# ssteinberg/wave_tracer

Measured on AMD Instinct MI355X. Metric: Msamples/sec (whole node), cornell-box 1440^2 wave-mode, higher is better.
Workload: dtype f32

## Files before the change

wave_tracer_amd/csrc/kernels_connect.hip:

```cpp
#include "wtgpu_kernels.h"

namespace wtk {

WT_D bool strategy_valid(const integrator_opts_t& o, int s, int t, int nS, int nT) {
    const int depth = t + s - 2;
    if (t > nT || s > nS) return false;
    if ((t == 1 && s == 1) || depth < 0 || depth > o.max_depth) return false;
    if (!o.emitter_direct && s == 1) return false;
    if (!o.sensor_direct && t == 1) return false;
    if (o.debug_only_s && (int)o.debug_only_s - 1 != s) return false;
    if (o.debug_only_t && (int)o.debug_only_t - 1 != t) return false;
    return true;
}
WT_D bool strategy_class_valid(const integrator_opts_t& o, int sk, int tk, int nS, int nT) {
    const int K = (int)kKeyDim - 1;
    const int t1 = tk < K ? tk : nT, s1 = sk < K ? sk : nS;
    for (int t = tk; t <= t1; ++t)
        for (int s = sk; s <= s1; ++s)
            if (strategy_valid(o, s, t, nS, nT)) return true;
    return false;
}
WT_D int wave_max_i(int v) {
#pragma unroll
    for (int off = 32; off > 0; off >>= 1) v = max(v, __shfl_xor(v, off, 64));
    return v;
}

__global__ void __launch_bounds__(kEnumBlock) k_connect_enum(launch_args_t a) {
    __shared__ uint32_t s_cnt[kNumKeys], s_base[kNumKeys];
    const uint32_t i = blockIdx.x * kEnumBlock + threadIdx.x;
    const size_t W2 = 2 * (size_t)a.st.cap;
    for (uint32_t k = threadIdx.x; k < kNumKeys; k += kEnumBlock) s_cnt[k] = 0;
    int nT = -1, nS = -1;
    if (i < a.nb) {
        nT = (int)a.st.walks[(size_t)(i) * a.st.walk_words + WT_WALK_NVERTS_WORD];
        nS = (int)a.st.walks[(size_t)(a.st.cap + i) * a.st.walk_words + WT_WALK_NVERTS_WORD];
#pragma unroll
        for (int c = 0; c < 4; ++c) a.st.lacc[(size_t)c * a.st.cap + i] = 0.0;
    }
    __syncthreads();
    const int K = (int)kKeyDim - 1;
    const int kT = nT < K ? nT : K, kS = nS < K ? nS : K;
    for (int tk = 0; tk <= kT; ++tk)
        for (int sk = 0; sk <= kS; ++sk)
            if (strategy_class_valid(a.sc.opts, sk, tk, nS, nT)) atomicAdd(&s_cnt[(uint32_t)tk * kKeyDim + (uint32_t)sk], 1u);
    __syncthreads();
    for (uint32_t k = threadIdx.x; k < kNumKeys; k += kEnumBlock) {
        const uint32_t c = s_cnt[k];
        s_base[k] = c ? atomicAdd(a.st.strat_count + k, c) : 0u;
        s_cnt[k] = 0;
    }
    __syncthreads();
    for (int tk = 0; tk <= kT; ++tk)
        for (int sk = 0; sk <= kS; ++sk)
            if (strategy_class_valid(a.sc.opts, sk, tk, nS, nT)) {
                const uint32_t key = (uint32_t)tk * kKeyDim + (uint32_t)sk;
                a.st.strat_items[(size_t)key * a.st.cap + s_base[key] + atomicAdd(&s_cnt[key], 1u)] = i;
            }
}
__global__ void __launch_bounds__(64) k_connect_scan(launch_args_t a) {
    if (a.st.ext)
        for (uint32_t q = threadIdx.x; q < a.st.ext->n_chunks * kChunkCtlWords; q += 64) a.st.ext->chunk_ctl[q] = 0;
    if (threadIdx.x == 0) {
        uint32_t acc = 0;
        for (uint32_t k = 0; k < kNumKeys; ++k) {
            const uint32_t c = a.st.strat_count[k];
            a.st.strat_prefix[k] = acc;
            acc += c;
            a.st.strat_count[k] = 0;
        }
        a.st.strat_prefix[kNumKeys] = acc;
        a.st.ctl[CTL_STRAT_HEAD] = 0;
        a.st.ctl[CTL_STRAT_HEAD_OPEN] = 0;

    }
}
template <bool OPEN>
WT_D void connect_strat_body(const launch_args_t& a) {
    __shared__ stack_entry_t lds[kLdsStack * kBlock];
    __shared__ uint32_t s_prefix[kNumKeys + 1];
    constexpr int K = (int)kKeyDim - 1;
    if (!OPEN) {
        for (uint32_t k = threadIdx.x; k <= kNumKeys; k += kBlock) s_prefix[k] = a.st.strat_prefix[k];
    } else if (threadIdx.x == 0) {
        uint32_t acc = 0;
        for (uint32_t k = 0; k < kNumKeys; ++k) {
            s_prefix[k] = acc;
            if ((int)(k / kKeyDim) == K || (int)(k % kKeyDim) == K) acc += a.st.strat_prefix[k + 1] - a.st.strat_prefix[k];
        }
        s_prefix[kNumKeys] = acc;
    }
    __syncthreads();
    const uint32_t total = s_prefix[kNumKeys];
    bdpt_counters_t ctr;
    memset(&ctr, 0, sizeof(ctr));
    stack_entry_t spill[kSpillStack];
    stack_ref_t stack;
    lds_stack(lds, spill, stack);
    const fsd_pool_t pool{a.st.fsd_hdr, a.st.fsd_edges, a.st.ctl + CTL_FSD_COUNTER, a.st.fsd_cap, a.st.ctl + CTL_FSD_ECOUNTER, a.st.fsd_ecap};
    for (;;) {
        const uint32_t idx = wave_grab(a.st.ctl + (OPEN ? CTL_STRAT_HEAD_OPEN : CTL_STRAT_HEAD)) + (threadIdx.x & 63);
        if (idx - (threadIdx.x & 63) >= total) break;
        if (idx < total) {
            uint32_t lo = 0, hi = kNumKeys;
            while (hi - lo > 1) {
                const uint32_t mid = (lo + hi) >> 1;
                if (s_prefix[mid] <= idx)
                    lo = mid;
                else
                    hi = mid;
            }
            const uint32_t key = lo;
            const int tk = (int)(key / kKeyDim), sk = (int)(key % kKeyDim);
            if (!OPEN && (tk == K || sk == K)) continue;
            const uint32_t i = a.st.strat_items[(size_t)key * a.st.cap + (idx - s_prefix[key])];
            const uint64_t j = a.j0 + i;
            const uint32_t pix = (uint32_t)(j % a.npix);
            const uint64_t smp = a.sample_begin + j / a.npix;
            const uint64_t sample_id = ((uint64_t)pix << 32) | (smp & 0xFFFFFFFFull);
            sample_ctx_t ctx;
            soa_load(a.st.ctx, kCtxWords, i, ctx);
            const vertex_store_t svs{a.st.verts, a.st.vert_words, i}, evs{a.st.verts, a.st.vert_words, (size_t)a.st.cap + i};
            auto one = [&](int s, int t) __attribute__((always_inline)) {
                const stokes_t flux = bdpt_strategy(a.sc, pool, a.film, svs, evs, s, t, ctx, a.seed, sample_id, stack, &ctr, nullptr);
                if (t > 1) {
#pragma unroll
                    for (int c = 0; c < 4; ++c)
                        if (flux.s[c] != 0.f) unsafeAtomicAdd(&a.st.lacc[(size_t)c * a.st.cap + i], (double)flux.s[c]);
                }
            };
            if constexpr (!OPEN) {
                one(sk, tk);
            } else {
                const int nT = (int)a.st.walks[(size_t)i * a.st.walk_words + WT_WALK_NVERTS_WORD];
                const int nS = (int)a.st.walks[((size_t)a.st.cap + i) * a.st.walk_words + WT_WALK_NVERTS_WORD];
                const int t1 = tk == K ? nT : tk, s1 = sk == K ? nS : sk;
                for (int t = tk; t <= t1; ++t)
                    for (int s = sk; s <= s1; ++s)
                        if (strategy_valid(a.sc.opts, s, t, nS, nT)) one(s, t);
            }
        }
    }
    if (a.count_stats) flush_counters(a.st.counters, ctr);
}
__global__ void __launch_bounds__(kBlock, WTGPU_LB_CONNECT) k_connect_strat(launch_args_t a) { connect_strat_body<false>(a); }
__global__ void __launch_bounds__(kBlock, WTGPU_LB_CONNECT) k_connect_strat_open(launch_args_t a) { connect_strat_body<true>(a); }
constexpr uint32_t kPendShadow = 0x80000000u;
WT_D void pending_append(const launch_args_t& a, uint32_t* cctl, bool keep, uint32_t i, int s, int t, const connect_ret_t& cr) {
    const bdpt_ext_t& x = *a.st.ext;
    const unsigned long long m = __ballot(keep);
    if (!m) return;
    const int lane = threadIdx.x & 63;
    const int leader = __ffsll((long long)m) - 1;
    uint32_t base = 0;
    if (lane == leader) base = atomicAdd(cctl + CHUNK_PEND_COUNT, (uint32_t)__popcll(m));
    base = (uint32_t)__shfl((int)base, leader, 64);
    const uint32_t slot = base + (uint32_t)__popcll(m & ((1ull << lane) - 1ull));
    if (!keep || slot >= x.pend_cap) return;
    conn_pending_t r;
    r.i = i;
    r.st = (uint32_t)s | ((uint32_t)t << 16) | (cr.need_shadow ? kPendShadow : 0u);
#pragma unroll
    for (int c = 0; c < 4; ++c) r.L[c] = cr.L.s[c];
    r.o[0] = cr.ray.o.x, r.o[1] = cr.ray.o.y, r.o[2] = cr.ray.o.z;
    r.d[0] = cr.ray.d.x, r.d[1] = cr.ray.d.y, r.d[2] = cr.ray.d.z;
    r.dist = cr.ray.dist;
    x.pend[slot] = r;
}
#ifndef WTGPU_LB_EVAL
#define WTGPU_LB_EVAL 2
#endif
__global__ void __launch_bounds__(kBlock, WTGPU_LB_EVAL) k_connect_eval(launch_args_t a, uint32_t chunk) {
    __shared__ uint32_t s_prefix[kNumKeys + 1];
    for (uint32_t k = threadIdx.x; k <= kNumKeys; k += kBlock) s_prefix[k] = a.st.strat_prefix[k];
    __syncthreads();
    const bdpt_ext_t& x = *a.st.ext;
    uint32_t* cctl = x.chunk_ctl + (size_t)chunk * kChunkCtlWords;
    const uint32_t total = s_prefix[kNumKeys];
    const uint64_t begin = (uint64_t)chunk * x.pend_cap;
    if (begin >= total) return;
    const uint32_t span = (uint32_t)min<uint64_t>(x.pend_cap, total - begin);
    bdpt_counters_t ctr;
    ctr.connections = ctr.shadow_rays = 0;
    const stack_ref_t no_stack = make_stack_ref(nullptr, 0, 0, 0, nullptr);
    const fsd_pool_t pool{a.st.fsd_hdr, a.st.fsd_edges, a.st.ctl + CTL_FSD_COUNTER, a.st.fsd_cap, a.st.ctl + CTL_FSD_ECOUNTER, a.st.fsd_ecap};
    for (;;) {
        const uint32_t off = wave_grab(cctl + CHUNK_EVAL_HEAD) + (threadIdx.x & 63);
        if (off - (threadIdx.x & 63) >= span) break;
        if (off < span) {
            const uint32_t idx = (uint32_t)begin + off;
            uint32_t lo = 0, hi = kNumKeys;
            while (hi - lo > 1) {
                const uint32_t mid = (lo + hi) >> 1;
                if (s_prefix[mid] <= idx)
                    lo = mid;
                else
                    hi = mid;
            }
            const uint32_t key = lo;
            const int t = (int)(key / kKeyDim), s = (int)(key % kKeyDim);
            const uint32_t i = a.st.strat_items[(size_t)key * a.st.cap + (idx - s_prefix[key])];
            const uint64_t j = a.j0 + i;
            const uint32_t pix = (uint32_t)(j % a.npix);
            const uint64_t smp = a.sample_begin + j / a.npix;
            const uint64_t sample_id = ((uint64_t)pix << 32) | (smp & 0xFFFFFFFFull);
            const vertex_store_t svs{a.st.verts, a.st.vert_words, i}, evs{a.st.verts, a.st.vert_words, (size_t)a.st.cap + i};
            connect_ret_t cr;
            bdpt_connect<true>(a.sc, pool, svs, evs, s, t, a.seed, sample_id, no_stack, cr, &ctr, nullptr);
            pending_append(a, cctl, cr.L.s[0] > 0.f, i, s, t, cr);
        }
    }
    if (a.count_stats) {
        unsigned long long vc = ctr.connections, vr = ctr.shadow_rays;
        for (int off = 32; off > 0; off >>= 1) {
            vc += __shfl_down(vc, off, 64);
            vr += __shfl_down(vr, off, 64);
        }
        if ((threadIdx.x & 63) == 0) {
            if (vc) atomicAdd(a.st.counters + offsetof(bdpt_counters_t, connections) / sizeof(unsigned long long), vc);
            if (vr) atomicAdd(a.st.counters + offsetof(bdpt_counters_t, shadow_rays) / sizeof(unsigned long long), vr);
        }
    }
}

__global__ void __launch_bounds__(kBlock, 4) k_connect_shadow(launch_args_t a, uint32_t chunk) {
    __shared__ stack_entry_t lds[kLdsStack * kBlock];
    stack_entry_t spill[kSpillStack];
    stack_ref_t stack;
    lds_stack(lds, spill, stack);
    const bdpt_ext_t& x = *a.st.ext;
    uint32_t* cctl = x.chunk_ctl + (size_t)chunk * kChunkCtlWords;
    const uint32_t n = min(cctl[CHUNK_PEND_COUNT], x.pend_cap);
    if (n == 0) return;
    for (;;) {
        const uint32_t idx = wave_grab(cctl + CHUNK_PEND_HEAD) + (threadIdx.x & 63);
        if (idx - (threadIdx.x & 63) >= n) break;
        bool alive = false;
        if (idx < n) {
            const conn_pending_t& r = x.pend[idx];
            alive = true;
            if (r.st & kPendShadow) alive = !ads_shadow_ray(a.sc, vec3{r.o[0], r.o[1], r.o[2]}, vec3{r.d[0], r.d[1], r.d[2]}, range_t{0.f, r.dist}, stack, nullptr);
        }
        wave_append(x.surv, cctl + CHUNK_SURV_COUNT, alive, idx);
    }
}

#ifndef WTGPU_LB_MIS
#define WTGPU_LB_MIS 2
#endif
__global__ void __launch_bounds__(kBlock, WTGPU_LB_MIS) k_connect_mis(launch_args_t a, uint32_t chunk) {
    const bdpt_ext_t& x = *a.st.ext;
    uint32_t* ctl = a.st.ctl;
    uint32_t* cctl = x.chunk_ctl + (size_t)chunk * kChunkCtlWords;
    const uint32_t n = cctl[CHUNK_SURV_COUNT];
    if (n == 0) return;
    const fsd_pool_t pool{a.st.fsd_hdr, a.st.fsd_edges, ctl + CTL_FSD_COUNTER, a.st.fsd_cap, ctl + CTL_FSD_ECOUNTER, a.st.fsd_ecap};
    bdpt_counters_t ctr;
    ctr.light_splats = 0;
    for (;;) {
        const uint32_t k = wave_grab(cctl + CHUNK_MIS_HEAD) + (threadIdx.x & 63);
        if (k - (threadIdx.x & 63) >= n) break;
        if (k < n) {
            const conn_pending_t& r = x.pend[x.surv[k]];
            const uint32_t i = r.i, st = r.st;
            const int s = (int)(st & 0xFFFFu), t = (int)((st >> 16) & 0x7FFFu);
            stokes_t L;
    #pragma unroll
            for (int c = 0; c < 4; ++c) L.s[c] = r.L[c];
            const uint64_t j = a.j0 + i;
            const uint32_t pix = (uint32_t)(j % a.npix);
            const uint64_t smp = a.sample_begin + j / a.npix;
            const uint64_t sample_id = ((uint64_t)pix << 32) | (smp & 0xFFFFFFFFull);
            sample_ctx_t ctx;
            soa_load(a.st.ctx, kCtxWords, i, ctx);
            const vertex_store_t svs{a.st.verts, a.st.vert_words, i}, evs{a.st.verts, a.st.vert_words, (size_t)a.st.cap + i};
            vertex_nb_t tv;
            sensor_element_t element;
            bool has_element = false;
            if (s <= 1 || t <= 1) bdpt_connect_temp(a.sc, svs, evs, s, t, a.seed, sample_id, tv, element, has_element);
            const stokes_t flux = bdpt_strategy_finish(a.sc, pool, a.film, svs, evs, s, t, ctx, L, tv, element, has_element, &ctr);
            if (t > 1) {
    #pragma unroll
                for (int c = 0; c < 4; ++c)
                    if (flux.s[c] != 0.f) unsafeAtomicAdd(&a.st.lacc[(size_t)c * a.st.cap + i], (double)flux.s[c]);
            }
        }
    }
    if (a.count_stats) {
        unsigned long long v = ctr.light_splats;
        for (int off = 32; off > 0; off >>= 1) v += __shfl_down(v, off, 64);
        if ((threadIdx.x & 63) == 0 && v) atomicAdd(a.st.counters + offsetof(bdpt_counters_t, light_splats) / sizeof(unsigned long long), v);
    }
}

__global__ void __launch_bounds__(kBlock) k_connect_splat(launch_args_t a) {
    const uint32_t i = blockIdx.x * kBlock + threadIdx.x;
    if (i >= a.nb) return;
    sample_ctx_t ctx;
    soa_load(a.st.ctx, kCtxWords, i, ctx);
    stokes_t L;
#pragma unroll
    for (int c = 0; c < 4; ++c) L.s[c] = (float)a.st.lacc[(size_t)c * a.st.cap + i];
    film_splat(a.sc, a.film, ctx.element, L, ctx.k);
}

__global__ void __launch_bounds__(kBlock) k_connect_splat_tiled(launch_args_t a) {
    extern __shared__ double tile[];
    const sensor_t& sn = a.sc.sensor;
    const uint32_t W = a.film.width, H = a.film.height;
    const uint32_t S = film_stokes(sn), P = sn.channels * S, PL = P + 1;
    const uint32_t bpr = (W + kBlock - 1) / kBlock;
    const uint32_t row = blockIdx.x / bpr, x0 = (blockIdx.x % bpr) * kBlock;
    const int r = sn.rf_radius;
    const uint32_t n_px = 3 * kSplatCols;
    for (uint32_t q = threadIdx.x; q < n_px * PL; q += kBlock) tile[q] = 0.0;
    __syncthreads();
    const uint32_t x = x0 + threadIdx.x;
    if (x < W && row < H) {
        const uint64_t p = (uint64_t)row * W + x;
        const uint64_t first = (p + a.npix - (a.j0 % a.npix)) % a.npix;
        for (uint64_t i = first; i < a.nb; i += a.npix) {
            sample_ctx_t ctx;
            soa_load(a.st.ctx, kCtxWords, i, ctx);
            stokes_t L;
#pragma unroll
            for (int c = 0; c < 4; ++c) L.s[c] = (float)a.st.lacc[(size_t)c * a.st.cap + i];
            const rfilter_weights_t rw = film_rfilter_weights(sn, ctx.element.offset);
            float val[16];
            for (uint32_t c = 0; c < sn.channels; ++c) {
                const float f = spectrum_f(a.sc, sn.response_spec[c], ctx.k);
                bool ok = true;
                for (uint32_t q = 0; q < S; ++q) {
                    val[c * S + q] = L.s[q] * f;
                    ok = ok && finitef(val[c * S + q]);
                }
                ok = ok && val[c * S] >= 0.f;
                if (!ok)
                    for (uint32_t q = 0; q < S; ++q) val[c * S + q] = 0.f;
            }
            for (int dy = -r; dy <= r; ++dy) {
                const int y = (int)ctx.element.y + dy;
                if (y < 0 || y >= (int)H) continue;
                for (int dx = -r; dx <= r; ++dx) {
                    const int xx = (int)ctx.element.x + dx;
                    if (xx < 0 || xx >= (int)W) continue;
                    const float w = fmaxf_(0.f, rw.wx[dx + r] * rw.wy[dy + r]) * rw.recp_total;
                    const int ty = y - ((int)row - 1), tx = xx - ((int)x0 - 1);
                    if (ty >= 0 && ty < 3 && tx >= 0 && tx < (int)kSplatCols) {
                        const uint32_t q = (uint32_t)ty * kSplatCols + (uint32_t)tx;
                        unsafeAtomicAdd(&tile[q], (double)w);
                        for (uint32_t c = 0; c < P; ++c) unsafeAtomicAdd(&tile[(size_t)(1 + c) * n_px + q], (double)(w * val[c]));
                    } else {
                        const size_t pix = (size_t)y * W + xx;
                        film_add(&a.film.weight[pix], (double)w);
                        for (uint32_t c = 0; c < P; ++c) film_add(&a.film.value[pix * P + c], (double)(w * val[c]));
                    }
                }
            }
        }
    }
    __syncthreads();
    for (uint32_t q = threadIdx.x; q < n_px; q += kBlock) {
        const int y = (int)row - 1 + (int)(q / kSplatCols), xx = (int)x0 - 1 + (int)(q % kSplatCols);
        if (y < 0 || y >= (int)H || xx < 0 || xx >= (int)W) continue;
        const size_t pix = (size_t)y * W + xx;
        const double wsum = tile[q];
        if (wsum != 0.0) film_add(&a.film.weight[pix], wsum);
        for (uint32_t c = 0; c < P; ++c) {
            const double v = tile[(size_t)(1 + c) * n_px + q];
            if (v != 0.0) film_add(&a.film.value[pix * P + c], v);
        }
    }
}

}
```

wave_tracer_amd/csrc/wt/bdpt.h:

```cpp
#pragma once
#include <cstddef>

#include "bvh.h"
#include "film.h"
#include "fsd.h"

namespace wt {

constexpr uint32_t kMaxVerts = 18;
#ifndef WT_MAX_WALK_ITERS
#define WT_MAX_WALK_ITERS 96
#endif
constexpr uint32_t kMaxWalkIters = WT_MAX_WALK_ITERS;
constexpr uint32_t kWalkIterLimit = 4096;
constexpr uint32_t kMaxConeTris = 64;
#ifdef WT_ORACLE_UNBOUNDED
constexpr uint32_t kMaxEdgeIds = 16384;
#else
constexpr uint32_t kMaxEdgeIds = 96;
#endif

enum vertex_type_e : uint32_t { VT_SENSOR = 0, VT_EMITTER = 1, VT_SURFACE = 2, VT_MEDIUM = 3, VT_FSD = 4 };
enum geo_kind_e : uint32_t { GEO_NONE = 0, GEO_POINT = 1, GEO_SURFACE = 2 };

struct vertex_t {
    uint32_t type;
    uint32_t transport;
    uint32_t delta;
    uint32_t fraunhofer_fsd;
    float pdf_fwd, pdf_bwd;
    float rr_weight;
    int32_t ref;
    int32_t emitter_of_shape;
    uint32_t fsd_slot;
    uint32_t geo_kind;
    uint32_t has_beam;
    surface_t surf;
    beam_t beam;
};
constexpr size_t kVertexWords = sizeof(vertex_t) / 4;
struct vertex_nb_t {
    uint32_t type;
    uint32_t transport;
    uint32_t delta;
    uint32_t fraunhofer_fsd;
    float pdf_fwd, pdf_bwd;
    float rr_weight;
    int32_t ref;
    int32_t emitter_of_shape;
    uint32_t fsd_slot;
    uint32_t geo_kind;
    uint32_t has_beam;
    surface_t surf;
    struct {
        float k;
    } beam;
};
static_assert(offsetof(vertex_nb_t, beam) == offsetof(vertex_t, beam) && offsetof(vertex_nb_t, surf) == offsetof(vertex_t, surf), "vertex_nb_t is a prefix of vertex_t");

struct vertex_store_t {
    uint32_t* base;
    size_t stride;
    size_t idx;
    vertex_t* stage = nullptr;
    uint32_t* staged_idx = nullptr;
    WT_HD void load(uint32_t v, vertex_t& out) const { soa_load(base + (size_t)v * kVertexWords, stride, idx, out); }
    WT_HD void load(uint32_t v, vertex_nb_t& out) const {
        const uint32_t* b = base + (size_t)v * kVertexWords + idx * stride;
        uint32_t* w = reinterpret_cast<uint32_t*>(&out);
#if defined(__HIP_DEVICE_COMPILE__)
#pragma unroll
#endif
        for (size_t i = 0; i < offsetof(vertex_t, beam) / 4; ++i) w[i] = b[i];
        out.beam.k = load_word<float>(v, (offsetof(vertex_t, beam) + offsetof(beam_t, k)) / 4);
    }
    WT_HD vec3 load_wp(uint32_t v) const {
        constexpr size_t o = (offsetof(vertex_t, surf) + offsetof(surface_t, wp)) / 4;
        return vec3{load_word<float>(v, o), load_word<float>(v, o + 1), load_word<float>(v, o + 2)};
    }
    WT_HD void store(uint32_t v, const vertex_t& in) const {
        if (stage) {
            *stage = in;
            *staged_idx = v;
            return;
        }
        soa_store(base + (size_t)v * kVertexWords, stride, idx, in);
    }
    template <class F>
    WT_HD void store_word(uint32_t v, size_t word, F value) const {
        static_assert(sizeof(F) == 4, "");
        uint32_t w;
        __builtin_memcpy(&w, &value, 4);
        if (stage && *staged_idx == v) {
            reinterpret_cast<uint32_t*>(stage)[word] = w;
            return;
        }
        base[idx * stride + (size_t)v * kVertexWords + word] = w;
    }
    template <class F>
    WT_HD F load_word(uint32_t v, size_t word) const {
        const uint32_t w = base[idx * stride + (size_t)v * kVertexWords + word];
        F f;
        __builtin_memcpy(&f, &w, 4);
        return f;
    }
};
#define WT_VWORD(field) (offsetof(vertex_t, field) / 4)

struct fsd_pool_t {
    fsd_aperture_t* hdr;
    fsd_edge_t* edges;
    uint32_t* counter;
    uint32_t cap;
    uint32_t* edge_counter;
    uint32_t edge_cap;
};
WT_HD fsd_edges_ref_t fsd_pool_edges(const fsd_pool_t& p, uint32_t slot) {
    return fsd_edges_ref_t{p.edges + (size_t)p.hdr[slot].edge_offset, 1};
}
WT_HD bool fsd_pool_alloc_edges(const fsd_pool_t& p, uint32_t slot, uint32_t need, fsd_aperture_t& ap) {
    if (!p.edge_counter) {
        ap.edge_offset = slot * kFsdMaxEdges;
        ap.edge_cap = kFsdMaxEdges;
        return true;
    }
    if (need > kFsdMaxEdges) need = kFsdMaxEdges;
    uint32_t off = 0;
    if (need) {
#if defined(__HIP_DEVICE_COMPILE__)
        off = atomicAdd(p.edge_counter, need);
#else
        off = __atomic_fetch_add(p.edge_counter, need, __ATOMIC_RELAXED);
#endif
    }
    ap.edge_offset = off;
    ap.edge_cap = need;
    if ((size_t)off + need > p.edge_cap) {
        ap.edge_offset = 0;
        ap.edge_cap = 0;
        return false;
    }
    return true;
}
WT_HD uint32_t fsd_pool_alloc(const fsd_pool_t& p) {
#if defined(__HIP_DEVICE_COMPILE__)
    const unsigned long long m = __ballot(1);
    const int lane = (int)(threadIdx.x & 63u);
    const int leader = __ffsll((long long)m) - 1;
    uint32_t base = 0;
    if (lane == leader) base = atomicAdd(p.counter, (uint32_t)__popcll(m));
    base = (uint32_t)__shfl((int)base, leader, 64);
    return base + (uint32_t)__popcll(m & ((1ull << lane) - 1ull));
#else
    return __atomic_fetch_add(p.counter, 1u, __ATOMIC_RELAXED);
#endif
}

template <class V>
WT_HD vec3 vertex_wp(const V& v) { return v.surf.wp; }
template <class V>
WT_HD bool vertex_is_on_surface(const scene_t& sc, const V& v) {
    return v.type == VT_SURFACE || (v.type == VT_EMITTER && emitter_is_area(sc.emitters[v.ref])) ||
           (v.type == VT_SENSOR && v.geo_kind == GEO_SURFACE);
}
template <class V>
WT_HD bool vertex_has_real_surface(const scene_t& sc, const V& v) {
    return v.type == VT_SURFACE || (v.type == VT_EMITTER && emitter_is_area(sc.emitters[v.ref]));
}
template <class V>
WT_HD vec3 vertex_ng(const scene_t& sc, const V& v) { return vertex_has_real_surface(sc, v) ? v.surf.geo.n : vec3{0, 0, 1}; }
template <class V>
WT_HD vec3 vertex_ns(const scene_t& sc, const V& v) { return vertex_has_real_surface(sc, v) ? v.surf.shading.n : vec3{0, 0, 1}; }
WT_HD bool vertex_is_interaction(const vertex_t& v) { return v.type == VT_FSD || v.type == VT_SURFACE || v.type == VT_MEDIUM; }
WT_HD bool vertex_on_emitter(const vertex_t& v) { return v.type == VT_EMITTER || (v.type == VT_SURFACE && v.emitter_of_shape >= 0); }
template <class V>
WT_HD int vertex_get_emitter(const V& v) { return v.type == VT_EMITTER ? v.ref : v.emitter_of_shape; }
template <class V>
WT_HD bool vertex_is_delta_emitter(const scene_t& sc, const V& v) {
    return v.type == VT_EMITTER && (emitter_is_delta_direction(sc.emitters[v.ref]) || emitter_is_delta_position(sc.emitters[v.ref]));
}
template <class V>
WT_HD bool vertex_is_delta_sensor(const scene_t& sc, const V& v) {
    return v.type == VT_SENSOR && (sensor_is_delta_direction(sc.sensor) || sensor_is_delta_position(sc.sensor));
}
WT_HD bool vertex_is_connectible(const scene_t& sc, const vertex_t& v) {
    switch (v.type) {
    case VT_FSD: return true;
    case VT_EMITTER: return !emitter_is_delta_direction(sc.emitters[v.ref]);
    case VT_SENSOR: return !sensor_is_delta_direction(sc.sensor);
    case VT_SURFACE: return !material_is_delta_only(sc, v.ref, v.beam.k);
    default: return false;
    }
}
WT_HD vec3 geo_offseted_ray_origin(const scene_t& sc, const vertex_t& v, vec3 ro, vec3 rd) {
    return v.geo_kind == GEO_SURFACE ? surface_offseted_ray_origin(sc, v.surf, ro, rd) : ro;
}

template <class V>
WT_HD float convert_directional_density_to_area(const scene_t& sc, float dpdf_tagged, vec3 p, const V& next) {
    const float dens = pd_density_or_zero(dpdf_tagged);
    if (dens == 0.f) return 0.f;
    const vec3 d = vertex_wp(next) - p;
    const float d2 = length2(d);
    if (d2 == 0.f) return WT_INF;
    float ppdf = dens * (1.f / d2);
    if (vertex_is_on_surface(sc, next)) ppdf *= fabsf(dot(vertex_ng(sc, next), normalize(d)));
    return ppdf;
}
template <class V, class N>
WT_HD float vertex_pdf_next_from_sensor(const scene_t& sc, const V& v, const N& next) {
    const vec3 dl = vertex_wp(next) - vertex_wp(v);
    const float recp_dist2 = 1.f / length2(dl);
    const vec3 d = dl * sqrtf(recp_dist2);
    const float dpdf = pd_density_or_zero(sensor_pdf_direction(sc, d));
    float ppdf = dpdf * recp_dist2;
    if (vertex_is_on_surface(sc, next)) ppdf *= fabsf(dot(vertex_ng(sc, next), d));
    return ppdf;
}
WT_HD float vertex_pdf_sensor(const scene_t& sc) { return pd_density_or_zero(sensor_pdf_position(sc)); }
template <class V, class N>
WT_HD float vertex_pdf_next_from_emitter(const scene_t& sc, const V& v, const N& next) {
    const vec3 dl = vertex_wp(next) - vertex_wp(v);
    const float recp_dist2 = 1.f / length2(dl);
    const vec3 d = dl * sqrtf(recp_dist2);
    const int ei = vertex_get_emitter(v);
    if (emitter_is_infinite(sc.emitters[ei])) return directional_pdf_target_position(sc.emitters[ei], vertex_wp(next));
    const float dpdf = pd_density_or_zero(emitter_pdf_direction(sc, ei, d, vertex_has_real_surface(sc, v) ? &v.surf : nullptr));
    float ppdf = dpdf * recp_dist2;
    if (vertex_is_on_surface(sc, next)) ppdf *= fabsf(dot(vertex_ng(sc, next), d));
    return ppdf;
}
template <class V>
WT_HD float vertex_pdf_emitter(const scene_t& sc, const V& v) {
    const int ei = vertex_get_emitter(v);
    return sc.emitters[ei].select_pmf * pd_density_or_zero(emitter_pdf_position(sc, ei, vertex_has_real_surface(sc, v) ? &v.surf : nullptr));
}
template <class V, class N>
WT_HD float vertex_pdf(const scene_t& sc, const fsd_pool_t& pool, const V& v, vec3 prev_wp, const N& next, uint32_t mode) {
    if (v.type == VT_EMITTER) return vertex_pdf_next_from_emitter(sc, v, next);
    if (v.type == VT_SENSOR) return vertex_pdf_next_from_sensor(sc, v, next);
    const vec3 p = vertex_wp(v);
    const vec3 wiworld = normalize(prev_wp - p);
    const vec3 woworld = normalize(vertex_wp(next) - p);
    float pdf = 0.f;
    if (v.type == VT_SURFACE) {
        const vec3 wi = to_local(v.surf.shading, wiworld), wo = to_local(v.surf.shading, woworld);
        pdf = material_pdf(sc, v.ref, wi, wo, v.beam.k, mode, v.surf.uv);
    } else if (v.type == VT_FSD) {
        const fsd_aperture_t ap = pool.hdr[v.fsd_slot];
        pdf = fsd_pdf(ap, fsd_pool_edges(pool, v.fsd_slot), to_local(ap.frame, woworld));
    }
    return convert_directional_density_to_area(sc, pdf, p, next);
}

WT_HD bool vertex_interact(const scene_t& sc, const fsd_pool_t& pool, const vertex_t& v, vec3 next_wp, bool ignore_fsd, beam_t& out) {
    const vec3 wiworld = -v.beam.env.d;
    const float k = v.beam.k;
    float f = 0.f;
    if (v.fraunhofer_fsd && !ignore_fsd) {
        const fsd_aperture_t ap = pool.hdr[v.fsd_slot];
        const vec3 woworld = normalize(next_wp - vertex_wp(v));
        f = fsd_pdf(ap, fsd_pool_edges(pool, v.fsd_slot), to_local(ap.frame, woworld));
    }
    if (v.type == VT_SURFACE) {
        const surface_t& srf = v.surf;
        const vec3 woworld = normalize(next_wp - vertex_wp(v));
        const vec3 wi = to_local(srf.shading, wiworld), wo = to_local(srf.shading, woworld);
        const vec3 ng = srf.geo.n, ns = srf.shading.n;
        const float wig = dot(wiworld, ng), wog = dot(woworld, ng);
        const float wis = wi.z, wos = wo.z;
        if (wig * wis <= 0.f || wog * wos <= 0.f) return false;
        mueller_t M = material_f(sc, v.ref, wi, wo, k, v.transport, v.surf.uv);
        float scale = 1.f / fabsf(wos);
        if (!veq(ns, ng)) scale *= shading_normals_correction_scale(v.transport, wig, wog, wis, wos);
        M = M * scale;
        if (f > 0.f) M = M + mueller_identity() * f;
        if (mueller_mean_intensity(M) == 0.f) return false;
        out = v.beam;
        beam_transform_surface_interaction(out, srf, woworld, M, 1.f);
        return true;
    }
    if (v.type == VT_FSD) {
        const vec3 p = vertex_wp(v);
        const float beam_dist = dot(p - v.beam.env.o, v.beam.env.d);
        const vec3 woworld = normalize(next_wp - p);
        out = v.beam;
        beam_transform_region_interaction(out, p, beam_dist, woworld, f);
        return true;
    }
    return false;
}

struct conn_end_t {
    vec3 wp, ng;
    uint32_t geo_kind, tuid;
};
template <class V>
WT_HD conn_end_t conn_end_of(const V& v) { return conn_end_t{v.surf.wp, v.surf.geo.n, v.geo_kind, v.surf.tuid}; }
WT_HD vec3 conn_end_offseted_origin(const scene_t& sc, const conn_end_t& e, vec3 ro, vec3 rd) {
    if (e.geo_kind != GEO_SURFACE || e.tuid == kInvalid) return ro;
    const tri_geo_t g = sc.tri_geo[e.tuid];
    const vec3 err = triangle_fp_errors(g.a, g.b, g.c, ro);
    const float offset_dist = dot(err, vabs(e.ng));
    const vec3 offset = offset_dist * e.ng;
    return ro + (dot(rd, offset) >= 0.f ? offset : -offset);
}
struct shadow_ray_t {
    vec3 o, d;
    float dist;
};
WT_HD shadow_ray_t conn_shadow_ray(const scene_t& sc, const conn_end_t& a, const conn_end_t& b) {
    const vec3 rd = normalize(b.wp - a.wp);
    const vec3 o = conn_end_offseted_origin(sc, a, a.wp, rd);
    const vec3 t = conn_end_offseted_origin(sc, b, b.wp, -rd);
    const float dist = length(t - o);
    return shadow_ray_t{o, (t - o) / dist, dist};
}
WT_HD bool bdpt_shadow(const scene_t& sc, const vertex_t& a, const vertex_t& b, const stack_ref_t& stack, bvh_counters_t* ctr) {
    const shadow_ray_t r = conn_shadow_ray(sc, conn_end_of(a), conn_end_of(b));
    return ads_shadow_ray(sc, r.o, r.d, range_t{0.f, r.dist}, stack, ctr);
}

struct walk_t {
    beam_t beam;
    float pdf_from_prev;
    float throughput, rr_weight;
    uint32_t nverts;
    uint32_t active;
    uint32_t rng_draws;
    vec3 prev_wp, prev_ng;
    uint32_t prev_on_surface;
    uint32_t prev_offset_tuid;
};

#define WT_WALK_NVERTS_WORD (offsetof(walk_t, nverts) / 4)

struct sample_ctx_t {
    float k;
    float recp_spectral_pd;
    float k_density;
    sensor_element_t element;
};

struct bdpt_counters_t {
    unsigned long long segments, ray_queries, cone_queries, vertices, connections, shadow_rays;
    unsigned long long cone_tri_overflow, edge_overflow, fsd_edge_overflow, fsd_pool_overflow, fsd_interactions, null_interactions;
    unsigned long long surface_interactions, light_splats;
};

WT_HD void walk_cache_prev(const scene_t& sc, walk_t& w, const vertex_t& v) {
    w.prev_wp = vertex_wp(v);
    w.prev_ng = vertex_ng(sc, v);
    w.prev_on_surface = vertex_is_on_surface(sc, v);
    w.prev_offset_tuid = v.geo_kind == GEO_SURFACE ? v.surf.tuid : kInvalid;
}

WT_HD void bdpt_generate(const scene_t& sc, uint64_t seed, uint64_t sample_id, uint32_t px, uint32_t py, sample_ctx_t& ctx, walk_t& sw, walk_t& ew,
                         const vertex_store_t& svs, const vertex_store_t& evs) {
    sampler_t smp = make_sampler(seed, sample_id, STREAM_SCENE);
    const emitter_k_sample_t ek = scene_sample_emitter_and_spectrum(sc, smp);
    const float k = ek.wavenumber.k;
    const emitter_sample_t es = emitter_sample(sc, ek.emitter, k, smp);
    const bool disc = pd_is_discrete(ek.wavenumber.wpd);
    ctx.k = k;
    ctx.recp_spectral_pd = disc ? 1.f / pd_mass(ek.wavenumber.wpd) : 1.f / scene_sum_spectral_pdf(sc, k);
    ctx.k_density = disc ? pd_mass(ek.wavenumber.wpd) : ek.wavenumber.wpd;
    const sensor_sample_t ss = sensor_sample(sc, px, py, k, smp);
    ctx.element = ss.element;

    vertex_t v;
    v.type = VT_SENSOR;
    v.transport = TRANSPORT_BACKWARD;
    v.delta = 0;
    v.fraunhofer_fsd = 0;
    v.pdf_fwd = -1.f;
    v.pdf_bwd = pd_density_or_zero(ss.ppd);
    v.rr_weight = 1.f;
    v.ref = -1;
    v.emitter_of_shape = -1;
    v.fsd_slot = kInvalid;
    v.has_beam = 1;
    v.beam = ss.beam;
    if (ss.has_surface) {
        v.geo_kind = GEO_SURFACE;
        v.surf = ss.surface;
    } else {
        v.geo_kind = GEO_POINT;
        v.surf = make_dummy_surface(vec3{0, 0, 1}, ss.beam.env.o);
    }
    svs.store(0, v);
    sw.beam = ss.beam;
    sw.pdf_from_prev = ss.dpd;
    sw.throughput = 1.f;
    sw.rr_weight = 1.f;
    sw.nverts = 1;
    sw.active = 1;
    sw.rng_draws = 0;
    walk_cache_prev(sc, sw, v);

    v.type = VT_EMITTER;
    v.transport = TRANSPORT_FORWARD;
    v.pdf_fwd = pd_density_or_zero(es.ppd) * ek.emitter_pdf;
    v.pdf_bwd = -1.f;
    v.ref = ek.emitter;
    v.beam = es.beam;
    if (es.has_surface) {
        v.geo_kind = GEO_SURFACE;
        v.surf = es.surface;
    } else {
        v.geo_kind = GEO_POINT;
        v.surf = make_dummy_surface(vec3{0, 0, 1}, es.beam.env.o);
    }
    evs.store(0, v);
    ew.beam = es.beam;
    ew.pdf_from_prev = es.dpd;
    ew.throughput = 1.f;
    ew.rr_weight = 1.f;
    ew.nverts = 1;
    ew.active = 1;
    ew.rng_draws = 0;
    walk_cache_prev(sc, ew, v);
}

struct walk_trace_in_t {
    cone_t env;
    float k;
    vec3 prev_ng;
    uint32_t prev_offset_tuid;
};
template <class F>
WT_HD F soa_word(const uint32_t* base, size_t stride, size_t idx, size_t word) {
    static_assert(sizeof(F) == 4, "");
    const uint32_t w = base[idx * stride + word];
    F f;
    __builtin_memcpy(&f, &w, 4);
    return f;
}
#define WT_WALK_WORD(field) (offsetof(walk_t, field) / 4)
WT_HD walk_trace_in_t walk_load_trace_in(const uint32_t* base, size_t stride, size_t idx) {
    walk_trace_in_t r;
    r.env.o = {soa_word<float>(base, stride, idx, WT_WALK_WORD(beam.env.o.x)), soa_word<float>(base, stride, idx, WT_WALK_WORD(beam.env.o.y)),
               soa_word<float>(base, stride, idx, WT_WALK_WORD(beam.env.o.z))};
    r.env.d = {soa_word<float>(base, stride, idx, WT_WALK_WORD(beam.env.d.x)), soa_word<float>(base, stride, idx, WT_WALK_WORD(beam.env.d.y)),
               soa_word<float>(base, stride, idx, WT_WALK_WORD(beam.env.d.z))};
    r.env.x = {soa_word<float>(base, stride, idx, WT_WALK_WORD(beam.env.x.x)), soa_word<float>(base, stride, idx, WT_WALK_WORD(beam.env.x.y)),
               soa_word<float>(base, stride, idx, WT_WALK_WORD(beam.env.x.z))};
    r.env.x0 = soa_word<float>(base, stride, idx, WT_WALK_WORD(beam.env.x0));
    r.env.tan_alpha = soa_word<float>(base, stride, idx, WT_WALK_WORD(beam.env.tan_alpha));
    r.env.e = soa_word<float>(base, stride, idx, WT_WALK_WORD(beam.env.e));
    r.env.one_over_e = soa_word<float>(base, stride, idx, WT_WALK_WORD(beam.env.one_over_e));
    r.env.z_apex = soa_word<float>(base, stride, idx, WT_WALK_WORD(beam.env.z_apex));
    r.k = soa_word<float>(base, stride, idx, WT_WALK_WORD(beam.k));
    r.prev_ng = {soa_word<float>(base, stride, idx, WT_WALK_WORD(prev_ng.x)), soa_word<float>(base, stride, idx, WT_WALK_WORD(prev_ng.y)),
                 soa_word<float>(base, stride, idx, WT_WALK_WORD(prev_ng.z))};
    r.prev_offset_tuid = soa_word<uint32_t>(base, stride, idx, WT_WALK_WORD(prev_offset_tuid));
    return r;
}
WT_HD cone_t walk_trace_envelope(const scene_t& sc, const walk_trace_in_t& w) {
    cone_t env = w.env;
    if (w.prev_offset_tuid != kInvalid) {
        const tri_geo_t g = sc.tri_geo[w.prev_offset_tuid];
        const vec3 err = triangle_fp_errors(g.a, g.b, g.c, env.o);
        const float offset_dist = dot(err, vabs(w.prev_ng));
        const vec3 offset = offset_dist * w.prev_ng;
        env.o = env.o + (dot(env.d, offset) >= 0.f ? offset : -offset);
    }
    return env;
}

WT_HD cone_t walk_trace_envelope(const scene_t& sc, const walk_t& w) {
    cone_t env = w.beam.env;
    if (w.prev_offset_tuid != kInvalid) {
        const tri_geo_t g = sc.tri_geo[w.prev_offset_tuid];
        const vec3 err = triangle_fp_errors(g.a, g.b, g.c, env.o);
        const float offset_dist = dot(err, vabs(w.prev_ng));
        const vec3 offset = offset_dist * w.prev_ng;
        env.o = env.o + (dot(env.d, offset) >= 0.f ? offset : -offset);
    }
    return env;
}

WT_HD bool walk_append_vertex(const scene_t& sc, walk_t& w, const vertex_store_t& vs, vertex_t& v, float pdf_fwd, float pdf_revr) {
    if (veq(w.prev_wp, vertex_wp(v))) return false;
    const float pv = convert_directional_density_to_area(sc, w.pdf_from_prev, w.prev_wp, v);
    if (v.transport == TRANSPORT_FORWARD)
        v.pdf_fwd = pv;
    else
        v.pdf_bwd = pv;
    v.beam = w.beam;
    v.has_beam = 1;
    {
        const float dens = pd_density_or_zero(pdf_revr);
        float prev_rev = 0.f;
        if (dens != 0.f) {
            const vec3 d = w.prev_wp - vertex_wp(v);
            const float d2 = length2(d);
            if (d2 == 0.f)
                prev_rev = WT_INF;
            else {
                prev_rev = dens * (1.f / d2);
                if (w.prev_on_surface) prev_rev *= fabsf(dot(w.prev_ng, normalize(d)));
            }
        }
        vs.store_word(w.nverts - 1, v.transport == TRANSPORT_BACKWARD ? WT_VWORD(pdf_fwd) : WT_VWORD(pdf_bwd), prev_rev);
    }
    w.pdf_from_prev = pdf_fwd;
    vs.store(w.nverts, v);
    w.nverts++;
    walk_cache_prev(sc, w, v);
    return true;
}

WT_HD bool walk_continue(const scene_t& sc, walk_t& w, const vertex_store_t& vs, bool allow_RR, sampler_t& smp) {
    if ((int)w.nverts > sc.opts.max_depth + 1) return false;
    if (!allow_RR || !sc.opts.RR) return true;
    vs.store_word(w.nverts - 1, WT_VWORD(rr_weight), w.rr_weight);
    const float r = w.throughput < 1.f ? fmaxf_(w.throughput, .5f) : 1.f;
    if (sampler_r(smp) <= r) {
        const float scale = 1.f / r;
        w.rr_weight *= scale;
        w.throughput *= scale;
        return true;
    }
    return false;
}

WT_HD float region_triangle_flux(const scene_t& sc, const frame_t& beam_frame, const cone_t& envelope, const range_t& izr, vec2 sigma, uint32_t tuid,
                                 bool want_front) {
    const tri_geo_t g = sc.tri_geo[tuid];
    const bool front_face = dot(g.n, -envelope.d) > 0.f;
    if (front_face != want_front) return 0.f;
    return region_local_triangle_flux(envelope, izr, centre(izr), sigma, to_local(beam_frame, g.a - envelope.o), to_local(beam_frame, g.b - envelope.o),
                                      to_local(beam_frame, g.c - envelope.o));
}

struct fsd_defer_t {
    uint32_t split_no_primary, no_primary;
    uint32_t known_no_primary;
    uint32_t has_gather, gather_n_edges, gather_edge_overflow;
    float gather_flux;
    const uint32_t* gather_edges;
    uint32_t defer_sampling, to_sampling_pass, have_aperture;
    uint32_t pending, resolved;
    uint32_t slot, base, next_try, end_draws;
    fsd_sample_t fs;
#ifdef WTGPU_STEP_PROF
    long long marks[8];
#endif
};

#if defined(WTGPU_STEP_PROF) && defined(__HIP_DEVICE_COMPILE__)
#define WT_STEP_MARK(i) \
    if (defer) defer->marks[i] = clock64()
#else
#define WT_STEP_MARK(i) ((void)0)
#endif
template <int MODE = 0, class TriList>
WT_HD bool bdpt_walk_step(const scene_t& sc, walk_t& w, const trav_result_t& tr, const TriList& tris, const vertex_store_t& vs,
                          const fsd_pool_t& pool, uint64_t seed, uint64_t sample_id, uint32_t stream, bdpt_counters_t* ctr,
                          const stack_ref_t* primary_query_stack = nullptr, fsd_defer_t* defer = nullptr) {
    if (tr.empty) return false;
    sampler_t smp = make_sampler(seed, sample_id, stream, w.rng_draws);
    beam_t& beam = w.beam;
    const float beam_dist = tr.dist;
    const range_t izr{beam_dist, beam_dist + tr.region_depth};
    const bool is_ballistic = tr.ballistic || beam_is_ray(beam);
    const vec3 origin_wp = tr.origin;
    const vec3 interaction_wp = origin_wp + izr.min * beam.env.d;
    const frame_t beam_frame = cone_frame(beam.env);
    const cone_t envelope = beam.env;
    const vec3 sd3 = beam_footprint(beam, beam_dist) / kBeamEnvelope;
    const vec2 sigma{sd3.x, sd3.y};

    uint32_t primary = kInvalid;
    ray_tri_hit_t phit{WT_INF, 0.f, 0.f};
    double integrated_flux = 0.0;
    if (is_ballistic) {
        primary = tr.tuid;
        phit.dist = tr.dist;
        phit.bx = tr.bx;
        phit.by = tr.by;
    } else {
        if (defer && defer->known_no_primary) {
        } else if (tr.aborted == 2) {
            if (tr.tuid != kInvalid) {
                primary = tr.tuid;
                phit.dist = tr.pdist;
                phit.bx = tr.bx;
                phit.by = tr.by;
            }
        } else if (primary_query_stack && tr.overflow > 0) {
            const float wtol = cone_intersection_tolerance(origin_wp, sc.world_min, sc.world_max, sc.world_max);
            ray_hit_t rh;
            if (ads_intersect_ray(sc, origin_wp, beam.env.d, grow(izr, wtol), *primary_query_stack, rh)) {
                const tri_geo_t g = sc.tri_geo[rh.tuid];
                const float fptol = cone_intersection_tolerance(origin_wp, g.a, g.b, g.c);
                if (contains(grow(izr, fptol), rh.dist)) {
                    primary = rh.tuid;
                    phit.dist = rh.dist;
                    phit.bx = rh.bx;
                    phit.by = rh.by;
                }
            }
        } else
        for (uint32_t i = 0; i < tr.ntris; ++i) {
            const uint32_t tuid = tris[i];
            const tri_geo_t g = sc.tri_geo[tuid];
            const float fptol = cone_intersection_tolerance(origin_wp, g.a, g.b, g.c);
            ray_tri_hit_t h;
            if (intersect_ray_tri(origin_wp, beam.env.d, g.a, g.b, g.c, grow(izr, fptol), h) && h.dist < phit.dist) {
                primary = tuid;
                phit = h;
            }
        }
        if (primary == kInvalid && defer && defer->split_no_primary) {
            defer->no_primary = 1;
            return false;
        }
        WT_STEP_MARK(0);
    }

    bool do_RR = true;
    bool ok = true;
    bool took_surface = false;
    if constexpr (MODE != 2) {
    if (primary != kInvalid) {
        took_surface = true;
        const tri_geo_t g = sc.tri_geo[primary];
        const vec3 sampled_tri_wp = origin_wp + envelope.d * phit.dist;
        surface_t srf = make_surface(sc, primary, g.n, vec2{phit.bx, phit.by}, sampled_tri_wp);
        srf.footprint = beam_surface_footprint_static(beam, srf, beam_dist);
        const shape_t shp = sc.shapes[srf.shape];
        const float k = beam.k;
        const uint32_t transport = beam.transport;
        const vec3 ng = srf.geo.n, ns = srf.shading.n;
        const vec3 wiworld = -beam.env.d;
        const vec3 wi = to_local(srf.shading, wiworld);
        const float wig = dot(wiworld, ng), wis = wi.z;
        ok = wig * wis > 0.f;
        bsdf_sample_t bs;
        if (ok) {
            bs = material_sample(sc, shp.material, wi, k, transport, smp, srf.uv);
            ok = bs.valid && bs.dpd != 0.f;
        }
        if (ok) {
            const bool is_delta = pd_is_discrete(bs.dpd);
            const vec3 wo = bs.wo;
            const vec3 woworld = normalize(to_world(srf.shading, wo));
            const float wog = dot(woworld, ng), wos = wo.z;
            if (ctr) ctr->surface_interactions++;
            ok = wog * wos > 0.f;
            if (ok) {
                const float pdf_revr = material_pdf(sc, shp.material, wo, wi, k, flip_transport(transport), srf.uv);
                vertex_t v;
                v.type = VT_SURFACE;
                v.transport = transport;
                v.delta = is_delta;
                v.fraunhofer_fsd = 0;
                v.pdf_fwd = v.pdf_bwd = -1.f;
                v.rr_weight = 1.f;
                v.ref = shp.material;
                v.emitter_of_shape = shp.emitter;
                v.fsd_slot = kInvalid;
                v.geo_kind = GEO_SURFACE;
                v.surf = srf;
                ok = walk_append_vertex(sc, w, vs, v, bs.dpd, pdf_revr);
                if (ok) {
                    if (ctr) ctr->vertices++;
                    float ws = 1.f;
                    if (!veq(ns, ng)) ws *= shading_normals_correction_scale(transport, wig, wog, wis, wos);
                    beam_transform_surface_interaction(beam, srf, woworld, bs.M, ws);
                    w.throughput *= ws * mueller_mean_intensity(bs.M);
                    if (transport == TRANSPORT_BACKWARD && bs.eta != 1.f) w.throughput /= sqr(bs.eta);
                }
            }
        }
    }
    }
    if constexpr (MODE != 1) {
    if (!took_surface) {
        WT_STEP_MARK(1);
        uint32_t edge_ids[kMaxEdgeIds];
        const uint32_t* eids = edge_ids;
        uint32_t n_edge_ids = 0;
        const bool have_ap = defer && (defer->resolved || defer->have_aperture);
        if (have_ap) {
            n_edge_ids = 1;
        } else if (sc.opts.FSD && !is_ballistic && defer && defer->has_gather) {
            n_edge_ids = defer->gather_n_edges;
            eids = defer->gather_edges;
            if (ctr) ctr->edge_overflow += defer->gather_edge_overflow;
        } else if (sc.opts.FSD && !is_ballistic) {
            for (uint32_t i = 0; i < tr.ntris; ++i) {
                const tri_meta_t m = sc.tri_meta[tris[i]];
                for (int e = 0; e < 3; ++e) {
                    const uint32_t id = m.edge[e];
                    if (id == kInvalid) continue;
                    uint32_t pos = 0;
                    while (pos < n_edge_ids && edge_ids[pos] < id) ++pos;
                    if (pos < n_edge_ids && edge_ids[pos] == id) continue;
                    if (n_edge_ids == kMaxEdgeIds) {
                        if (ctr) ctr->edge_overflow++;
                        continue;
                    }
                    for (uint32_t j = n_edge_ids; j > pos; --j) edge_ids[j] = edge_ids[j - 1];
                    edge_ids[pos] = id;
                    ++n_edge_ids;
                }
            }
        }
        WT_STEP_MARK(2);
        if (n_edge_ids > 0) {
            const bool resume = defer && defer->resolved;
            const uint32_t slot = have_ap ? defer->slot : fsd_pool_alloc(pool);
            if (slot >= pool.cap) {
                if (ctr) ctr->fsd_pool_overflow++;
                ok = false;
            } else {
                fsd_aperture_t ap;
                if (have_ap) {
                    ap = pool.hdr[slot];
                } else {
                    uint32_t need = 0;
                    if (pool.edge_counter) {
                        const vec2 cse = sigma * kBeamEnvelope;
                        const float max_len = .33f * fmaxf_(cse.x, cse.y);
                        for (uint32_t ei = 0; ei < n_edge_ids; ++ei) need += fsd_count_segments(sc, beam_frame, envelope, cse, max_len, eids[ei]);
                    }
                    if (!fsd_pool_alloc_edges(pool, slot, need, ap) && ctr) ctr->fsd_pool_overflow++;
                }
                const fsd_edges_ref_t ed{pool.edges + (size_t)ap.edge_offset, 1};
                if (!have_ap) {
                    fsd_build_aperture(sc, beam_frame, beam.k, 1.f, envelope, eids, n_edge_ids, sigma, ap, ed);
                    WT_STEP_MARK(3);
                    if (ctr && ap.overflow) ctr->fsd_edge_overflow += ap.overflow;
                    pool.hdr[slot] = ap;
                    if (ap.n_edges > 0 && defer && defer->defer_sampling) {
                        defer->to_sampling_pass = 1;
                        defer->slot = slot;
                        return false;
                    }
                }
                if (ap.n_edges > 0 && !resume) {
                    if (defer && defer->has_gather) {
                        integrated_flux = defer->gather_flux;
                    } else {
                        for (uint32_t i = 0; i < tr.ntris; ++i)
                            integrated_flux += region_triangle_flux(sc, beam_frame, envelope, izr, sigma, tris[i], tr.front_face != 0);
                    }
                    const float I = (float)(1.0 - integrated_flux);
                    ap.recp_I = I > 0.f ? 1.f / I : 0.f;
                    pool.hdr[slot] = ap;
                }
                if (ap.n_edges == 0) {
                    beam_transform_restart(beam, interaction_wp, beam_dist);
                    do_RR = false;
                } else {
                    fsd_sample_t fs;
                    if (!defer) {
                        fs = fsd_sample(sc, ap, ed, smp);
                    } else if (resume) {
                        fs = defer->fs;
                        sampler_seek(smp, defer->end_draws);
                    } else {
                        const uint32_t max_tries = fsd_max_tries(ap), base = fsd_tries_base(smp);
                        const uint32_t t1 = max_tries < kFsdInlineTries ? max_tries : kFsdInlineTries;
                        fsd_try_t r{{0.f, 0.f}, 0.f, 0u};
                        const uint32_t t = fsd_run_tries(sc, ap, ed, smp, base, 0, t1, r);
                        if (t == 0xFFFFFFFFu && t1 < max_tries) {
                            defer->pending = 1;
                            defer->slot = slot;
                            defer->base = base;
                            defer->next_try = t1;
                            return false;
                        }
                        const bool accepted = t != 0xFFFFFFFFu;
                        sampler_seek(smp, fsd_draws_after(base, accepted ? t : max_tries - 1u));
                        fs = fsd_finalize(ap, accepted, r.x, r.f);
                    }
                    ok = !(fs.dpd == 0.f || fs.weight == 0.f);
                    if (ok) {
                        if (ctr) ctr->fsd_interactions++;
                        const vec3 woworld = to_world(ap.frame, fs.wo);
                        vertex_t v;
                        v.type = VT_FSD;
                        v.transport = beam.transport;
                        v.delta = 0;
                        v.fraunhofer_fsd = 1;
                        v.pdf_fwd = v.pdf_bwd = -1.f;
                        v.rr_weight = 1.f;
                        v.ref = -1;
                        v.emitter_of_shape = -1;
                        v.fsd_slot = slot;
                        v.geo_kind = GEO_POINT;
                        v.surf = make_dummy_surface(vec3{0, 0, 1}, interaction_wp);
                        ok = walk_append_vertex(sc, w, vs, v, fs.dpd, fs.dpd);
                        if (ok) {
                            if (ctr) ctr->vertices++;
                            beam_transform_region_interaction(beam, interaction_wp, beam_dist, woworld, fs.weight);
                            w.throughput *= fs.weight;
                        }
                    }
                }
            }
        } else {
            do_RR = false;
            beam_transform_restart(beam, interaction_wp, beam_dist);
            if (ctr) ctr->null_interactions++;
        }
    }
    }
    WT_STEP_MARK(4);
    bool cont = false;
    if (ok) cont = walk_continue(sc, w, vs, do_RR, smp);
    WT_STEP_MARK(5);
    w.rng_draws = smp.draws;
    return cont;
}

enum walk_class_e : uint32_t { WCLS_DIFFUSE = 0, WCLS_DIELECTRIC = 1, WCLS_SPM = 2, WCLS_ANY = 3, kNumWalkClasses = 4, WCLS_NO_PRIMARY = 4, WCLS_END = 5 };
struct primary_hit_t {
    uint32_t tuid;
    float dist, bx, by;
};
WT_HD uint32_t walk_class_of_material_type(int32_t type) { return type >= 0 && type < (int32_t)MAT_COMPOSITE ? (uint32_t)type : (uint32_t)WCLS_ANY; }
WT_HD uint32_t walk_class_of_triangle(const scene_t& sc, uint32_t tuid) {
    return walk_class_of_material_type(sc.materials[sc.shapes[sc.tri_meta[tuid].shape_idx].material].type);
}
template <class TriList>
WT_HD uint32_t bdpt_classify(const scene_t& sc, vec3 beam_d, bool beam_ray, const trav_result_t& tr, const TriList& tris, const unsigned char* tri_class, primary_hit_t& ph) {
    ph.tuid = kInvalid;
    ph.dist = WT_INF;
    ph.bx = ph.by = 0.f;
    if (tr.empty) return WCLS_END;
    const bool is_ballistic = tr.ballistic || beam_ray;
    if (is_ballistic) {
        ph.tuid = tr.tuid;
        ph.dist = tr.dist;
        ph.bx = tr.bx;
        ph.by = tr.by;
    } else if (tr.aborted == 2) {
        if (tr.tuid != kInvalid) {
            ph.tuid = tr.tuid;
            ph.dist = tr.pdist;
            ph.bx = tr.bx;
            ph.by = tr.by;
        }
    } else {
        const range_t izr{tr.dist, tr.dist + tr.region_depth};
        for (uint32_t i = 0; i < tr.ntris; ++i) {
            const uint32_t tuid = tris[i];
            const tri_geo_t g = sc.tri_geo[tuid];
            const float fptol = cone_intersection_tolerance(tr.origin, g.a, g.b, g.c);
            ray_tri_hit_t h;
            if (intersect_ray_tri(tr.origin, beam_d, g.a, g.b, g.c, grow(izr, fptol), h) && h.dist < ph.dist) {
                ph.tuid = tuid;
                ph.dist = h.dist;
                ph.bx = h.bx;
                ph.by = h.by;
            }
        }
    }
    if (ph.tuid == kInvalid) return WCLS_NO_PRIMARY;
    return tri_class ? (uint32_t)tri_class[ph.tuid] : walk_class_of_triangle(sc, ph.tuid);
}

struct walk_rec_t {
    uint32_t* p;
    template <class F>
    WT_HD F get(size_t word) const {
        static_assert(sizeof(F) == 4, "");
        const uint32_t w = p[word];
        F f;
        __builtin_memcpy(&f, &w, 4);
        return f;
    }
    template <class F>
    WT_HD void set(size_t word, F value) const {
        static_assert(sizeof(F) == 4, "");
        uint32_t w;
        __builtin_memcpy(&w, &value, 4);
        p[word] = w;
    }
    WT_HD vec3 get3(size_t word) const { return vec3{get<float>(word), get<float>(word + 1), get<float>(word + 2)}; }
    WT_HD void set3(size_t word, vec3 v) const {
        set(word, v.x);
        set(word + 1, v.y);
        set(word + 2, v.z);
    }
};
template <int CLS>
WT_HD bool bdpt_surface_step(const scene_t& sc, const walk_rec_t& wr, vec3 origin_wp, float beam_dist, const primary_hit_t& ph, const vertex_store_t& vs, uint64_t seed,
                             uint64_t sample_id, uint32_t stream, bdpt_counters_t* ctr) {
    sampler_t smp = make_sampler(seed, sample_id, stream, wr.get<uint32_t>(WT_WALK_WORD(rng_draws)));
    cone_t env;
    {
        uint32_t* e = reinterpret_cast<uint32_t*>(&env);
#if defined(__HIP_DEVICE_COMPILE__)
#pragma unroll
#endif
        for (size_t i = 0; i < sizeof(cone_t) / 4; ++i) e[i] = wr.p[WT_WALK_WORD(beam.env) + i];
    }
    const float k = wr.get<float>(WT_WALK_WORD(beam.k));
    const uint32_t transport = wr.get<uint32_t>(WT_WALK_WORD(beam.transport));
    const uint32_t primary = ph.tuid;
    const vec3 gn = sc.tri_geo[primary].n;
    const vec3 sampled_tri_wp = origin_wp + env.d * ph.dist;
    surface_t srf = make_surface(sc, primary, gn, vec2{ph.bx, ph.by}, sampled_tri_wp);
    srf.footprint = cone_surface_footprint_static(env, srf, beam_dist);
    const shape_t shp = sc.shapes[srf.shape];
    const vec3 ng = srf.geo.n, ns = srf.shading.n;
    const vec3 wiworld = -env.d;
    const vec3 wi = to_local(srf.shading, wiworld);
    const float wig = dot(wiworld, ng), wis = wi.z;
    if (!(wig * wis > 0.f)) return false;
    const bsdf_sample_t bs = material_sample<CLS>(sc, shp.material, wi, k, transport, smp, srf.uv);
    if (!(bs.valid && bs.dpd != 0.f)) return false;
    const bool is_delta = pd_is_discrete(bs.dpd);
    const vec3 wo = bs.wo;
    const vec3 woworld = normalize(to_world(srf.shading, wo));
    const float wog = dot(woworld, ng), wos = wo.z;
    if (ctr) ctr->surface_interactions++;
    if (!(wog * wos > 0.f)) return false;
    const float pdf_revr = material_pdf<CLS>(sc, shp.material, wo, wi, k, flip_transport(transport), srf.uv);
    const vec3 prev_wp = wr.get3(WT_WALK_WORD(prev_wp));
    if (veq(prev_wp, srf.wp)) return false;
    uint32_t nverts = wr.get<uint32_t>(WT_WALK_WORD(nverts));
    {
        struct {
            uint32_t type;
            int32_t ref;
            uint32_t geo_kind;
            const surface_t& surf;
        } vview{VT_SURFACE, shp.material, GEO_SURFACE, srf};
        const float pv = convert_directional_density_to_area(sc, wr.get<float>(WT_WALK_WORD(pdf_from_prev)), prev_wp, vview);
        const uint32_t hdr[12] = {VT_SURFACE,
                                  transport,
                                  is_delta ? 1u : 0u,
                                  0u,
                                  __builtin_bit_cast(uint32_t, transport == TRANSPORT_FORWARD ? pv : -1.f),
                                  __builtin_bit_cast(uint32_t, transport == TRANSPORT_FORWARD ? -1.f : pv),
                                  __builtin_bit_cast(uint32_t, 1.f),
                                  (uint32_t)shp.material,
                                  (uint32_t)shp.emitter,
                                  kInvalid,
                                  (uint32_t)GEO_SURFACE,
                                  1u};
        static_assert(WT_VWORD(type) == 0 && WT_VWORD(transport) == 1 && WT_VWORD(delta) == 2 && WT_VWORD(fraunhofer_fsd) == 3 && WT_VWORD(pdf_fwd) == 4 && WT_VWORD(pdf_bwd) == 5 &&
                          WT_VWORD(rr_weight) == 6 && WT_VWORD(ref) == 7 && WT_VWORD(emitter_of_shape) == 8 && WT_VWORD(fsd_slot) == 9 && WT_VWORD(geo_kind) == 10 &&
                          WT_VWORD(has_beam) == 11 && WT_VWORD(surf) == 12,
                      "vertex_t header layout");
        uint32_t* vp = vs.base + vs.idx * vs.stride + (size_t)nverts * kVertexWords;
#if defined(__HIP_DEVICE_COMPILE__)
#pragma unroll
#endif
        for (int i = 0; i < 12; ++i) vp[i] = hdr[i];
        const uint32_t* sw = reinterpret_cast<const uint32_t*>(&srf);
#if defined(__HIP_DEVICE_COMPILE__)
#pragma unroll
#endif
        for (size_t i = 0; i < sizeof(surface_t) / 4; ++i) vp[WT_VWORD(surf) + i] = sw[i];
        const uint32_t* ew = reinterpret_cast<const uint32_t*>(&env);
#if defined(__HIP_DEVICE_COMPILE__)
#pragma unroll
#endif
        for (size_t i = 0; i < sizeof(cone_t) / 4; ++i) vp[WT_VWORD(beam) + i] = ew[i];
#if defined(__HIP_DEVICE_COMPILE__)
#pragma unroll
#endif
        for (size_t i = sizeof(cone_t) / 4; i < sizeof(beam_t) / 4; ++i) vp[WT_VWORD(beam) + i] = wr.p[WT_WALK_WORD(beam) + i];
        const float dens = pd_density_or_zero(pdf_revr);
        float prev_rev = 0.f;
        if (dens != 0.f) {
            const vec3 d = prev_wp - srf.wp;
            const float d2 = length2(d);
            if (d2 == 0.f)
                prev_rev = WT_INF;
            else {
                prev_rev = dens * (1.f / d2);
                if (wr.get<uint32_t>(WT_WALK_WORD(prev_on_surface))) prev_rev *= fabsf(dot(wr.get3(WT_WALK_WORD(prev_ng)), normalize(d)));
            }
        }
        vs.store_word(nverts - 1, transport == TRANSPORT_BACKWARD ? WT_VWORD(pdf_fwd) : WT_VWORD(pdf_bwd), prev_rev);
        ++nverts;
        wr.set(WT_WALK_WORD(pdf_from_prev), bs.dpd);
        wr.set(WT_WALK_WORD(nverts), nverts);
        wr.set3(WT_WALK_WORD(prev_wp), srf.wp);
        wr.set3(WT_WALK_WORD(prev_ng), ng);
        wr.set(WT_WALK_WORD(prev_on_surface), 1u);
        wr.set(WT_WALK_WORD(prev_offset_tuid), srf.tuid);
    }
    if (ctr) ctr->vertices++;
    float ws = 1.f;
    if (!veq(ns, ng)) ws *= shading_normals_correction_scale(transport, wig, wog, wis, wos);
    {
        beam_t b;
        float sid;
        b.env = cone_through_surface_footprint(srf, srf.wp, woworld, env.tan_alpha, &sid);
        b.k = k;
        b.transport = transport;
        uint32_t* bw = reinterpret_cast<uint32_t*>(&b);
#if defined(__HIP_DEVICE_COMPILE__)
#pragma unroll
#endif
        for (size_t i = offsetof(beam_t, frame) / 4; i < sizeof(beam_t) / 4; ++i) bw[i] = wr.p[WT_WALK_WORD(beam) + i];
        beam_apply_bsdf(b, ws * bs.M, woworld, srf, cone_frame(b.env));
        b.self_intersection_distance = sid;
#if defined(__HIP_DEVICE_COMPILE__)
#pragma unroll
#endif
        for (size_t i = 0; i < sizeof(beam_t) / 4; ++i) wr.p[WT_WALK_WORD(beam) + i] = bw[i];
    }
    float throughput = wr.get<float>(WT_WALK_WORD(throughput)) * (ws * mueller_mean_intensity(bs.M));
    if (transport == TRANSPORT_BACKWARD && bs.eta != 1.f) throughput /= sqr(bs.eta);
    bool cont = true;
    float rr_weight = wr.get<float>(WT_WALK_WORD(rr_weight));
    if ((int)nverts > sc.opts.max_depth + 1)
        cont = false;
    else if (sc.opts.RR) {
        vs.store_word(nverts - 1, WT_VWORD(rr_weight), rr_weight);
        const float r = throughput < 1.f ? fmaxf_(throughput, .5f) : 1.f;
        if (sampler_r(smp) <= r) {
            const float scale = 1.f / r;
            rr_weight *= scale;
            throughput *= scale;
        } else
            cont = false;
    }
    wr.set(WT_WALK_WORD(throughput), throughput);
    wr.set(WT_WALK_WORD(rr_weight), rr_weight);
    wr.set(WT_WALK_WORD(rng_draws), smp.draws);
    return cont;
}

WT_HD uint32_t connect_stream(int s, int t) {
    if (s < 32 && t < 32) return STREAM_CONNECT + (uint32_t)t * 32u + (uint32_t)s;
    return STREAM_CONNECT + 1024u + (uint32_t)t * 4096u + (uint32_t)s;
}
struct connect_ret_t {
    stokes_t L;
    vertex_t temporary_vert;
    uint32_t has_temp;
    sensor_element_t element;
    uint32_t has_element;
    shadow_ray_t ray;
    uint32_t need_shadow;
};

template <bool DEFER>
WT_HD stokes_t connect_and_integrate(const scene_t& sc, const beam_t& db, const conn_end_t& dv, const beam_t& eb, const conn_end_t& ev, const stack_ref_t& stack,
                                     bdpt_counters_t* ctr, bvh_counters_t* bctr, connect_ret_t& ret) {
    if (beam_intensity(db) == 0.f || beam_intensity(eb) == 0.f) return stokes_zero();
    if (ctr) ctr->shadow_rays++;
    const shadow_ray_t ray = conn_shadow_ray(sc, dv, ev);
    if (DEFER) {
        const stokes_t L = integrate_beams(db, eb);
        if (L.s[0] > 0.f) {
            ret.ray = ray;
            ret.need_shadow = 1;
        }
        return L;
    }
    if (ads_shadow_ray(sc, ray.o, ray.d, range_t{0.f, ray.dist}, stack, bctr)) return stokes_zero();
    return integrate_beams(db, eb);
}

WT_HD void make_temp_vertex(vertex_t& v, uint32_t type, uint32_t transport, int ref, bool has_surface, const surface_t& surface, vec3 p) {
    v.type = type;
    v.transport = transport;
    v.delta = 0;
    v.fraunhofer_fsd = 0;
    v.pdf_fwd = v.pdf_bwd = -1.f;
    v.rr_weight = 1.f;
    v.ref = ref;
    v.emitter_of_shape = -1;
    v.fsd_slot = kInvalid;
    v.has_beam = 0;
    if (has_surface) {
        v.geo_kind = GEO_SURFACE;
        v.surf = surface;
    } else {
        v.geo_kind = GEO_POINT;
        v.surf = make_dummy_surface(vec3{0, 0, 1}, p);
    }
}
WT_HD bool vertex_store_connectible(const scene_t& sc, const vertex_store_t& vs, uint32_t idx) {
    struct {
        uint32_t type;
        int32_t ref;
        struct {
            float k;
        } beam;
    } v{vs.load_word<uint32_t>(idx, WT_VWORD(type)), vs.load_word<int32_t>(idx, WT_VWORD(ref)), {vs.load_word<float>(idx, WT_VWORD(beam) + offsetof(beam_t, k) / 4)}};
    switch (v.type) {
    case VT_FSD: return true;
    case VT_EMITTER: return !emitter_is_delta_direction(sc.emitters[v.ref]);
    case VT_SENSOR: return !sensor_is_delta_direction(sc.sensor);
    case VT_SURFACE: return !material_is_delta_only(sc, v.ref, v.beam.k);
    default: return false;
    }
}

template <bool DEFER = false>
WT_HD void bdpt_connect(const scene_t& sc, const fsd_pool_t& pool, const vertex_store_t& svs, const vertex_store_t& evs, int s, int t,
                        uint64_t seed, uint64_t sample_id, const stack_ref_t& stack, connect_ret_t& ret, bdpt_counters_t* ctr, bvh_counters_t* bctr) {
    ret.L = stokes_zero();
    ret.has_temp = 0;
    ret.has_element = 0;
    ret.need_shadow = 0;
    sampler_t smp = make_sampler(seed, sample_id, connect_stream(s, t));
    if (ctr) ctr->connections++;

    if (s == 0) {
        vertex_t last;
        svs.load(t - 1, last);
        if (vertex_on_emitter(last)) {
            beam_t QE = last.beam;
            beam_scale(QE, last.rr_weight);
            ret.L = emitter_Li(sc, vertex_get_emitter(last), QE, last.surf);
        }
    } else if (t == 0) {
        if (sensor_is_virtual(sc.sensor)) {
            vertex_t last;
            evs.load(s - 1, last);
            vertex_nb_t current;
            evs.load(s - 2, current);
            const vec3 wp_end = vertex_wp(last);
            const beam_t& beam = last.beam;
            const float dist = length(wp_end - beam.env.o);
            sensor_direct_connection_t dc = vplane_Si(sc, beam, range_t{0.f, dist});
            if (dc.valid) {
                ret.element = dc.element;
                ret.has_element = 1;
                float wgt = current.rr_weight;
                if (vertex_is_on_surface(sc, current) && (current.type == VT_FSD || current.type == VT_SURFACE || current.type == VT_MEDIUM) && !current.delta)
                    wgt /= fabsf(dot(dc.beam.env.d, vertex_ns(sc, current)));
                wgt /= fabsf(dot(dc.beam.env.d, dc.surface.geo.n));
                beam_scale(dc.beam, wgt);
                make_temp_vertex(ret.temporary_vert, VT_SENSOR, TRANSPORT_BACKWARD, -1, true, dc.surface, dc.beam.env.o);
                ret.has_temp = 1;
                ret.L = integrate_beams(dc.beam, beam);
            }
        }
    } else if (s == 1) {
        vertex_t last;
        svs.load(t - 1, last);
        if (vertex_is_connectible(sc, last)) {
            const float k = last.beam.k;
            const vec3 wp = vertex_wp(last);
            emitter_direct_sample_t ed = scene_sample_emitter_direct(sc, wp, k, smp);
            if ((pd_is_discrete(ed.dpd) || ed.dpd != 0.f) && beam_intensity(ed.beam) > 0.f) {
                float wgt = last.rr_weight;
                if (vertex_is_on_surface(sc, last)) wgt *= fabsf(dot(ed.beam.env.d, vertex_ns(sc, last)));
                beam_scale(ed.beam, wgt);
                make_temp_vertex(ret.temporary_vert, VT_EMITTER, TRANSPORT_FORWARD, ed.emitter, ed.has_surface, ed.surface, ed.beam.env.o);
                ret.has_temp = 1;
                beam_t db;
                if (vertex_interact(sc, pool, last, vertex_wp(ret.temporary_vert), false, db))
                    ret.L = connect_and_integrate<DEFER>(sc, db, conn_end_of(last), ed.beam, conn_end_of(ret.temporary_vert), stack, ctr, bctr, ret);
            }
        }
    } else if (t == 1) {
        vertex_t last;
        evs.load(s - 1, last);
        const bool is_virtual = sensor_is_virtual(sc.sensor);
        const bool do_direct = (is_virtual || last.type != VT_FSD) && vertex_is_connectible(sc, last);
        if (do_direct) {
            sensor_direct_sample_t sd = sensor_sample_direct(sc, vertex_wp(last), last.beam.k, smp);
            if ((pd_is_discrete(sd.dpd) || sd.dpd != 0.f) && beam_intensity(sd.beam) > 0.f) {
                float wgt = last.rr_weight;
                if (vertex_is_on_surface(sc, last)) wgt *= fabsf(dot(sd.beam.env.d, vertex_ns(sc, last)));
                beam_scale(sd.beam, wgt);
                make_temp_vertex(ret.temporary_vert, VT_SENSOR, TRANSPORT_BACKWARD, -1, sd.has_surface, sd.surface, sd.beam.env.o);
                ret.has_temp = 1;
                beam_t eb;
                if (vertex_interact(sc, pool, last, vertex_wp(ret.temporary_vert), false, eb)) {
                    ret.L = connect_and_integrate<DEFER>(sc, sd.beam, conn_end_of(ret.temporary_vert), eb, conn_end_of(last), stack, ctr, bctr, ret);
                    ret.element = sd.element;
                    ret.has_element = 1;
                }
            }
        }
    } else {
        const vec3 ev_wp = evs.load_wp(s - 1), sv_wp = svs.load_wp(t - 1);
        const vec3 dl = ev_wp - sv_wp;
        if (vertex_store_connectible(sc, evs, s - 1) && vertex_store_connectible(sc, svs, t - 1) && !(dl.x == 0.f && dl.y == 0.f && dl.z == 0.f)) {
            beam_t eb, db;
            conn_end_t ev_end, sv_end;
            vec3 ev_ns, sv_ns;
            bool ev_on, sv_on, heb, hdb = false;
            float ev_rr, sv_rr;
            {
                vertex_t ev;
                evs.load(s - 1, ev);
                heb = vertex_interact(sc, pool, ev, sv_wp, true, eb);
                ev_end = conn_end_of(ev);
                ev_ns = vertex_ns(sc, ev);
                ev_on = vertex_is_on_surface(sc, ev);
                ev_rr = ev.rr_weight;
            }
            if (heb) {
                vertex_t sv;
                svs.load(t - 1, sv);
                hdb = vertex_interact(sc, pool, sv, ev_wp, true, db);
                sv_end = conn_end_of(sv);
                sv_ns = vertex_ns(sc, sv);
                sv_on = vertex_is_on_surface(sc, sv);
                sv_rr = sv.rr_weight;
            }
            if (heb && hdb) {
                const float recp_d2 = 1.f / length2(dl);
                const vec3 d = dl * sqrtf(recp_d2);
                float wev = ev_rr;
                float wsv = sv_rr * recp_d2;
                if (sv_on) wev *= fabsf(dot(sv_ns, d));
                if (ev_on) wsv *= fabsf(dot(ev_ns, d));
                beam_scale(db, wsv);
                beam_scale(eb, wev);
                ret.L = connect_and_integrate<DEFER>(sc, db, sv_end, eb, ev_end, stack, ctr, bctr, ret);
            }
        }
    }
}
WT_HD void bdpt_connect_temp(const scene_t& sc, const vertex_store_t& svs, const vertex_store_t& evs, int s, int t, uint64_t seed, uint64_t sample_id, vertex_nb_t& tv,
                             sensor_element_t& element, bool& has_element) {
    has_element = false;
    vertex_t tmp;
    bool has_temp = false;
    sampler_t smp = make_sampler(seed, sample_id, connect_stream(s, t));
    if (s == 0) {
    } else if (t == 0) {
        if (sensor_is_virtual(sc.sensor)) {
            vertex_t last;
            evs.load(s - 1, last);
            const float dist = length(vertex_wp(last) - last.beam.env.o);
            const sensor_direct_connection_t dc = vplane_Si(sc, last.beam, range_t{0.f, dist});
            if (dc.valid) {
                element = dc.element;
                has_element = true;
                make_temp_vertex(tmp, VT_SENSOR, TRANSPORT_BACKWARD, -1, true, dc.surface, dc.beam.env.o);
                has_temp = true;
            }
        }
    } else if (s == 1) {
        const emitter_direct_sample_t ed = scene_sample_emitter_direct(sc, svs.load_wp(t - 1), svs.load_word<float>(t - 1, WT_VWORD(beam) + offsetof(beam_t, k) / 4), smp);
        make_temp_vertex(tmp, VT_EMITTER, TRANSPORT_FORWARD, ed.emitter, ed.has_surface, ed.surface, ed.beam.env.o);
        has_temp = true;
    } else if (t == 1) {
        const sensor_direct_sample_t sd = sensor_sample_direct(sc, evs.load_wp(s - 1), evs.load_word<float>(s - 1, WT_VWORD(beam) + offsetof(beam_t, k) / 4), smp);
        make_temp_vertex(tmp, VT_SENSOR, TRANSPORT_BACKWARD, -1, sd.has_surface, sd.surface, sd.beam.env.o);
        has_temp = true;
        element = sd.element;
        has_element = true;
    }
    if (has_temp) __builtin_memcpy(&tv, &tmp, offsetof(vertex_t, beam));
    tv.beam.k = 0.f;
}

template <class TV>
WT_HD float bdpt_mis_weight(const scene_t& sc, const fsd_pool_t& pool, const vertex_store_t& svs, const vertex_store_t& evs, int s, int t, const TV& tv) {
    if (s + t <= 2) return 1.f;
    float srev_last = 0.f, srev_prev = 0.f, spdf_first = 0.f, erev_last = 0.f, erev_prev = 0.f, epdf_first = 0.f;
    bool has_srev_last = false, has_srev_prev = false, has_spdf_first = false, has_erev_last = false, has_erev_prev = false, has_epdf_first = false;
    if (s == 0) {
        vertex_nb_t last, prev;
        svs.load(t - 1, last);
        svs.load(t - 2, prev);
        srev_last = vertex_pdf_emitter(sc, last);
        srev_prev = vertex_pdf_next_from_emitter(sc, last, prev);
        has_srev_last = has_srev_prev = true;
    } else if (t == 0) {
        vertex_nb_t prev;
        evs.load(s - 2, prev);
        erev_last = vertex_pdf_sensor(sc);
        if (sensor_is_virtual(sc.sensor))
            erev_prev = vertex_pdf_next_from_sensor(sc, tv, prev);
        else {
            vertex_nb_t last;
            evs.load(s - 1, last);
            erev_prev = vertex_pdf_next_from_sensor(sc, last, prev);
        }
        has_erev_last = has_erev_prev = true;
    } else if (s == 1) {
        vertex_nb_t last;
        svs.load(t - 1, last);
        srev_last = vertex_pdf_next_from_emitter(sc, tv, last);
        erev_last = vertex_pdf(sc, pool, last, svs.load_wp(t - 2), tv, TRANSPORT_BACKWARD);
        epdf_first = vertex_pdf_emitter(sc, tv);
        has_srev_last = has_erev_last = has_epdf_first = true;
    } else if (t == 1) {
        vertex_nb_t last;
        evs.load(s - 1, last);
        erev_last = vertex_pdf_next_from_sensor(sc, tv, last);
        srev_last = vertex_pdf(sc, pool, last, evs.load_wp(s - 2), tv, TRANSPORT_FORWARD);
        spdf_first = vertex_pdf_sensor(sc);
        has_erev_last = has_srev_last = has_spdf_first = true;
    } else {
        vertex_nb_t ev, sv;
        evs.load(s - 1, ev);
        svs.load(t - 1, sv);
        const vec3 ev_prev_wp = evs.load_wp(s - 2), sv_prev_wp = svs.load_wp(t - 2);
        vertex_nb_t ev_prev, sv_prev;
        evs.load(s - 2, ev_prev);
        svs.load(t - 2, sv_prev);
        erev_last = vertex_pdf(sc, pool, sv, sv_prev_wp, ev, TRANSPORT_BACKWARD);
        erev_prev = vertex_pdf(sc, pool, ev, vertex_wp(sv), ev_prev, TRANSPORT_BACKWARD);
        srev_last = vertex_pdf(sc, pool, ev, ev_prev_wp, sv, TRANSPORT_FORWARD);
        srev_prev = vertex_pdf(sc, pool, sv, vertex_wp(ev), sv_prev, TRANSPORT_FORWARD);
        has_erev_last = has_erev_prev = has_srev_last = has_srev_prev = true;
    }
    bool delta_emitter, delta_sensor;
    if (s == 1)
        delta_emitter = vertex_is_delta_emitter(sc, tv);
    else if (s > 1) {
        struct {
            uint32_t type;
            int32_t ref;
        } ev0{evs.load_word<uint32_t>(0, WT_VWORD(type)), evs.load_word<int32_t>(0, WT_VWORD(ref))};
        delta_emitter = vertex_is_delta_emitter(sc, ev0);
    } else
        delta_emitter = true;
    if (t == 1)
        delta_sensor = vertex_is_delta_sensor(sc, tv);
    else if (t > 1) {
        struct {
            uint32_t type;
        } sv0{svs.load_word<uint32_t>(0, WT_VWORD(type))};
        delta_sensor = vertex_is_delta_sensor(sc, sv0);
    } else
        delta_sensor = true;

    float sum_Ri = 0.f, ri = 1.f;
    {
        bool del_i = false;
        for (int i0 = t - 1; i0 >= 0; i0 -= 4) {
            float F[4], R[4];
            uint32_t D[4];
#pragma unroll
            for (int j = 0; j < 4; ++j) {
                const int i = i0 - j;
                F[j] = R[j] = 0.f;
                D[j] = 0u;
                if (i >= 0) {
                    F[j] = svs.load_word<float>(i, WT_VWORD(pdf_bwd));
                    R[j] = svs.load_word<float>(i, WT_VWORD(pdf_fwd));
                    if (i > 0) D[j] = svs.load_word<uint32_t>(i - 1, WT_VWORD(delta));
                }
            }
#pragma unroll
            for (int j = 0; j < 4; ++j) {
                const int i = i0 - j;
                if (i < 0) break;
                const float f = (i == 0 && has_spdf_first) ? spdf_first : F[j];
                const float rv = (i == t - 1 && has_srev_last) ? srev_last : ((i == t - 2 && has_srev_prev) ? srev_prev : R[j]);
                const bool del_prev = i > 0 ? D[j] != 0 : delta_sensor;
                const float fwd = (finitef(f) && f > FLT_EPSILON) ? f : 1.f;
                const float rev = (finitef(rv) && rv > FLT_EPSILON) ? rv : 1.f;
                ri *= rev / fwd;
                if (!del_i && !del_prev) sum_Ri += ri;
                del_i = del_prev;
            }
        }
    }
    ri = 1.f;
    {
        bool del_i = false;
        for (int i0 = s - 1; i0 >= 0; i0 -= 4) {
            float F[4], R[4];
            uint32_t D[4];
#pragma unroll
            for (int j = 0; j < 4; ++j) {
                const int i = i0 - j;
                F[j] = R[j] = 0.f;
                D[j] = 0u;
                if (i >= 0) {
                    F[j] = evs.load_word<float>(i, WT_VWORD(pdf_fwd));
                    R[j] = evs.load_word<float>(i, WT_VWORD(pdf_bwd));
                    if (i > 0) D[j] = evs.load_word<uint32_t>(i - 1, WT_VWORD(delta));
                }
            }
#pragma unroll
            for (int j = 0; j < 4; ++j) {
                const int i = i0 - j;
                if (i < 0) break;
                const float f = (i == 0 && has_epdf_first) ? epdf_first : F[j];
                const float rv = (i == s - 1 && has_erev_last) ? erev_last : ((i == s - 2 && has_erev_prev) ? erev_prev : R[j]);
                const bool del_prev = i > 0 ? D[j] != 0 : delta_emitter;
                const float fwd = (finitef(f) && f > FLT_EPSILON) ? f : 1.f;
                const float rev = (finitef(rv) && rv > FLT_EPSILON) ? rv : 1.f;
                ri *= rev / fwd;
                if (!del_i && !del_prev) sum_Ri += ri;
                del_i = del_prev;
            }
        }
    }
    return 1.f / (1.f + sum_Ri);
}

template <class TV>
WT_HD stokes_t bdpt_strategy_finish(const scene_t& sc, const fsd_pool_t& pool, const film_t& film, const vertex_store_t& svs, const vertex_store_t& evs, int s, int t,
                                    const sample_ctx_t& ctx, const stokes_t& L, const TV& tv, const sensor_element_t& element, bool has_element, bdpt_counters_t* ctr) {
    float mis;
    if (sc.opts.debug_only_s || sc.opts.debug_only_t)
        mis = ctx.recp_spectral_pd;
    else if (sc.opts.MIS)
        mis = bdpt_mis_weight(sc, pool, svs, evs, s, t, tv) * ctx.recp_spectral_pd;
    else
        mis = 1.f / (float(s + t + 1) * ctx.k_density);
    const stokes_t flux = L * mis;
    if (t > 1) return flux;
    if (has_element) {
        film_splat_direct(sc, film, element, flux, ctx.k);
        if (ctr) ctr->light_splats++;
    }
    return stokes_zero();
}
template <bool STAGED = false>
WT_HD stokes_t bdpt_strategy(const scene_t& sc, const fsd_pool_t& pool, const film_t& film, const vertex_store_t& svs, const vertex_store_t& evs, int s,
                             int t, const sample_ctx_t& ctx, uint64_t seed, uint64_t sample_id, const stack_ref_t& stack, bdpt_counters_t* ctr,
                             bvh_counters_t* bctr) {
    connect_ret_t cr;
    bdpt_connect<STAGED>(sc, pool, svs, evs, s, t, seed, sample_id, stack, cr, ctr, bctr);
    if (!(cr.L.s[0] > 0.f)) return stokes_zero();
    if (STAGED) {
        if (cr.need_shadow && ads_shadow_ray(sc, cr.ray.o, cr.ray.d, range_t{0.f, cr.ray.dist}, stack, bctr)) return stokes_zero();
        vertex_nb_t tv;
        sensor_element_t element;
        bool has_element;
        bdpt_connect_temp(sc, svs, evs, s, t, seed, sample_id, tv, element, has_element);
        return bdpt_strategy_finish(sc, pool, film, svs, evs, s, t, ctx, cr.L, tv, element, has_element, ctr);
    }
    return bdpt_strategy_finish(sc, pool, film, svs, evs, s, t, ctx, cr.L, cr.temporary_vert, cr.element, cr.has_element != 0, ctr);
}

template <bool STAGED = false>
WT_HD void bdpt_connect_all(const scene_t& sc, const fsd_pool_t& pool, const film_t& film, const vertex_store_t& svs, const vertex_store_t& evs, int nT,
                            int nS, const sample_ctx_t& ctx, uint64_t seed, uint64_t sample_id, const stack_ref_t& stack, bdpt_counters_t* ctr,
                            bvh_counters_t* bctr) {
    stokes_t L = stokes_zero();
    for (int t = 0; t <= nT; ++t)
        for (int s = 0; s <= nS; ++s) {
            const int depth = t + s - 2;
            if ((t == 1 && s == 1) || depth < 0) continue;
            if (!sc.opts.emitter_direct && s == 1) continue;
            if (!sc.opts.sensor_direct && t == 1) continue;
            if (depth > sc.opts.max_depth) break;
            if (sc.opts.debug_only_s && (int)sc.opts.debug_only_s - 1 != s) continue;
            if (sc.opts.debug_only_t && (int)sc.opts.debug_only_t - 1 != t) continue;
            L = L + bdpt_strategy<STAGED>(sc, pool, film, svs, evs, s, t, ctx, seed, sample_id, stack, ctr, bctr);
        }
#if defined(WTGPU_DEBUG_PRINT) && defined(__HIP_DEVICE_COMPILE__)
    if (ctx.element.x == 0 && ctx.element.y == 0)
        printf("dbg3 L=%g nT=%d nS=%d ch=%u rfs=%g r=%d\n", L.s[0], nT, nS, sc.sensor.channels, sc.sensor.rfilter_sigma, sc.sensor.rf_radius);
#endif
    film_splat(sc, film, ctx.element, L, ctx.k);
}

}
```

wave_tracer_amd/csrc/wtgpu.hip:

```cpp
#include "wtgpu_host.h"

thread_local std::string g_err;

static void note_rounds(wtgpu_scene* s, uint32_t n) { s->rounds_hist[s->rounds_hist_n++ % 8u] = n; }
static int drain_rec(wtgpu_scene* s, chunk_rec_t& r) {
    if (!r.busy) return WTGPU_OK;
    HIP_CHECK(hipEventSynchronize(r.ev[r.ev_final]));
    const uint32_t rounds = r.h_ctl[CTL_ROUNDS];
    s->cap_hits += r.h_ctl[CTL_COUNT0 + (r.rounds_launched & 1u)] + r.h_ctl[CTL_BACK0 + (r.rounds_launched & 1u)];
    s->acc[4] += rounds;
    s->acc[5] += rounds;
    s->acc[6] += 1;
    s->rounds_launched_total += r.rounds_launched;
    if (s->knobs.timing) {
        auto elapsed = [](hipEvent_t a, hipEvent_t b) {
            float ms = 0.f;
            return hipEventElapsedTime(&ms, a, b) == hipSuccess ? ms : 0.f;
        };
        s->acc[0] += elapsed(r.ev[0], r.ev[1]);
        size_t e = 1;
        for (uint32_t k = 0; k < r.rounds_timed; ++k, e += 6) {
            static const int slot[6] = {1, 7, 2, 8, 9, 10};
            for (int q = 0; q < 6; ++q) s->acc[slot[q]] += elapsed(r.ev[e + q], r.ev[e + q + 1]);
        }
        s->acc[3] += elapsed(r.ev[e], r.ev[r.ev_final]);
    }
    r.busy = false;
    return WTGPU_OK;
}

struct batch_launcher_t {
    wtgpu_scene* s;
    const wtgpu_scene::knobs_t& K;
    uint32_t grid_round = 0, grid_heavy = 0;
    bool path_mode = false;
    bool ev_fail = false;
    static constexpr int kHpSlots = 64;
    bool hp_on = false, trace_on = false;
    double hp_t[kHpSlots] = {0};
    unsigned long hp_n[kHpSlots] = {0};
    static const char** hp_labels() {
        static const char* labels[kHpSlots] = {nullptr};
        return labels;
    }
    static int hp_slot(const char* label) {
        static std::mutex m;
        std::lock_guard<std::mutex> l(m);
        const char** labels = hp_labels();
        int i = 0;
        while (i < kHpSlots - 1 && labels[i] && std::strcmp(labels[i], label) != 0) ++i;
        if (!labels[i]) labels[i] = label;
        return i;
    }
    explicit batch_launcher_t(wtgpu_scene* s_) : s(s_), K(s_->knobs) {
        int n_cu = 256;
        (void)hipDeviceGetAttribute(&n_cu, hipDeviceAttributeMultiprocessorCount, s->device);
        grid_round = (uint32_t)n_cu * K.round_blocks_per_cu;
        grid_heavy = (uint32_t)n_cu * K.heavy_waves_per_cu;
        path_mode = s->host.opts.integrator != INTEGRATOR_BDPT;
        hp_on = K.host_prof != 0;
        trace_on = K.trace_launch != 0;
    }
#define HP_LAUNCH(kernel, ...)                                                                                            \
    do {                                                                                                                  \
        if (trace_on) {    \
            fprintf(stderr, "[wtgpu launch] %s ...", #kernel);                                                            \
            hipLaunchKernelGGL(kernel, __VA_ARGS__);                                                                      \
            const hipError_t e_ = hipDeviceSynchronize();                                                                 \
            fprintf(stderr, " done (%s)\n", hipGetErrorString(e_));                                                       \
        } else if (hp_on) {                                                                                                      \
            static const int slot_ = hp_slot(#kernel);                                                                    \
            const auto t0_ = std::chrono::steady_clock::now();                                                            \
            hipLaunchKernelGGL(kernel, __VA_ARGS__);                                                                      \
            hp_t[slot_] += std::chrono::duration<double, std::micro>(std::chrono::steady_clock::now() - t0_).count();     \
            hp_n[slot_]++;                                                                                                \
        } else                                                                                                            \
            hipLaunchKernelGGL(kernel, __VA_ARGS__);                                                                      \
    } while (0)
    void rec(chunk_rec_t& r, hipStream_t st_) {
        const auto hp0_ = std::chrono::steady_clock::now();
        if (s->knobs.timing && r.ev_used + 1 >= r.ev.size()) return;
        if (s->knobs.timing && hipEventRecord(r.ev[r.ev_used++], st_) != hipSuccess) ev_fail = true;
        if (hp_on) { static const int slot_ = hp_slot("hipEventRecord"); hp_t[slot_] += std::chrono::duration<double, std::micro>(std::chrono::steady_clock::now() - hp0_).count(); hp_n[slot_]++; }
    }
    uint32_t g_full(uint32_t nb) const { return std::min<uint32_t>(grid_round, ((path_mode ? 1u : 2u) * nb + kBlock - 1) / kBlock); }
    void generate(const launch_args_t& a, chunk_rec_t& r, hipStream_t st_) {
        r.ev_used = 0;
        r.rounds_launched = 0;
        r.rounds_timed = 0;
        rec(r, st_);
        if (path_mode)
            HP_LAUNCH(k_path_generate, dim3((a.nb + kBlock - 1) / kBlock), dim3(kBlock), 0, st_, a);
        else
            HP_LAUNCH(k_generate, dim3((a.nb + kBlock - 1) / kBlock), dim3(kBlock), 0, st_, a);
        rec(r, st_);
    }
    int rounds(const launch_args_t& a, const path_state_t* ps, chunk_rec_t& r, hipStream_t st_, uint32_t r_begin, uint32_t r_end, int stage_from = 0) {
        const uint32_t nb = a.nb, walks_per_sample = path_mode ? 1u : 2u, gf = g_full(nb);
        const uint32_t grid_div_b = K.grid_div_b, grid_div_c = K.grid_div_c, grid_mul_flux = K.grid_mul_flux;
        const int dbg_stage = (int)K.dbg_stage;
        for (uint32_t round = r_begin; round < r_end; ++round) {
            const int in = (int)(round & 1u), first = round == 0 ? 1 : 0;
            if (s->knobs.timing && r.ev_used + 7 < r.ev.size()) r.rounds_timed++;
            if (round == K.stagger_round && K.stagger_round > 0) {
                HIP_CHECK(hipEventRecord(r.ev_stagger, st_));
                s->ev_stagger_last = r.ev_stagger;
            }
            uint32_t g0, gh;
            if (K.decay_q > 0) {
                const double f = std::min(1.0, (double)K.decay_c * std::pow(K.decay_q * .01, (double)round));
                g0 = std::max<uint32_t>(2u, (uint32_t)(gf * f));
                gh = std::max<uint32_t>(2u, (uint32_t)(std::min<uint32_t>(grid_heavy, walks_per_sample * nb) * f));
            } else {
                const uint32_t shrink = round < K.shrink_r1 ? 1u : (round < K.shrink_r2 ? K.shrink_f1 : K.shrink_f2);
                g0 = std::max<uint32_t>(1u, gf / shrink);
                gh = std::max<uint32_t>(1u, std::min<uint32_t>(grid_heavy, walks_per_sample * nb) / (round < K.shrink_r1 ? 1u : (round < K.shrink_r2 ? K.shrink_h1 : 32u)));
            }
            const int sf = round == r_begin ? stage_from : 0;
            if (sf <= 0 && dbg_stage >= 2 + 3 * (int)round) {
                if (round < K.trace_ab) {
                    const int rc = trace_ab_round(s, a, st_, in, first, round, g0);
                    if (rc) return rc;
                } else if (K.trace_sm || (K.trace_staged && round < K.trace_staged_rounds))
                    launch_trace_alt(s, a, st_, in, first, round, g0);
                else
                    HP_LAUNCH(k_trace_refill, dim3(g0), dim3(kBlock), 0, st_, a, in, first, round);
            }
            rec(r, st_);
            if (sf <= 1 && dbg_stage >= 3 + 3 * (int)round) HP_LAUNCH(k_trace_heavy, dim3(gh), dim3(64), 0, st_, a);
            rec(r, st_);
            if (path_mode) {
                if (round > 0) HP_LAUNCH(k_path_fsd, dim3(gh), dim3(64), 0, st_, a, ps, round);
                if (dbg_stage >= 4 + 3 * (int)round) HP_LAUNCH(k_path_interact, dim3(g0), dim3(kBlock), 0, st_, a, ps, in, first, round);
                HP_LAUNCH(k_path_edges, dim3(gh), dim3(64), 0, st_, a, ps);
                HP_LAUNCH(k_path_interact_b, dim3(std::max<uint32_t>(1u, g0 / 2u)), dim3(kBlock), 0, st_, a, ps, in, round);
                HP_LAUNCH(k_path_nee, dim3(gh), dim3(64), 0, st_, a, ps, round);
                rec(r, st_);
                rec(r, st_);
                rec(r, st_);
                rec(r, st_);
                continue;
            }
            if (sf > 2) {
            } else if (K.sorted_interact) {
                HP_LAUNCH(k_classify, dim3(g0), dim3(kBlock), 0, st_, a, in, first);
                if (K.sorted_interact >= 2)
                    HP_LAUNCH(k_interact_sorted, dim3(g0), dim3(kBlock), 0, st_, a, in);
                else {
                HP_LAUNCH(k_interact_diffuse, dim3(std::max<uint32_t>(1u, g0 / K.grid_div_cls[0])), dim3(kBlock), 0, st_, a, in);
                HP_LAUNCH(k_interact_dielectric, dim3(std::max<uint32_t>(1u, g0 / K.grid_div_cls[1])), dim3(kBlock), 0, st_, a, in);
                HP_LAUNCH(k_interact_spm, dim3(std::max<uint32_t>(1u, g0 / K.grid_div_cls[2])), dim3(kBlock), 0, st_, a, in);
                HP_LAUNCH(k_interact_any, dim3(std::max<uint32_t>(1u, g0 / K.grid_div_cls[3])), dim3(kBlock), 0, st_, a, in);
                }
            } else if (K.coop_io)
                HP_LAUNCH(k_interact_coop, dim3(g0), dim3(kBlock), 0, st_, a, in, first);
            else
                HP_LAUNCH(k_interact, dim3(g0), dim3(kBlock), 0, st_, a, in, first);
            rec(r, st_);
            if (sf <= 3) HP_LAUNCH(k_edges, dim3(gh), dim3(64), 0, st_, a);
            if (sf <= 4) HP_LAUNCH(k_interact_b, dim3(std::max<uint32_t>(1u, g0 / grid_div_b)), dim3(kBlock), 0, st_, a, in);
            rec(r, st_);
            HP_LAUNCH(k_flux_split, dim3(std::max<uint32_t>(1u, gh / 4u)), dim3(64), 0, st_, a);
            HP_LAUNCH(k_flux_tasks, dim3(std::max<uint32_t>(1u, gh * grid_mul_flux)), dim3(64), 0, st_, a);
            rec(r, st_);
            HP_LAUNCH(k_interact_c, dim3(std::max<uint32_t>(1u, gh / grid_div_c)), dim3(64), 0, st_, a, in);
            HP_LAUNCH(k_interact_c_hard, dim3(std::max<uint32_t>(1u, gh / K.grid_div_hard)), dim3(WTGPU_HARD_BLOCK), 0, st_, a, in);
            rec(r, st_);
        }
        r.rounds_launched = r_end;
        return WTGPU_OK;
    }
    void light(const launch_args_t& a, hipStream_t st_, uint32_t launched) {
        if (path_mode || !K.light_rounds || launched >= K.max_rounds) return;
        HP_LAUNCH(k_light_rounds, dim3(1), dim3(kBlock), 0, st_, a, (int)(launched & 1u), launched, K.max_rounds - launched);
    }
    int tail(const launch_args_t& a, chunk_rec_t& r, hipStream_t st_) {
        const uint32_t nb = a.nb, gf = g_full(nb);
        if (path_mode) {
            HP_LAUNCH(k_path_flush, dim3(kFlushGrid), dim3(kBlock), 0, st_, a, (int)(r.rounds_launched & 1u));
        } else {
            HP_LAUNCH(k_connect_enum, dim3((nb + kEnumBlock - 1) / kEnumBlock), dim3(kEnumBlock), 0, st_, a);
            HP_LAUNCH(k_connect_scan, dim3(1), dim3(64), 0, st_, a);
            const bool open = (uint32_t)s->host.opts.max_depth + 2 >= kKeyDim - 1;
            if (K.staged_connect && !open) {
                for (uint32_t c = 0; c < s->n_chunks; ++c) {
                    const uint32_t g = c == 0 ? gf : std::max<uint32_t>(1u, gf / 8u);
                    HP_LAUNCH(k_connect_eval, dim3(g), dim3(kBlock), 0, st_, a, c);
                    HP_LAUNCH(k_connect_shadow, dim3(g), dim3(kBlock), 0, st_, a, c);
                    HP_LAUNCH(k_connect_mis, dim3(g), dim3(kBlock), 0, st_, a, c);
                }
            } else {
                HP_LAUNCH(k_connect_strat, dim3(gf), dim3(kBlock), 0, st_, a);
                if (open) HP_LAUNCH(k_connect_strat_open, dim3(std::max<uint32_t>(1u, gf / 8u)), dim3(kBlock), 0, st_, a);
            }
            const uint32_t fw = a.film.width, fh = a.film.height, planes = film_planes(s->host.sensor);
            if (K.tiled_splat && s->host.sensor.rf_radius <= 1 && planes <= 16 && (uint64_t)nb * 2u >= (uint64_t)a.npix)
                HP_LAUNCH(k_connect_splat_tiled, dim3(fh * ((fw + kBlock - 1) / kBlock)), dim3(kBlock), 3 * kSplatCols * (planes + 1) * sizeof(double), st_, a);
            else
                HP_LAUNCH(k_connect_splat, dim3((nb + kBlock - 1) / kBlock), dim3(kBlock), 0, st_, a);
        }
        HIP_CHECK(hipGetLastError());
        HIP_CHECK(hipMemcpyAsync(r.h_ctl, a.st.ctl, CTL_WORDS * sizeof(uint32_t), hipMemcpyDeviceToHost, st_));
        r.ev_final = s->knobs.timing ? r.ev_used : 0;
        HIP_CHECK(hipEventRecord(r.ev[r.ev_final], st_));
        if (ev_fail) return fail(WTGPU_ERR_HIP, "hipEventRecord failed");
        r.busy = true;
        return WTGPU_OK;
    }
#undef HP_LAUNCH
    void report() const {
        if (!hp_on) return;
        const char* const* labels = hp_labels();
        for (int i = 0; i < kHpSlots; ++i)
            if (hp_n[i]) fprintf(stderr, "[host prof] %-22s %6lu calls %9.1f us total %7.2f us each\n", labels[i], hp_n[i], hp_t[i], hp_t[i] / hp_n[i]);
    }
};
static_assert(sizeof(launch_args_t) <= sizeof(wtgpu_scene::pending_t::args), "pending_t::args holds a launch block");

static uint32_t expected_rounds(const wtgpu_scene* s) {
    if (s->knobs.first_rounds) return s->knobs.first_rounds;
    if (s->rounds_hist_n == 0) return std::min<uint32_t>(kMaxWalkIters, 32u);
    const uint32_t n = std::min<uint32_t>(s->rounds_hist_n, 8u);
    uint32_t sum = 0;
    for (uint32_t i = 0; i < n; ++i) sum += s->rounds_hist[i];
    const uint32_t mean = (sum + n - 1) / n;
    return std::min<uint32_t>(kMaxWalkIters, mean + s->knobs.rounds_margin);
}
static int finish_look(wtgpu_scene* s, size_t k, batch_launcher_t& L) {
    wtgpu_scene::pending_t& p = s->pending[k];
    chunk_rec_t& r = *p.rec;
    launch_args_t a;
    std::memcpy(&a, p.args, sizeof(a));
    hipStream_t st_ = s->streams[k];
    uint32_t& launched = p.launched;
    const bool light = !L.path_mode && s->knobs.light_rounds != 0;
    uint32_t stop = 0;
    if (light && launched < s->knobs.max_rounds) {
        launched += r.h_mid[CTL_LIGHT_DONE];
        stop = r.h_mid[CTL_LIGHT_STOP];
        s->light_rounds_run += r.h_mid[CTL_LIGHT_DONE];
    }
    bool done = false;
    if (s->knobs.tail_diag) {
        static unsigned long long looks = 0, by_stop[8] = {0}, light_done = 0, left_sum = 0;
        static bool reg = false;
        if (!reg) { reg = true; atexit([] { fprintf(stderr, "[tail diag] looks %llu (stop 0/1/2/3/4: %llu %llu %llu %llu %llu), light rounds %llu, walks left at looks (sum) %llu\n", looks, by_stop[0], by_stop[1], by_stop[2], by_stop[3], by_stop[4], light_done, left_sum); }); }
        looks++; by_stop[stop < 8 ? stop : 7]++; light_done += light ? r.h_mid[CTL_LIGHT_DONE] : 0;
        left_sum += r.h_mid[CTL_COUNT0 + (launched & 1u)] + r.h_mid[CTL_BACK0 + (launched & 1u)];
    }
    if (stop >= 1 && stop <= 3) {
        static const int from[4] = {0, 1, 3, 5};
        const int rc = L.rounds(a, s->d_path_slices[k], r, st_, launched, launched + 1, from[stop]);
        if (rc) return rc;
        launched += 1;
    } else {
        const uint32_t q = launched & 1u;
        const uint32_t left = r.h_mid[CTL_COUNT0 + q] + r.h_mid[CTL_BACK0 + q];
        if (left == 0) {
            note_rounds(s, std::min<uint32_t>(r.h_mid[CTL_ROUNDS], kMaxWalkIters));
            done = true;
        } else if (launched >= s->knobs.max_rounds)
            done = true;
        else {
            s->round_fallbacks++;
            const uint32_t next = std::min<uint32_t>(s->knobs.max_rounds, launched + p.rounds_step);
            const int rc = L.rounds(a, s->d_path_slices[k], r, st_, launched, next);
            if (rc) return rc;
            launched = next;
            p.rounds_step = std::min<uint32_t>(64u, p.rounds_step * 2u);
        }
    }
    if (done) {
        p.active = false;
        r.rounds_launched = launched;
        return L.tail(a, r, st_);
    }
    L.light(a, st_, launched);
    HIP_CHECK(hipMemcpyAsync(r.h_mid, a.st.ctl, CTL_WORDS * sizeof(uint32_t), hipMemcpyDeviceToHost, st_));
    HIP_CHECK(hipEventRecord(r.ev_mid, st_));
    return WTGPU_OK;
}
static int serve_pending(wtgpu_scene* s, size_t k, batch_launcher_t& L) {
    const size_t n = s->pending.size();
    for (;;) {
        bool any = false, progressed = false;
        for (size_t j = 0; j < n; ++j) {
            wtgpu_scene::pending_t& p = s->pending[j];
            if (!p.active) continue;
            if (k != (size_t)-1 && !s->pending[k].active) break;
            any = true;
            const hipError_t q = hipEventQuery(p.rec->ev_mid);
            if (q == hipSuccess) {
                const int rc = finish_look(s, j, L);
                if (rc) return rc;
                progressed = true;
            } else if (q != hipErrorNotReady)
                HIP_CHECK(q);
            else
                (void)hipGetLastError();
        }
        if (k != (size_t)-1 ? !s->pending[k].active : !any) return WTGPU_OK;
        if (!progressed) {
            std::this_thread::sleep_for(std::chrono::microseconds(20));
        }
    }
}
static int finish_all_pending(wtgpu_scene* s) {
    bool any = false;
    for (const auto& p : s->pending) any = any || p.active;
    if (!any) return WTGPU_OK;
    batch_launcher_t L(s);
    return serve_pending(s, (size_t)-1, L);
}
int drain_all(wtgpu_scene* s) {
    {
        const int rc = finish_all_pending(s);
        if (rc) return rc;
    }
    for (auto& r : s->recs) {
        const int rc = drain_rec(s, r);
        if (rc) return rc;
    }
    return WTGPU_OK;
}

extern "C" {

const char* wtgpu_last_error(void) { return g_err.c_str(); }

int wtgpu_join(wtgpu_scene* s, void* stream_) {
    if (!s || !s->uploaded) return fail(WTGPU_ERR_INVALID, "scene not uploaded");
    hipStream_t caller = static_cast<hipStream_t>(stream_);
    device_guard_t guard(s->device);
    {
        const int rc = finish_all_pending(s);
        if (rc) return rc;
    }
    for (size_t k = 0; k < s->slices.size(); ++k) {
        HIP_CHECK(hipEventRecord(s->ev_done[k], s->streams[k]));
        HIP_CHECK(hipStreamWaitEvent(caller, s->ev_done[k], 0));
    }
    return WTGPU_OK;
}

int wtgpu_render(wtgpu_scene* s, void* stream_, double* d_value, double* d_weight, double* d_light, uint64_t sb, uint64_t se, uint64_t seed) {
    const int rc = wtgpu_render_async(s, stream_, d_value, d_weight, d_light, sb, se, seed);
    return rc ? rc : wtgpu_join(s, stream_);
}

int wtgpu_render_async(wtgpu_scene* s, void* stream_, double* d_value, double* d_weight, double* d_light, uint64_t sb, uint64_t se, uint64_t seed) {
    if (!s || !s->uploaded) return fail(WTGPU_ERR_INVALID, "scene not uploaded");
    if (!d_value || !d_weight || !d_light || se < sb) return fail(WTGPU_ERR_INVALID, "bad film pointers / sample range");
    hipStream_t caller = static_cast<hipStream_t>(stream_);
    device_guard_t guard(s->device);
    const scene_t& h = s->host;
    const uint64_t npix = (uint64_t)h.sensor.width * h.sensor.height;
    const uint64_t total = npix * (se - sb);
    if (total == 0) return WTGPU_OK;
    launch_args_t a;
    static_assert(sizeof(launch_args_t) <= 984, "by-value kernel arguments beyond 1 KB serialise the streams (see path_state_t)");
    a.sc = s->dev;
    a.film = film_t{d_value, d_weight, d_light, h.sensor.width, h.sensor.height, h.sensor.channels};
    a.seed = seed;
    a.npix = (uint32_t)npix;
    a.sample_begin = sb;
    const wtgpu_scene::knobs_t& K = s->knobs;
    a.count_stats = K.count_stats;
    a.cone_budget = K.cone_budget;
    a.profile = K.profile;
    a.coop_aperture_min = K.coop_aperture_min;
    a.heavy_probe = K.heavy_probe;
    a.split_queues = K.split_queues;
    a.lane_cache = K.lane_cache;
    a.heavy_cache = K.heavy_cache;
    a.flux_task_tris = K.flux_task_tris;
    a.collect_list = ((h.opts.integrator != INTEGRATOR_BDPT || !K.no_lists) ? 1u : 0u) | ((h.opts.integrator == INTEGRATOR_BDPT && K.primary_axis) ? 2u : 0u);
    batch_launcher_t L(s);

    HIP_CHECK(hipEventRecord(s->ev_begin, caller));
    const size_t n_slices = s->slices.size();
    std::vector<char> used(n_slices, 0);
    const uint64_t cap = s->slices[0].cap;
    for (uint64_t j0 = 0; j0 < total; j0 += cap) {
        const size_t k = s->slice_next++ % n_slices;
        hipStream_t st_ = s->streams[k];
        {
            const int rc = s->pending[k].active ? serve_pending(s, k, L) : WTGPU_OK;
            if (rc) return rc;
        }
        if (!used[k]) {
            HIP_CHECK(hipStreamWaitEvent(st_, s->ev_begin, 0));
            used[k] = 1;
        }
        chunk_rec_t& r = s->recs[s->rec_next];
        s->rec_next = (s->rec_next + 1) % s->recs.size();
        int rc = drain_rec(s, r);
        if (rc) return rc;
        const uint32_t nb = (uint32_t)std::min<uint64_t>(cap, total - j0);
        if (K.stagger_round > 0 && s->ev_stagger_last && n_slices > 1) HIP_CHECK(hipStreamWaitEvent(st_, s->ev_stagger_last, 0));
        a.st = s->slices[k];
        a.j0 = j0;
        a.nb = nb;
        const uint32_t r1 = expected_rounds(s);
        L.generate(a, r, st_);
        rc = L.rounds(a, s->d_path_slices[k], r, st_, 0, r1);
        if (rc) return rc;
        HIP_CHECK(hipGetLastError());
        L.light(a, st_, r1);
        HIP_CHECK(hipMemcpyAsync(r.h_mid, a.st.ctl, CTL_WORDS * sizeof(uint32_t), hipMemcpyDeviceToHost, st_));
        HIP_CHECK(hipEventRecord(r.ev_mid, st_));
        wtgpu_scene::pending_t& p = s->pending[k];
        std::memcpy(p.args, &a, sizeof(a));
        p.rec = &r;
        p.launched = r1;
        p.rounds_step = 8;
        p.active = true;

    }
    L.report();
    s->samples_rendered += total;
    return WTGPU_OK;
}

int wtgpu_last_render_timings(wtgpu_scene* s, float out[12]) {
    if (!s || !out || !s->uploaded) return fail(WTGPU_ERR_INVALID, "scene not uploaded");
    const int rc = drain_all(s);
    if (rc) return rc;
    for (int i = 0; i < 12; ++i) out[i] = (float)s->acc[i];
    out[11] = s->acc[6] > 0 ? (float)((double)s->rounds_launched_total / s->acc[6]) : (float)kMaxWalkIters;
    return WTGPU_OK;
}

}
```

wave_tracer_amd/csrc/wtgpu_kernels.h:

```cpp
#pragma once
#include <hip/hip_runtime.h>

#include <cstddef>
#include <cstdint>
#include <cstring>

#include "../../include/wtgpu.h"
#include "wt/bdpt.h"
#include "wt/coop.h"
#include "wt/coop_fsd.h"
#include "wt/coop_utd.h"
#include "wt/path.h"

using namespace wt;

namespace wtk {


#ifndef WTGPU_LB_TRACE
#define WTGPU_LB_TRACE 3
#endif
#ifndef WTGPU_LB_HEAVY
#define WTGPU_LB_HEAVY 2
#endif
#ifndef WTGPU_LB_INTERACT
#define WTGPU_LB_INTERACT 3
#endif
#ifndef WTGPU_LB_INTERACT_B
#define WTGPU_LB_INTERACT_B 3
#endif
#ifndef WTGPU_LB_INTERACT_C
#define WTGPU_LB_INTERACT_C 3
#endif
#ifndef WTGPU_LB_FLUX
#define WTGPU_LB_FLUX 3
#endif
#ifndef WTGPU_LB_CONNECT
#define WTGPU_LB_CONNECT 2
#endif
constexpr uint32_t kFluxTaskTris = 2048;
constexpr int kBlock = 128;
#ifndef WTGPU_LDS_STACK
#define WTGPU_LDS_STACK 20
#endif
constexpr int kLdsStack = WTGPU_LDS_STACK;
constexpr uint32_t kConeBudget = 96;
constexpr int kSpillStack = 64 - kLdsStack;

enum : uint32_t { CTL_STRAT_HEAD_OPEN = 25, CTL_UTD_COUNT0 = 26, CTL_UTD_COUNT1 = 27, CTL_FSDQ_COUNT0 = 28, CTL_FSDQ_COUNT1 = 29, CTL_FSDQ_HEAD = 30, CTL_NEEQ_COUNT = 31, CTL_NEEQ_HEAD = 32, CTL_COUNT0 = 0, CTL_COUNT1 = 1, CTL_HEAD_TRACE = 2, CTL_HEAD_INTERACT = 3, CTL_HEAVY_COUNT = 4, CTL_HEAVY_HEAD = 5, CTL_FSD_COUNTER = 6,
                  CTL_ROUNDS = 7, CTL_STRAT_HEAD = 8, CTL_INTB_COUNT = 9, CTL_INTB_HEAD = 10, CTL_GATHER_COUNT = 11, CTL_GATHER_HEAD = 12, CTL_INTC_COUNT = 13, CTL_INTC_HEAD = 14, CTL_FTASK_COUNT = 15, CTL_FTASK_HEAD = 16, CTL_FSPLIT_HEAD = 17, CTL_EPOOL_COUNT = 18, CTL_FSD_ECOUNTER = 19, CTL_INTD_COUNT = 20, CTL_INTD_HEAD = 21, CTL_BACK0 = 22, CTL_BACK1 = 23,
                  CTL_TPOL_COUNT0 = 41, CTL_TPOL_COUNT1 = 42, CTL_TPOL_HEAD = 43, CTL_TCONE_COUNT0 = 44, CTL_TCONE_COUNT1 = 45, CTL_TCONE_HEAD = 46,
                  CTL_CLS_COUNT0 = 33, CTL_CLS_HEAD0 = 37,
                  CTL_LIGHT_DONE = 47, CTL_LIGHT_STOP = 48,
                  CTL_WORDS = 56 };
constexpr uint32_t kTriListWords = 128;
constexpr uint32_t kGatherMarker = 0xFFFFFFFEu;
constexpr uint32_t kApertureMarker = 0xFFFFFFFDu, kNullApertureMarker = 0xFFFFFFFCu;
__host__ __device__ inline bool is_region_marker(uint32_t t) { return t == kGatherMarker || t == kApertureMarker; }
constexpr uint32_t kKeyDim = kMaxVerts + 2, kNumKeys = kKeyDim * kKeyDim;

struct device_state_t {
    uint64_t cap = 0;
    uint32_t max_verts = 0;
    uint32_t walk_words = 0;
    size_t vert_words = 0;
    uint32_t* walks = nullptr;
    uint32_t* verts = nullptr;
    uint32_t* ctx = nullptr;
    uint32_t* trav = nullptr;
    uint32_t* tris = nullptr;
    uint32_t* queue[2] = {nullptr, nullptr};
    uint32_t* heavy_queue = nullptr;
    uint32_t* intb_queue = nullptr;
    uint32_t* gather_queue = nullptr;
    uint32_t* intc_queue = nullptr;
    uint32_t* intd_queue = nullptr;
    uint2* ftasks = nullptr;
    uint32_t ftask_cap = 0;
    double* facc = nullptr;
    uint32_t* epool = nullptr;
    uint32_t epool_cap = 0;
    uint32_t* ctl = nullptr;
    fsd_aperture_t* fsd_hdr = nullptr;
    fsd_edge_t* fsd_edges = nullptr;
    uint32_t fsd_cap = 0;
    uint32_t fsd_ecap = 0;
    uint32_t* strat_items = nullptr;
    uint32_t* strat_count = nullptr;
    uint32_t* strat_prefix = nullptr;
    double* lacc = nullptr;
    unsigned long long* counters = nullptr;
    const struct bdpt_ext_t* ext = nullptr;
};
struct bdpt_ext_t {
    const unsigned char* tri_class = nullptr;
    uint32_t* cls_queue = nullptr;
    struct conn_pending_t* pend = nullptr;
    uint32_t* surv = nullptr;
    uint32_t* chunk_ctl = nullptr;
    uint32_t pend_cap = 0, n_chunks = 0;
};
enum : uint32_t { CHUNK_EVAL_HEAD = 0, CHUNK_PEND_COUNT = 1, CHUNK_PEND_HEAD = 2, CHUNK_SURV_COUNT = 3, CHUNK_MIS_HEAD = 4, kChunkCtlWords = 8 };
struct conn_pending_t {
    uint32_t i;
    uint32_t st;
    float L[4];
    float o[3], d[3], dist;
};
struct path_state_t {
    utd_edge_rec_t* utd[2] = {nullptr, nullptr};
    uint32_t utd_cap = 0;
    uint32_t* fsdq[2] = {nullptr, nullptr};
    uint32_t* neeq = nullptr;
    float* fsd_f = nullptr;
    path_nee_rec_t* nee_recs = nullptr;
    uint2* gather_info = nullptr;
};
constexpr size_t kWalkWords = sizeof(walk_t) / 4;
constexpr size_t kCtxWords = sizeof(sample_ctx_t) / 4;
constexpr size_t kTravWords = sizeof(trav_result_t) / 4;
#define WT_TRAV_WORD(field) (offsetof(trav_result_t, field) / 4)
struct trace_stage_t {
    cone_t env;
    axis_walk_t aw;
};
constexpr size_t kStageWords = sizeof(trace_stage_t) / 4;
constexpr size_t kNumCounters = sizeof(bdpt_counters_t) / sizeof(unsigned long long);
constexpr size_t kProfSlots = 128;
constexpr size_t kDroppedSlot = kNumCounters + kProfSlots;


struct launch_args_t {
    scene_t sc;
    device_state_t st;
    film_t film;
    uint64_t seed;
    uint64_t j0;
    uint32_t nb;
    uint32_t npix;
    uint64_t sample_begin;
    uint32_t count_stats;
    uint32_t cone_budget;
    uint32_t flux_task_tris;
    uint32_t heavy_probe;
    uint32_t coop_aperture_min;
    uint32_t profile;
    uint32_t split_queues;
    uint32_t lane_cache, heavy_cache;
    uint32_t collect_list;
};

WT_D uint32_t* trace_stage_words(const launch_args_t& a) { return a.st.trav + kTravWords * 2 * (size_t)a.st.cap; }
WT_D uint32_t* trace_pol_queue(const launch_args_t& a) { return a.st.heavy_queue + 2 * (size_t)a.st.cap; }
WT_D uint32_t* trace_cone_queue(const launch_args_t& a) { return a.st.heavy_queue + 4 * (size_t)a.st.cap; }
WT_D void lds_stack(stack_entry_t* lds, stack_entry_t* spill, stack_ref_t& s, uint32_t block = kBlock) {
    s = make_stack_ref(lds + threadIdx.x, block, kLdsStack + kSpillStack, kLdsStack, spill);
}

WT_D void flush_counters(unsigned long long* g, const bdpt_counters_t& c) {
    const unsigned long long* p = reinterpret_cast<const unsigned long long*>(&c);
#pragma unroll
    for (size_t i = 0; i < kNumCounters; ++i) {
        unsigned long long v = p[i];
        for (int off = 32; off > 0; off >>= 1) v += __shfl_down(v, off, 64);
        if ((threadIdx.x & 63) == 0 && v) atomicAdd(&g[i], v);
    }
}

WT_D void walk_ident(const launch_args_t& a, uint32_t w, uint32_t& i, uint32_t& stream) {
    if (w < a.st.cap) {
        i = w;
        stream = STREAM_SENSOR_WALK;
    } else {
        i = w - (uint32_t)a.st.cap;
        stream = STREAM_EMITTER_WALK;
    }
}
WT_D uint32_t queue_count(const uint32_t* ctl, int in) { return ctl[CTL_COUNT0 + in] + ctl[CTL_BACK0 + in]; }
WT_D uint32_t queue_walk(const launch_args_t& a, const uint32_t* ctl, int in, uint32_t qi, int first_round) {
    if (first_round) return qi < a.nb ? qi : (uint32_t)a.st.cap + (qi - a.nb);
    const uint32_t front = ctl[CTL_COUNT0 + in];
    return qi < front ? a.st.queue[in][qi] : a.st.queue[in][2 * (size_t)a.st.cap - 1 - (qi - front)];
}
WT_D bool wave_first_lane() { return __builtin_amdgcn_mbcnt_hi(~0u, __builtin_amdgcn_mbcnt_lo(~0u, 0u)) == 0u; }
WT_D uint32_t wave_grab0(uint32_t* head, uint32_t inc) {
    __builtin_amdgcn_wave_barrier();
    uint32_t old = 0;
    if (wave_first_lane()) old = atomicAdd(head, inc);
    __builtin_amdgcn_wave_barrier();
    return (uint32_t)__builtin_amdgcn_readfirstlane((int)old);
}
WT_D uint32_t wave_grab(uint32_t* head) { return wave_grab0(head, 64u); }
WT_D uint32_t wave_grab_item(uint32_t* head) { return wave_grab0(head, 1u); }
WT_D uint32_t wave_bcast0(uint32_t v) {
    __builtin_amdgcn_wave_barrier();
    return (uint32_t)__builtin_amdgcn_readfirstlane((int)v);
}
WT_D void wave_append(uint32_t* queue, uint32_t* count, bool pred, uint32_t w) {
    const unsigned long long m = __ballot(pred);
    if (!m) return;
    const int lane = threadIdx.x & 63;
    const int leader = __ffsll((long long)m) - 1;
    uint32_t base = 0;
    if (lane == leader) base = atomicAdd(count, (uint32_t)__popcll(m));
    base = (uint32_t)__shfl((int)base, leader, 64);
    if (pred) queue[base + (uint32_t)__popcll(m & ((1ull << lane) - 1ull))] = w;
}

WT_D void queue_append(const launch_args_t& a, uint32_t* ctl, int out, bool pred, uint32_t w) {
    const bool back = pred && w >= a.st.cap && a.split_queues;
    wave_append(a.st.queue[out], ctl + CTL_COUNT0 + out, pred && !back, w);
    const unsigned long long m = __ballot(back);
    if (!m) return;
    const int lane = threadIdx.x & 63;
    const int leader = __ffsll((long long)m) - 1;
    uint32_t base = 0;
    if (lane == leader) base = atomicAdd(ctl + CTL_BACK0 + out, (uint32_t)__popcll(m));
    base = (uint32_t)__shfl((int)base, leader, 64);
    if (back) a.st.queue[out][2 * (size_t)a.st.cap - 1 - (base + (uint32_t)__popcll(m & ((1ull << lane) - 1ull)))] = w;
}

constexpr int kIoRows = 32;
template <int W>
constexpr int io_pitch() { return (W & 1) ? W : W + 1; }
template <int W, class T>
WT_D void wave_load_records(const uint32_t* base, size_t stride, uint32_t idx, bool valid, uint32_t* lds, T& out) {
    static_assert(sizeof(T) == 4 * W, "record size");
    constexpr int P = io_pitch<W>();
    const int lane = threadIdx.x & 63;
    uint32_t* o = reinterpret_cast<uint32_t*>(&out);
    const unsigned long long all = __ballot(valid);
#pragma unroll 1
    for (int h = 0; h < 2; ++h) {
        unsigned long long m = all & (h ? 0xFFFFFFFF00000000ull : 0x00000000FFFFFFFFull);
        while (m) {
            const int r = __ffsll((long long)m) - 1;
            m &= m - 1;
            const uint32_t* src = base + (size_t)__builtin_amdgcn_readlane(idx, r) * stride;
#pragma unroll
            for (int w0 = 0; w0 < W; w0 += 64)
                if (w0 + lane < W) lds[(r & 31) * P + w0 + lane] = src[w0 + lane];
        }
        __builtin_amdgcn_wave_barrier();
        if (valid && (lane >> 5) == h) {
#pragma unroll
            for (int i = 0; i < W; ++i) o[i] = lds[(lane & 31) * P + i];
        }
        __builtin_amdgcn_wave_barrier();
    }
}
template <int W, class T>
WT_D void wave_store_records(uint32_t* base, size_t stride, uint32_t idx, uint32_t off, bool valid, uint32_t* lds, const T& in) {
    static_assert(sizeof(T) == 4 * W, "record size");
    constexpr int P = io_pitch<W>();
    const int lane = threadIdx.x & 63;
    const uint32_t* o = reinterpret_cast<const uint32_t*>(&in);
    const unsigned long long all = __ballot(valid);
    if (!all) return;
#pragma unroll 1
    for (int h = 0; h < 2; ++h) {
        if (valid && (lane >> 5) == h) {
#pragma unroll
            for (int i = 0; i < W; ++i) lds[(lane & 31) * P + i] = o[i];
        }
        __builtin_amdgcn_wave_barrier();
        unsigned long long m = all & (h ? 0xFFFFFFFF00000000ull : 0x00000000FFFFFFFFull);
        while (m) {
            const int r = __ffsll((long long)m) - 1;
            m &= m - 1;
            uint32_t* dst = base + (size_t)__builtin_amdgcn_readlane(idx, r) * stride + __builtin_amdgcn_readlane(off, r);
#pragma unroll
            for (int w0 = 0; w0 < W; w0 += 64)
                if (w0 + lane < W) dst[w0 + lane] = lds[(r & 31) * P + w0 + lane];
        }
        __builtin_amdgcn_wave_barrier();
    }
}

constexpr uint32_t kFlushGrid = 64;
constexpr int kEnumBlock = 1024;
constexpr uint32_t kSplatCols = kBlock + 2;
#ifndef WTGPU_HARD_BLOCK
#define WTGPU_HARD_BLOCK 256
#endif
__global__ void k_generate(launch_args_t a);
__global__ void k_trace_refill(launch_args_t a, int in, int first_round, uint32_t round);
__global__ void k_trace_sm(launch_args_t a, int in, int first_round, uint32_t round);
__global__ void k_tr_axis(launch_args_t a, int in, int first_round, uint32_t round);
__global__ void k_tr_cone(launch_args_t a, uint32_t it);
__global__ void k_tr_policy(launch_args_t a, uint32_t it);
__global__ void k_tr_tail(launch_args_t a, uint32_t it);
__global__ void k_trace_heavy(launch_args_t a);
__global__ void k_interact(launch_args_t a, int in, int first_round);
__global__ void k_classify(launch_args_t a, int in, int first_round);
__global__ void k_interact_diffuse(launch_args_t a, int in);
__global__ void k_interact_dielectric(launch_args_t a, int in);
__global__ void k_interact_spm(launch_args_t a, int in);
__global__ void k_interact_any(launch_args_t a, int in);
__global__ void k_interact_sorted(launch_args_t a, int in);
__global__ void k_interact_coop(launch_args_t a, int in, int first_round);
__global__ void k_edges(launch_args_t a);
__global__ void k_interact_b(launch_args_t a, int in);
__global__ void k_light_rounds(launch_args_t a, int in, uint32_t round, uint32_t max_rounds);
__global__ void k_flux_split(launch_args_t a);
__global__ void k_flux_tasks(launch_args_t a);
__global__ void k_interact_c(launch_args_t a, int in);
__global__ void k_interact_c_hard(launch_args_t a, int in);
__global__ void k_path_generate(launch_args_t a);
__global__ void k_path_fsd(launch_args_t a, const path_state_t* __restrict__ ps, uint32_t round);
__global__ void k_path_edges(launch_args_t a, const path_state_t* __restrict__ ps);
__global__ void k_path_interact(launch_args_t a, const path_state_t* __restrict__ ps, int in, int first_round, uint32_t round);
__global__ void k_path_interact_b(launch_args_t a, const path_state_t* __restrict__ ps, int in, uint32_t round);
__global__ void k_path_nee(launch_args_t a, const path_state_t* __restrict__ ps, uint32_t round);
__global__ void k_path_flush(launch_args_t a, int in);
__global__ void k_connect_enum(launch_args_t a);
__global__ void k_connect_scan(launch_args_t a);
__global__ void k_connect_strat(launch_args_t a);
__global__ void k_connect_strat_open(launch_args_t a);
__global__ void k_connect_eval(launch_args_t a, uint32_t chunk);
__global__ void k_connect_shadow(launch_args_t a, uint32_t chunk);
__global__ void k_connect_mis(launch_args_t a, uint32_t chunk);
__global__ void k_connect_splat(launch_args_t a);
__global__ void k_connect_splat_tiled(launch_args_t a);
__global__ void k_calib_copy(const uint32_t* in, uint32_t* out, size_t n);
__global__ void k_trace_rays(scene_t sc, const float* rays, uint32_t n, float* dist, uint32_t* tuid, float* bary, uint32_t* front);
__global__ void k_traverse_cones(scene_t sc, const float* cones, uint32_t n, uint32_t cap, float* dist, uint32_t* flags, uint32_t* ntris, uint32_t* out_tris,
                                 uint32_t* scratch_tris);
__global__ void k_query_regions(scene_t sc, const float* cones, uint32_t n, uint32_t edge_cap, float* dist, uint32_t* flags, uint32_t* primary, uint32_t* ntris,
                                uint32_t* nedges, uint32_t* edges, float* flux, unsigned long long* dropped);
int test_fsd_apertures(const scene_t& sc, hipStream_t stream, const float* d_cones, const float* d_sk, const uint32_t* d_ids, const uint32_t* d_n_ids,
                       uint32_t n, uint32_t id_cap, uint32_t pool_cap, uint32_t mode, uint32_t* d_hdr, float* d_segs);
int test_utd_sums(const scene_t& sc, hipStream_t stream, const float* d_queries, const uint32_t* d_ids, const uint32_t* d_n_ids, uint32_t n, uint32_t id_cap,
                  uint32_t utd_cap, uint32_t* d_recs, uint32_t* d_hdr, uint32_t* d_edges);
int test_bsdf_queries(const scene_t& sc, hipStream_t stream, const uint32_t* d_queries, uint32_t n, int form, uint32_t* d_out);
int sensor_mask_launch(const scene_t& sc, hipStream_t stream, const uint8_t* d_shape_matches, uint32_t samples, uint64_t seed, float* d_out);
void sensor_mask_host(const scene_t& sc, const uint8_t* shape_matches, uint32_t samples, uint64_t seed, uint32_t n_threads, float* out);

}
using namespace wtk;
```

wave_tracer_amd/csrc/wtgpu_knobs.h:

```cpp
#pragma once
#include <cstddef>
#include <cstdint>

struct knobs_t {
    uint32_t cone_budget, count_stats, split_queues, lane_cache, heavy_cache, heavy_probe, coop_aperture_min, flux_task_tris, profile, no_lists, primary_axis;
    uint32_t streams, state_gb, timing, conn_pool;
    uint32_t first_rounds, rounds_margin, light_rounds, max_rounds, stagger_round;
    uint32_t shrink_r1, shrink_f1, shrink_r2, shrink_f2, shrink_h1, decay_q, decay_c;
    uint32_t heavy_waves_per_cu, round_blocks_per_cu, grid_div_b, grid_div_c, grid_div_hard, grid_mul_flux;
    uint32_t sorted_interact, coop_io, staged_connect, tiled_splat;
    uint32_t trace_staged, trace_stages, trace_staged_rounds, trace_sm, trace_ab;
    uint32_t dbg_stage;
    uint32_t host_prof, trace_launch, tail_diag, trace_ab_verbose;
    uint32_t grid_div_cls[4];
};

enum knob_kind_t {
    KNOB_U32,
    KNOB_INT,
    KNOB_NONZERO,
    KNOB_PRESENT
};
struct knob_t {
    const char* name;
    uint32_t knobs_t::*field;
    knob_kind_t kind;
    long long dflt, lo, hi;
    const char* help;
};
#pragma GCC visibility push(hidden)
extern const knob_t kKnobs[];
extern const size_t kNumKnobs;
constexpr uint32_t kKnobConeBudget = 96, kKnobFluxTaskTris = 2048;

void read_knobs(knobs_t& k);
#pragma GCC visibility pop
```

wave_tracer_amd/csrc/wtgpu_knobs.hip:

```cpp
#include "wtgpu_knobs.h"

#include <algorithm>
#include <climits>
#include <cstdio>
#include <cstdlib>

#include "wt/bdpt.h"

using wt::kMaxWalkIters;
using wt::kWalkIterLimit;

#define K(field) &knobs_t::field
static constexpr long long kU32 = 0xFFFFFFFFll;
const knob_t kKnobs[] = {
    {"WTGPU_CONE_BUDGET", K(cone_budget), KNOB_U32, kKnobConeBudget, 0, kU32, "work units one lane may spend on a cone query before it is handed to a wavefront (wtgpu_kernels.h: kConeBudget)"},
    {"WTGPU_COUNT_STATS", K(count_stats), KNOB_U32, 1, 0, kU32, "0: the kernels keep no statistics (wtgpu_kernels.h: launch_args_t::count_stats)"},
    {"WTGPU_SPLIT_QUEUES", K(split_queues), KNOB_U32, 1, 0, kU32, "round queues keep sensor and emitter walks apart; 0: one mixed queue (A/B)"},
    {"WTGPU_LANE_CACHE", K(lane_cache), KNOB_U32, 1, 0, kU32, "0 (diagnostic): the per-lane traversal without its remembered rejecting triangles"},
    {"WTGPU_HEAVY_CACHE", K(heavy_cache), KNOB_U32, 1, 0, kU32, "0 (diagnostic): the wave-cooperative traversal without its remembered rejecting triangles"},
    {"WTGPU_HEAVY_PROBE", K(heavy_probe), KNOB_U32, 1, 0, kU32, "k_trace_heavy: any-hit probe of the near slab before the handed-over cone query too; 0: off"},
    {"WTGPU_COOP_APERTURE_MIN", K(coop_aperture_min), KNOB_U32, 8, 0, kU32, "segments from which an aperture is built by a wavefront; 0xFFFFFFFF: every aperture by a single lane of pass B"},
    {"WTGPU_FLUX_TASK_TRIS", K(flux_task_tris), KNOB_U32, kKnobFluxTaskTris, 64, kU32, "triangles per region-sum task (k_flux_split / k_flux_tasks; wtgpu_kernels.h: kFluxTaskTris)"},
    {"WTGPU_PROFILE", K(profile), KNOB_U32, 0, 0, kU32, "1 / 2 / 3: in-kernel clock breakdowns, printed by wtgpu_get_counters (wtgpu_counters.hip)"},
    {"WTGPU_NO_LISTS", K(no_lists), KNOB_PRESENT, 0, 0, 1, "set (any value; plt_bdpt, diagnostic): no bounded triangle lists, every interaction region is gathered"},
    {"WTGPU_PRIMARY_AXIS", K(primary_axis), KNOB_U32, 0, 0, kU32, "1 (plt_bdpt): the triangle under the beam axis of every diffusive hit comes from the trace kernels' axis query"},
    {"WTGPU_STREAMS", K(streams), KNOB_INT, 3, 1, INT_MAX, "state slices = internal streams; ms per pass at 1 / 2 / 3 / 4 / 6 / 8: 158 / 142 / 130 / 142 / 157 / 206 (headline)"},
    {"WTGPU_STATE_GB", K(state_gb), KNOB_INT, 224, 1, INT_MAX, "budget of the per-batch state of all slices, GB (of the MI355X's 288; never more than 85 % of what is free): deep scenes get smaller batches"},
    {"WTGPU_TIMING", K(timing), KNOB_NONZERO, 1, 0, 1, "0: no per-kernel HIP events (wtgpu_last_render_timings reads zeros)"},
    {"WTGPU_CONN_POOL", K(conn_pool), KNOB_U32, 16, 1, kU32, "staged connections: pending connections per sample of a chunk"},
    {"WTGPU_FIRST_ROUNDS", K(first_rounds), KNOB_U32, 0, 0, kMaxWalkIters, "rounds launched up front; 0: adaptive (the recent batches' mean + WTGPU_ROUNDS_MARGIN); tests use 2, 96 = as before round 4"},
    {"WTGPU_ROUNDS_MARGIN", K(rounds_margin), KNOB_U32, 2, 0, kU32, "rounds added to the recent batches' mean"},
    {"WTGPU_LIGHT_ROUNDS", K(light_rounds), KNOB_U32, 1, 0, kU32, "0: the rounds beyond the expected ones as ordinary rounds only (k_light_rounds off)"},
    {"WTGPU_MAX_ROUNDS", K(max_rounds), KNOB_U32, kWalkIterLimit, 8, kWalkIterLimit, "rounds a batch may get before its surviving walks are dropped and counted (CHANGES RESULTS below the default, wt/bdpt.h kWalkIterLimit: nothing is dropped in any workload seen; 96 = rounds 1-5)"},
    {"WTGPU_STAGGER_ROUND", K(stagger_round), KNOB_U32, 0, 0, kMaxWalkIters - 1, "r > 0 (diagnostic): a batch starts when the previous one has finished its round r; 0: all streams start at once.  4 streams, r = 0 / 3 / 6 / 10 / 16: 151 / 150 / 161 / 200 / 263 ms per pass"},
    {"WTGPU_SHRINK_R1", K(shrink_r1), KNOB_U32, 8, 0, kU32, "from this round on the round kernels' grids are divided by WTGPU_SHRINK_F1 (heavy: WTGPU_SHRINK_H1)"},
    {"WTGPU_SHRINK_F1", K(shrink_f1), KNOB_U32, 4, 1, kU32, "see WTGPU_SHRINK_R1"},
    {"WTGPU_SHRINK_R2", K(shrink_r2), KNOB_U32, 16, 0, kU32, "from this round on the grids are divided by WTGPU_SHRINK_F2 (heavy: 32)"},
    {"WTGPU_SHRINK_F2", K(shrink_f2), KNOB_U32, 32, 1, kU32, "see WTGPU_SHRINK_R2"},
    {"WTGPU_SHRINK_H1", K(shrink_h1), KNOB_U32, 4, 1, kU32, "see WTGPU_SHRINK_R1"},
    {"WTGPU_DECAY_Q", K(decay_q), KNOB_U32, 0, 0, kU32, "per cent; > 0: grids follow WTGPU_DECAY_C x q^round instead of the step schedule above"},
    {"WTGPU_DECAY_C", K(decay_c), KNOB_U32, 4, 1, kU32, "safety factor of the geometric schedule"},
    {"WTGPU_HEAVY_WAVES", K(heavy_waves_per_cu), KNOB_U32, 8, 1, kU32, "wavefronts per CU of the wave-per-item kernels; swept 6 / 8 / 10 / 12 / 16 / 24 / 32: 169.6 / 168.0 / 171.6 / 174.3 / 176 / 181 / 183 ms per pass"},
    {"WTGPU_ROUND_BLOCKS", K(round_blocks_per_cu), KNOB_U32, 8, 1, kU32, "blocks per CU of the round kernels' persistent grids"},
    {"WTGPU_GRID_B", K(grid_div_b), KNOB_U32, 4, 1, kU32, "pass B's grid relative to the round's (divisor)"},
    {"WTGPU_GRID_C", K(grid_div_c), KNOB_U32, 1, 1, kU32, "pass C's grid (divisor); 2 until round 4; 1: bidir_room 33.6 -> 33.9, cornell 25.15 -> 25.35 Msamples/s, pass C's bracket 69 -> 56 / 93 -> 65 ms"},
    {"WTGPU_GRID_HARD", K(grid_div_hard), KNOB_U32, 4, 1, kU32, "k_interact_c_hard's grid (divisor)"},
    {"WTGPU_GRID_FLUX", K(grid_mul_flux), KNOB_U32, 2, 1, kU32, "k_flux_tasks' grid (multiplier)"},
    {"WTGPU_SORTED_INTERACT", K(sorted_interact), KNOB_U32, 0, 0, kU32, "pass A: 0 k_interact (one kernel, every walk); 1 k_classify + one kernel per material class; 2 k_classify + k_interact_sorted"},
    {"WTGPU_COOP_IO", K(coop_io), KNOB_U32, 0, 0, kU32, "1: pass A with wave-cooperative record transfers (k_interact_coop)"},
    {"WTGPU_STAGED_CONNECT", K(staged_connect), KNOB_U32, 0, 0, kU32, "connections: 0 k_connect_strat (one kernel per strategy item); 1 k_connect_eval -> k_connect_shadow -> k_connect_mis, in chunks"},
    {"WTGPU_TILED_SPLAT", K(tiled_splat), KNOB_U32, 1, 0, kU32, "0: the plain per-sample splat kernel"},
    {"WTGPU_TRACE_STAGED", K(trace_staged), KNOB_U32, 1, 0, kU32, "1: the traversal in stages (k_tr_axis / k_tr_cone / k_tr_policy / k_tr_tail) ..."},
    {"WTGPU_TRACE_STAGES", K(trace_stages), KNOB_U32, 3, 1, 16, "... with this many cone stages before the tail ..."},
    {"WTGPU_TRACE_STAGED_ROUNDS", K(trace_staged_rounds), KNOB_U32, 4, 0, kU32, "... for the first so many rounds of a batch (the long ones: a stage is a launch, and a short round is bound by its launches)"},
    {"WTGPU_TRACE_SM", K(trace_sm), KNOB_U32, 0, 0, kU32, "1: the phase-machine trace kernel (k_trace_sm)"},
    {"WTGPU_TRACE_AB", K(trace_ab), KNOB_U32, 0, 0, kU32, "n: the first n rounds replay their trace queue through both trace kernels, timed, outputs compared (wtgpu_trace_ab.hip)"},
    {"WTGPU_DEBUG_STAGE", K(dbg_stage), KNOB_INT, 1 << 30, INT_MIN, INT_MAX, "bring-up aid: stops launching the round kernels after stage n (INVALID RESULTS)"},
    {"WTGPU_HOST_PROF", K(host_prof), KNOB_PRESENT, 0, 0, 1, "set: host time spent inside each kind of launch call, printed per render call"},
    {"WTGPU_TRACE_LAUNCH", K(trace_launch), KNOB_PRESENT, 0, 0, 1, "set (bring-up aid): every launch is named and waited for — the last line names a kernel that hangs"},
    {"WTGPU_TAIL_DIAG", K(tail_diag), KNOB_PRESENT, 0, 0, 1, "set: why the host was called back for a pending batch, printed at exit (DESIGN.md §9)"},
    {"WTGPU_TRACE_AB_VERBOSE", K(trace_ab_verbose), KNOB_PRESENT, 0, 0, 1, "set: one line per round replayed by WTGPU_TRACE_AB"},
};
#undef K
const size_t kNumKnobs = sizeof(kKnobs) / sizeof(kKnobs[0]);

void read_knobs(knobs_t& k) {
    for (size_t i = 0; i < kNumKnobs; ++i) {
        const knob_t& d = kKnobs[i];
        const char* e = getenv(d.name);
        long long v = d.dflt;
        if (d.kind == KNOB_PRESENT) v = e ? 1 : 0;
        else if (e && d.kind == KNOB_U32) v = std::min<long long>(std::max<long long>(0, strtoll(e, nullptr, 10)), kU32);
        else if (e && d.kind == KNOB_INT) v = atoi(e);
        else if (e) v = atoi(e) != 0;
        k.*d.field = (uint32_t)std::min(d.hi, std::max(d.lo, v));
    }
    unsigned v[4] = {1, 4, 2, 4};
    if (const char* e = getenv("WTGPU_GRID_CLS")) sscanf(e, "%u,%u,%u,%u", &v[0], &v[1], &v[2], &v[3]);
    for (int c = 0; c < 4; ++c) k.grid_div_cls[c] = std::max(1u, v[c]);
}
```

wave_tracer_amd/csrc/wtgpu_upload.hip:

```cpp
#include "wtgpu_host.h"

static int g_env_by_host = 0;
__attribute__((constructor)) static void wtgpu_runtime_settings() {
    if (getenv("HSA_KERNARG_POOL_SIZE")) g_env_by_host |= 1;
    setenv("HSA_KERNARG_POOL_SIZE", "16777216", 0);
}
static int runtime_settings_ok(std::string& why) {
    const char* k = getenv("HSA_KERNARG_POOL_SIZE");
    const long ring = k ? atol(k) : (1l << 20);
    if (getenv("WTGPU_ALLOW_SLOW_RUNTIME")) return 1;
    if (ring < (4l << 20)) {
        why = "HSA_KERNARG_POOL_SIZE=" + std::string(k ? k : "(unset)") + ": a batch enqueues ~900 launches of ~1 KB of kernel arguments; with a ring below 4 MiB the enqueueing "
              "thread blocks and the streams serialise; export HSA_KERNARG_POOL_SIZE=16777216 before the HIP runtime initialises, or WTGPU_ALLOW_SLOW_RUNTIME=1";
        return 0;
    }
    if (!(g_env_by_host & 1) && !getenv("WTGPU_QUIET")) {
        static bool told = false;
        if (!told) fprintf(stderr, "[wtgpu] note: HSA_KERNARG_POOL_SIZE=16777216 defaulted by libwtgpu.so; effective only if the HIP runtime had not initialised before the library was loaded "
                           "(a host that uses HIP earlier exports it itself, INTEGRATION.md)\n");
        told = true;
    }
    return 1;
}

static int upload_scene_arrays(wtgpu_scene* s) {
    const scene_t& h = s->host;
    scene_t d = h;
    int rc;
#define UP(field, n) \
    if ((rc = upload(s, h.field, (size_t)(n), &d.field)) != WTGPU_OK) return rc;
    {
        d.tri_geo = nullptr;
        if (h.n_tris > 0 && h.tri_geo) {
            const size_t nt = h.n_tris;
            std::vector<float> sph(4 * nt);
            for (size_t i = 0; i < nt; ++i) tri_bounding_sphere(h.tri_geo[i].a, h.tri_geo[i].b, h.tri_geo[i].c, &sph[4 * i]);
            void* p = nullptr;
            HIP_CHECK(hipMalloc(&p, nt * (sizeof(tri_geo_t) + 16)));
            s->dev_allocs.push_back(p);
            HIP_CHECK(hipMemcpy(p, h.tri_geo, nt * sizeof(tri_geo_t), hipMemcpyHostToDevice));
            HIP_CHECK(hipMemcpy(static_cast<char*>(p) + nt * sizeof(tri_geo_t), sph.data(), nt * 16, hipMemcpyHostToDevice));
            d.tri_geo = static_cast<const tri_geo_t*>(p);
        }
    }
    UP(tri_meta, h.n_tris)
    UP(tri_shade, h.n_tris)
    UP(edges, h.n_edges)
    {
        d.nodes = nullptr;
        if (h.n_nodes > 0 && h.nodes) {
            const size_t nn = h.n_nodes;
            vec3 mn{WT_INF, WT_INF, WT_INF}, mx{-WT_INF, -WT_INF, -WT_INF};
            for (size_t i = 0; i < nn; ++i)
                for (int c = 0; c < 8; ++c)
                    if (h.nodes[i].child[c] != 0) {
                        mn = vmin(mn, vec3{h.nodes[i].minx[c], h.nodes[i].miny[c], h.nodes[i].minz[c]});
                        mx = vmax(mx, vec3{h.nodes[i].maxx[c], h.nodes[i].maxy[c], h.nodes[i].maxz[c]});
                    }
            const qgrid_t g = qgrid_make(mn, mx);
            std::vector<bvh8_qnode_t> qn(nn);
            bool ok = finitef(mn.x) && finitef(mn.y) && finitef(mn.z) && finitef(mx.x) && finitef(mx.y) && finitef(mx.z);
            for (size_t i = 0; i < nn && ok; ++i) ok = qnode_make(h.nodes[i], g, qn[i]);
            if (!ok) return fail(WTGPU_ERR_INVALID, "the scene's BVH boxes cannot be enclosed by the 16-bit node grid (non-finite or out-of-range box)");
            const float gw[8] = {g.origin.x, g.origin.y, g.origin.z, g.cell.x, g.cell.y, g.cell.z, 0.f, 0.f};
            void* p = nullptr;
            HIP_CHECK(hipMalloc(&p, nn * (sizeof(bvh8_node_t) + sizeof(bvh8_qnode_t)) + sizeof(gw)));
            s->dev_allocs.push_back(p);
            HIP_CHECK(hipMemcpy(p, h.nodes, nn * sizeof(bvh8_node_t), hipMemcpyHostToDevice));
            HIP_CHECK(hipMemcpy(static_cast<char*>(p) + nn * sizeof(bvh8_node_t), qn.data(), nn * sizeof(bvh8_qnode_t), hipMemcpyHostToDevice));
            HIP_CHECK(hipMemcpy(static_cast<char*>(p) + nn * (sizeof(bvh8_node_t) + sizeof(bvh8_qnode_t)), gw, sizeof(gw), hipMemcpyHostToDevice));
            d.nodes = static_cast<const bvh8_node_t*>(p);
        }
    }
    UP(leaves, h.n_leaves)
    UP(shapes, h.n_shapes)
    const scene_extents_t ex = scene_extents(h);
    UP(shape_tri_tuid, ex.shape_tris)
    UP(shape_tri_cdf, ex.shape_tris + h.n_shapes)
    UP(materials, h.n_materials)
    UP(spectra, h.n_spectra)
    UP(spectra_data, ex.spec_words)
    UP(textures, h.n_textures)
    for (uint32_t i = 0; i < h.n_emitters; ++i)
        if (h.emitters[i].type == EMIT_AREA && h.emitters[i].radiance_tex > 0) {
            const emitter_t& e = h.emitters[i];
            if ((uint32_t)e.radiance_tex > h.n_textures || h.textures[e.radiance_tex - 1].type != TEX_BITMAP || e.shape < 0 || (uint32_t)e.shape >= h.n_shapes ||
                e.tab_words < h.shapes[e.shape].tri_count * 5ull + 1)
                return fail(WTGPU_ERR_INVALID, "area emitter " + std::to_string(i) + ": radiance_tex must name a bitmap texture and tab / tab_words the emitter's sampling tables (wt/sources.h area_table_*)");
        }
    UP(texture_data, ex.tex_words)
    UP(emitters, h.n_emitters)
    UP(emitter_cdf, h.n_emitters + 1)
    UP(kdists, h.n_emitters)
    UP(kdist_data, ex.kd_words)
    if ((rc = upload(s, h.lut.icdf_theta1, h.lut.m ? h.lut.n_theta : 0, &d.lut.icdf_theta1)) != WTGPU_OK) return rc;
    if ((rc = upload(s, h.lut.icdf_theta2, h.lut.m ? h.lut.n_theta : 0, &d.lut.icdf_theta2)) != WTGPU_OK) return rc;
    if ((rc = upload(s, h.lut.icdf1, (size_t)h.lut.m * h.lut.m, &d.lut.icdf1)) != WTGPU_OK) return rc;
    if ((rc = upload(s, h.lut.icdf2, (size_t)h.lut.m * h.lut.m, &d.lut.icdf2)) != WTGPU_OK) return rc;
#undef UP
    s->dev = d;
    s->d_tri_class = nullptr;
    if (h.n_tris > 0 && h.opts.integrator == INTEGRATOR_BDPT) {
        std::vector<unsigned char> cls(h.n_tris);
        for (uint32_t t = 0; t < h.n_tris; ++t) cls[t] = (unsigned char)walk_class_of_triangle(h, t);
        if ((rc = upload(s, cls.data(), cls.size(), &s->d_tri_class)) != WTGPU_OK) return rc;
    }
    return WTGPU_OK;
}

static int alloc_slice(wtgpu_scene* s, uint32_t k, uint64_t batch_cap, unsigned long long* counters) {
    const scene_t& h = s->host;
    int rc;
    device_state_t& st = s->slices[k];
    st.cap = batch_cap;
    st.max_verts = (uint32_t)h.opts.max_depth + 2;
    st.walk_words = (uint32_t)(h.opts.integrator != INTEGRATOR_BDPT ? kPathWalkWords : kWalkWords);
    st.vert_words = (size_t)st.max_verts * kVertexWords;
    st.counters = counters;
    const size_t W2 = 2 * (size_t)st.cap;
    const bool path_mode = h.opts.integrator != INTEGRATOR_BDPT;
    if ((rc = dmalloc(s, &st.walks, (path_mode ? kPathWalkWords : kWalkWords) * W2))) return rc;
    {
        path_state_t P;
        P.utd_cap = path_mode ? (uint32_t)std::min<uint64_t>(48ull * st.cap + 65536, 1ull << 28) : 1u;
        for (int q = 0; q < 2; ++q) {
            if ((rc = dmalloc(s, &P.utd[q], (size_t)P.utd_cap))) return rc;
            if ((rc = dmalloc(s, &P.fsdq[q], path_mode ? (size_t)st.cap : 1))) return rc;
        }
        if ((rc = dmalloc(s, &P.neeq, path_mode ? (size_t)st.cap : 1))) return rc;
        if ((rc = dmalloc(s, &P.fsd_f, path_mode ? (size_t)st.cap : 1))) return rc;
        if ((rc = dmalloc(s, &P.nee_recs, path_mode ? (size_t)st.cap : 1))) return rc;
        if ((rc = dmalloc(s, &P.gather_info, path_mode ? (size_t)st.cap : 1))) return rc;
        path_state_t* dP = nullptr;
        if ((rc = dmalloc(s, &dP, 1))) return rc;
        HIP_CHECK(hipMemcpy(dP, &P, sizeof(P), hipMemcpyHostToDevice));
        s->d_path_slices.push_back(dP);
    }
    if (!path_mode) {
        bdpt_ext_t X;
        X.tri_class = s->d_tri_class;
        if (s->knobs.sorted_interact && (rc = dmalloc(s, &X.cls_queue, (size_t)kNumWalkClasses * W2))) return rc;
        X.pend_cap = (uint32_t)std::min<uint64_t>((uint64_t)s->knobs.conn_pool * st.cap + 4096, 0xFFFFFF00ull);
        if (s->knobs.staged_connect) {
            uint64_t pairs = 0;
            const int md = h.opts.max_depth;
            for (int t = 0; t <= md + 2; ++t)
                for (int q = 0; q <= md + 2; ++q)
                    if (t + q - 2 >= 0 && t + q - 2 <= md && !(t == 1 && q == 1)) ++pairs;
            X.n_chunks = (uint32_t)((pairs * st.cap + X.pend_cap - 1) / X.pend_cap);
            if ((rc = dmalloc(s, &X.pend, (size_t)X.pend_cap))) return rc;
            if ((rc = dmalloc(s, &X.surv, (size_t)X.pend_cap))) return rc;
            if ((rc = dmalloc(s, &X.chunk_ctl, (size_t)X.n_chunks * kChunkCtlWords))) return rc;
        } else
            X.pend_cap = 0;
        s->pend_cap = X.pend_cap;
        s->n_chunks = X.n_chunks;
        bdpt_ext_t* dX = nullptr;
        if ((rc = dmalloc(s, &dX, 1))) return rc;
        HIP_CHECK(hipMemcpy(dX, &X, sizeof(X), hipMemcpyHostToDevice));
        st.ext = dX;
    }
    if ((rc = dmalloc(s, &st.verts, path_mode ? 1 : (size_t)st.max_verts * kVertexWords * W2))) return rc;
    if ((rc = dmalloc(s, &st.ctx, kCtxWords * (size_t)st.cap))) return rc;
    if ((rc = dmalloc(s, &st.trav, (kTravWords + kStageWords) * W2))) return rc;
    if ((rc = dmalloc(s, &st.tris, (size_t)kTriListWords * W2))) return rc;
    if ((rc = dmalloc(s, &st.queue[0], W2))) return rc;
    if ((rc = dmalloc(s, &st.queue[1], W2))) return rc;
    if ((rc = dmalloc(s, &st.heavy_queue, 3 * W2))) return rc;
    if ((rc = dmalloc(s, &st.intb_queue, W2))) return rc;
    if ((rc = dmalloc(s, &st.gather_queue, W2))) return rc;
    if ((rc = dmalloc(s, &st.intc_queue, W2))) return rc;
    if ((rc = dmalloc(s, &st.intd_queue, W2))) return rc;
    st.ftask_cap = path_mode ? 1u : (1u << 22);
    if ((rc = dmalloc(s, &st.ftasks, (size_t)st.ftask_cap))) return rc;
    if ((rc = dmalloc(s, &st.facc, path_mode ? 1 : W2))) return rc;
    st.epool_cap = 1u << 23;
    if ((rc = dmalloc(s, &st.epool, (size_t)st.epool_cap))) return rc;
    if ((rc = dmalloc(s, &st.ctl, (size_t)CTL_WORDS))) return rc;
    HIP_CHECK(hipMemset(st.ctl, 0, CTL_WORDS * sizeof(uint32_t)));
    st.fsd_cap = (h.opts.FSD && !h.opts.force_ray_tracing && !path_mode) ? (uint32_t)std::min<uint64_t>(W2, 1u << 22) : 1u;
    if ((rc = dmalloc(s, &st.fsd_hdr, st.fsd_cap))) return rc;
    st.fsd_ecap = st.fsd_cap > 1 ? (uint32_t)std::min<uint64_t>(64ull * st.cap + kFsdMaxEdges, 1ull << 28) : 1u;
    if ((rc = dmalloc(s, &st.fsd_edges, (size_t)st.fsd_ecap))) return rc;
    if ((rc = dmalloc(s, &st.strat_items, path_mode ? 1 : (size_t)kNumKeys * st.cap))) return rc;
    if ((rc = dmalloc(s, &st.strat_count, (size_t)kNumKeys))) return rc;
    if ((rc = dmalloc(s, &st.strat_prefix, (size_t)kNumKeys + 1))) return rc;
    if ((rc = dmalloc(s, &st.lacc, 4 * (size_t)st.cap))) return rc;
    HIP_CHECK(hipMemset(st.strat_count, 0, kNumKeys * sizeof(uint32_t)));
    HIP_CHECK(hipStreamCreateWithFlags(&s->streams[k], hipStreamNonBlocking));
    HIP_CHECK(hipEventCreateWithFlags(&s->ev_done[k], hipEventDisableTiming));
    return WTGPU_OK;
}

static uint64_t size_batches(const wtgpu_scene* s, uint64_t max_batch, uint32_t& n_slices) {
    const scene_t& h = s->host;
    const uint64_t npix = (uint64_t)h.sensor.width * h.sensor.height;
    n_slices = s->knobs.streams;
    uint64_t batch_cap = max_batch ? std::min<uint64_t>(max_batch, 1u << 24) : std::min<uint64_t>(npix, 1u << 22);
    n_slices = (uint32_t)std::min<uint64_t>(n_slices, std::max<uint64_t>(1, batch_cap / 64));
    {
        const bool pm = h.opts.integrator != INTEGRATOR_BDPT;
        const uint64_t mv = (uint64_t)h.opts.max_depth + 2;
        uint64_t per_sample = 4ull * (2 * ((pm ? kPathWalkWords : kWalkWords) + (pm ? 0 : mv * kVertexWords) + kTravWords + kStageWords + 2 + kTriListWords) + kCtxWords) + 64ull * 28ull + 2048ull;
        if (pm) per_sample += 2ull * 48ull * sizeof(utd_edge_rec_t) + sizeof(path_nee_rec_t) + 3ull * 4ull + 4ull + sizeof(uint2);
        else per_sample += (s->knobs.staged_connect ? (uint64_t)s->knobs.conn_pool * (sizeof(conn_pending_t) + 4ull) : 0ull) + (s->knobs.sorted_interact ? 4ull * 2ull * kNumWalkClasses : 0ull);
        uint64_t budget = (uint64_t)s->knobs.state_gb << 30;
        size_t free_b = 0, total_b = 0;
        if (hipMemGetInfo(&free_b, &total_b) == hipSuccess && free_b > 0) budget = std::min<uint64_t>(budget, (uint64_t)((double)free_b * 0.85));
        const uint64_t fixed = (uint64_t)n_slices * ((1ull << 23) * 4ull + (1ull << 22) * 8ull + (64ull << 20));
        budget = budget > 2 * fixed ? budget - fixed : budget / 2;
        const uint64_t fit = std::max<uint64_t>(4096, budget / per_sample / n_slices);
        if (batch_cap > fit) batch_cap = fit;
    }
    return batch_cap;
}

static int upload_impl(wtgpu_scene* s, uint64_t max_batch) {
    read_knobs(s->knobs);
    int rc;
    if ((rc = upload_scene_arrays(s)) != WTGPU_OK) return rc;
    uint32_t n_slices = 0;
    const uint64_t batch_cap = size_batches(s, max_batch, n_slices);
    unsigned long long* counters = nullptr;
    if ((rc = dmalloc(s, &counters, kNumCounters + kProfSlots + 1))) return rc;
    HIP_CHECK(hipMemset(counters, 0, (kNumCounters + kProfSlots + 1) * sizeof(unsigned long long)));
    s->slices.resize(n_slices);
    s->streams.resize(n_slices);
    s->ev_done.resize(n_slices);
    for (uint32_t k = 0; k < n_slices; ++k)
        if ((rc = alloc_slice(s, k, batch_cap, counters)) != WTGPU_OK) return rc;
    HIP_CHECK(hipEventCreateWithFlags(&s->ev_begin, hipEventDisableTiming));
    s->recs.resize(4 * (size_t)n_slices);
    s->pending.assign(n_slices, wtgpu_scene::pending_t{});
    for (auto& r : s->recs) {
        r.ev.resize(s->knobs.timing ? 3 + 6 * (size_t)kMaxWalkIters : 1);
        for (auto& e : r.ev) HIP_CHECK(hipEventCreate(&e));
        HIP_CHECK(hipHostMalloc((void**)&r.h_ctl, CTL_WORDS * sizeof(uint32_t), hipHostMallocDefault));
        HIP_CHECK(hipHostMalloc((void**)&r.h_mid, CTL_WORDS * sizeof(uint32_t), hipHostMallocDefault));
        HIP_CHECK(hipEventCreateWithFlags(&r.ev_mid, hipEventDisableTiming));
        HIP_CHECK(hipEventCreateWithFlags(&r.ev_stagger, hipEventDisableTiming));
    }
    s->uploaded = true;
    return WTGPU_OK;
}

void release_device(wtgpu_scene* s) {
    if (s->device < 0) return;
    device_guard_t guard(s->device);
    (void)hipDeviceSynchronize();
    for (void* p : s->dev_allocs) (void)hipFree(p);
    s->dev_allocs.clear();
    for (auto& r : s->recs) {
        for (auto& e : r.ev)
            if (e) (void)hipEventDestroy(e);
        if (r.h_ctl) (void)hipHostFree(r.h_ctl);
        if (r.h_mid) (void)hipHostFree(r.h_mid);
        if (r.ev_mid) (void)hipEventDestroy(r.ev_mid);
        if (r.ev_stagger) (void)hipEventDestroy(r.ev_stagger);
    }
    s->recs.clear();
    s->pending.clear();
    for (auto& e : s->ev_done)
        if (e) (void)hipEventDestroy(e);
    s->ev_done.clear();
    s->ev_stagger_last = nullptr;
    if (s->ev_begin) (void)hipEventDestroy(s->ev_begin);
    s->ev_begin = nullptr;
    for (auto& st_ : s->streams)
        if (st_) (void)hipStreamDestroy(st_);
    s->streams.clear();
    s->slices.clear();
    s->d_path_slices.clear();
    s->d_tri_class = nullptr;
    s->pend_cap = s->n_chunks = 0;
    s->d_mask_flags = nullptr;
    if (s->h_mask_flags) (void)hipHostFree(s->h_mask_flags);
    s->h_mask_flags = nullptr;
    if (s->ev_mask) (void)hipEventDestroy(s->ev_mask);
    s->ev_mask = nullptr;
    s->uploaded = false;
}

extern "C" {

int wtgpu_scene_upload(wtgpu_scene* s, int device, uint64_t max_batch) {
    if (!s) return fail(WTGPU_ERR_INVALID, "null scene");
    if (s->uploaded) return fail(WTGPU_ERR_INVALID, "scene already uploaded");
    {
        std::string why;
        if (!runtime_settings_ok(why)) return fail(WTGPU_ERR_INVALID, why);
    }
    int ndev = 0;
    const hipError_t dc = hipGetDeviceCount(&ndev);
    if (dc != hipSuccess || ndev == 0)
        return fail(WTGPU_ERR_NO_DEVICE, std::string("no HIP device present (there is no CPU fallback): hipGetDeviceCount -> ") + hipGetErrorString(dc) +
                                             ", count " + std::to_string(ndev));
    if (device < 0 || device >= ndev) return fail(WTGPU_ERR_NO_DEVICE, "invalid device index");
    device_guard_t guard(device);
    s->device = device;
    const int rc_up = upload_impl(s, max_batch);
    if (rc_up != WTGPU_OK) release_device(s);
    return rc_up;
}

}
```

Baseline: 30.53.

## Add optional visibility-first pass splitting inner connections from edge strategies

Adds an opt-in mode that first traces shadow rays for all inner (s,t>=2) connection strategies in a dedicated kernel and stores the results in a bitmask. An inner kernel without a traversal stack then evaluates only the visible connections, and a separate edge kernel handles the remaining strategies. The aim is to separate divergent BVH traversal from shading/MIS work and cut register/LDS pressure. The MIS code also loads only the few fields of the previous vertices it needs instead of whole vertex records. The new path is disabled by default and adds extra launches plus a bitmask buffer.

```diff
diff --git a/wave_tracer_amd/csrc/kernels_connect.hip b/wave_tracer_amd/csrc/kernels_connect.hip
--- a/wave_tracer_amd/csrc/kernels_connect.hip
+++ b/wave_tracer_amd/csrc/kernels_connect.hip
@@ -72,79 +72,148 @@
         a.st.strat_prefix[kNumKeys] = acc;
         a.st.ctl[CTL_STRAT_HEAD] = 0;
         a.st.ctl[CTL_STRAT_HEAD_OPEN] = 0;
-
-    }
-}
-template <bool OPEN>
-WT_D void connect_strat_body(const launch_args_t& a) {
-    __shared__ stack_entry_t lds[kLdsStack * kBlock];
-    __shared__ uint32_t s_prefix[kNumKeys + 1];
+        a.st.ctl[CTL_STRAT_HEAD_VIS] = a.st.ctl[CTL_STRAT_HEAD_EDGE] = a.st.ctl[CTL_STRAT_HEAD_INNER] = 0;
+    }
+}
+enum strat_mode_e : int { STRAT_ALL = 0, STRAT_OPEN = 1, STRAT_EDGE = 2, STRAT_INNER = 3 };
+template <int MODE>
+WT_D bool strat_mode_takes(uint32_t key) {
     constexpr int K = (int)kKeyDim - 1;
-    if (!OPEN) {
+    const int tk = (int)(key / kKeyDim), sk = (int)(key % kKeyDim);
+    const bool open = tk == K || sk == K;
+    if (MODE == STRAT_OPEN) return open;
+    if (MODE == STRAT_EDGE) return !open && (tk < 2 || sk < 2);
+    if (MODE == STRAT_INNER) return !open && tk >= 2 && sk >= 2;
+    return true;
+}
+template <int MODE>
+WT_D void strat_mode_prefix(const launch_args_t& a, uint32_t* s_prefix) {
+    if (MODE == STRAT_ALL) {
         for (uint32_t k = threadIdx.x; k <= kNumKeys; k += kBlock) s_prefix[k] = a.st.strat_prefix[k];
     } else if (threadIdx.x == 0) {
         uint32_t acc = 0;
         for (uint32_t k = 0; k < kNumKeys; ++k) {
             s_prefix[k] = acc;
-            if ((int)(k / kKeyDim) == K || (int)(k % kKeyDim) == K) acc += a.st.strat_prefix[k + 1] - a.st.strat_prefix[k];
+            if (strat_mode_takes<MODE>(k)) acc += a.st.strat_prefix[k + 1] - a.st.strat_prefix[k];
         }
         s_prefix[kNumKeys] = acc;
     }
     __syncthreads();
+}
+WT_D uint32_t strat_key_of(const uint32_t* s_prefix, uint32_t idx) {
+    uint32_t lo = 0, hi = kNumKeys;
+    while (hi - lo > 1) {
+        const uint32_t mid = (lo + hi) >> 1;
+        if (s_prefix[mid] <= idx)
+            lo = mid;
+        else
+            hi = mid;
+    }
+    return lo;
+}
+template <int MODE>
+WT_D void connect_strat_body(const launch_args_t& a, stack_entry_t* lds) {
+    __shared__ uint32_t s_prefix[kNumKeys + 1];
+    constexpr int K = (int)kKeyDim - 1;
+    constexpr bool OPEN = MODE == STRAT_OPEN;
+    constexpr uint32_t HEAD = MODE == STRAT_OPEN ? CTL_STRAT_HEAD_OPEN : MODE == STRAT_EDGE ? CTL_STRAT_HEAD_EDGE : MODE == STRAT_INNER ? CTL_STRAT_HEAD_INNER : CTL_STRAT_HEAD;
+    strat_mode_prefix<MODE>(a, s_prefix);
     const uint32_t total = s_prefix[kNumKeys];
     bdpt_counters_t ctr;
     memset(&ctr, 0, sizeof(ctr));
+    stack_entry_t spill[MODE == STRAT_INNER ? 1 : kSpillStack];
+    stack_ref_t stack = make_stack_ref(nullptr, 0, 0, 0, nullptr);
+    if (MODE != STRAT_INNER) lds_stack(lds, spill, stack);
+    const fsd_pool_t pool{a.st.fsd_hdr, a.st.fsd_edges, a.st.ctl + CTL_FSD_COUNTER, a.st.fsd_cap, a.st.ctl + CTL_FSD_ECOUNTER, a.st.fsd_ecap};
+    const bool clear = true;
+    for (;;) {
+        const uint32_t idx = wave_grab(a.st.ctl + HEAD) + (threadIdx.x & 63);
+        if (idx - (threadIdx.x & 63) >= total) break;
+        uint64_t vis_word = 0;
+        if (MODE == STRAT_INNER) vis_word = a.st.ext->strat_vis[idx >> 6];
+        if (idx < total) {
+            const uint32_t key = strat_key_of(s_prefix, idx);
+            const int tk = (int)(key / kKeyDim), sk = (int)(key % kKeyDim);
+            if (MODE == STRAT_ALL && (tk == K || sk == K)) continue;
+            if (MODE == STRAT_INNER && !((vis_word >> (idx & 63u)) & 1ull)) {
+                ctr.connections++;
+            } else {
+                const uint32_t i = a.st.strat_items[(size_t)key * a.st.cap + (idx - s_prefix[key])];
+                const uint64_t j = a.j0 + i;
+                const uint32_t pix = (uint32_t)(j % a.npix);
+                const uint64_t smp = a.sample_begin + j / a.npix;
+                const uint64_t sample_id = ((uint64_t)pix << 32) | (smp & 0xFFFFFFFFull);
+                sample_ctx_t ctx;
+                soa_load(a.st.ctx, kCtxWords, i, ctx);
+                const vertex_store_t svs{a.st.verts, a.st.vert_words, i}, evs{a.st.verts, a.st.vert_words, (size_t)a.st.cap + i};
+                auto one = [&](int s, int t) __attribute__((always_inline)) {
+                    if (MODE == STRAT_INNER) __builtin_assume(s >= 2 && t >= 2);
+                    const stokes_t flux = bdpt_strategy(a.sc, pool, a.film, svs, evs, s, t, ctx, a.seed, sample_id, stack, &ctr, nullptr, MODE == STRAT_INNER ? &clear : nullptr);
+                    if (t > 1) {
+#pragma unroll
+                        for (int c = 0; c < 4; ++c)
+                            if (flux.s[c] != 0.f) unsafeAtomicAdd(&a.st.lacc[(size_t)c * a.st.cap + i], (double)flux.s[c]);
+                    }
+                };
+                if constexpr (!OPEN) {
+                    one(sk, tk);
+                } else {
+                    const int nT = (int)a.st.walks[(size_t)i * a.st.walk_words + WT_WALK_NVERTS_WORD];
+                    const int nS = (int)a.st.walks[((size_t)a.st.cap + i) * a.st.walk_words + WT_WALK_NVERTS_WORD];
+                    const int t1 = tk == K ? nT : tk, s1 = sk == K ? nS : sk;
+                    for (int t = tk; t <= t1; ++t)
+                        for (int s = sk; s <= s1; ++s)
+                            if (strategy_valid(a.sc.opts, s, t, nS, nT)) one(s, t);
+                }
+            }
+        }
+    }
+    if (a.count_stats) flush_counters(a.st.counters, ctr);
+}
+__global__ void __launch_bounds__(kBlock, WTGPU_LB_CONNECT) k_connect_strat(launch_args_t a) {
+    __shared__ stack_entry_t lds[kLdsStack * kBlock];
+    connect_strat_body<STRAT_ALL>(a, lds);
+}
+__global__ void __launch_bounds__(kBlock, WTGPU_LB_CONNECT) k_connect_strat_open(launch_args_t a) {
+    __shared__ stack_entry_t lds[kLdsStack * kBlock];
+    connect_strat_body<STRAT_OPEN>(a, lds);
+}
+__global__ void __launch_bounds__(kBlock, WTGPU_LB_CONNECT) k_connect_strat_edge(launch_args_t a) {
+    __shared__ stack_entry_t lds[kLdsStack * kBlock];
+    connect_strat_body<STRAT_EDGE>(a, lds);
+}
+__global__ void __launch_bounds__(kBlock, WTGPU_LB_CONNECT_INNER) k_connect_strat_inner(launch_args_t a) { connect_strat_body<STRAT_INNER>(a, nullptr); }
+
+__global__ void __launch_bounds__(kBlock, 4) k_connect_vis(launch_args_t a) {
+    __shared__ stack_entry_t lds[kLdsStack * kBlock];
+    __shared__ uint32_t s_prefix[kNumKeys + 1];
     stack_entry_t spill[kSpillStack];
     stack_ref_t stack;
     lds_stack(lds, spill, stack);
-    const fsd_pool_t pool{a.st.fsd_hdr, a.st.fsd_edges, a.st.ctl + CTL_FSD_COUNTER, a.st.fsd_cap, a.st.ctl + CTL_FSD_ECOUNTER, a.st.fsd_ecap};
+    strat_mode_prefix<STRAT_INNER>(a, s_prefix);
+    const uint32_t total = s_prefix[kNumKeys];
+    unsigned long long rays = 0;
     for (;;) {
-        const uint32_t idx = wave_grab(a.st.ctl + (OPEN ? CTL_STRAT_HEAD_OPEN : CTL_STRAT_HEAD)) + (threadIdx.x & 63);
+        const uint32_t idx = wave_grab(a.st.ctl + CTL_STRAT_HEAD_VIS) + (threadIdx.x & 63);
         if (idx - (threadIdx.x & 63) >= total) break;
+        bool clear = false;
         if (idx < total) {
-            uint32_t lo = 0, hi = kNumKeys;
-            while (hi - lo > 1) {
-                const uint32_t mid = (lo + hi) >> 1;
-                if (s_prefix[mid] <= idx)
-                    lo = mid;
-                else
-                    hi = mid;
-            }
-            const uint32_t key = lo;
-            const int tk = (int)(key / kKeyDim), sk = (int)(key % kKeyDim);
-            if (!OPEN && (tk == K || sk == K)) continue;
+            const uint32_t key = strat_key_of(s_prefix, idx);
+            const int t = (int)(key / kKeyDim), s = (int)(key % kKeyDim);
             const uint32_t i = a.st.strat_items[(size_t)key * a.st.cap + (idx - s_prefix[key])];
-            const uint64_t j = a.j0 + i;
-            const uint32_t pix = (uint32_t)(j % a.npix);
-            const uint64_t smp = a.sample_begin + j / a.npix;
-            const uint64_t sample_id = ((uint64_t)pix << 32) | (smp & 0xFFFFFFFFull);
-            sample_ctx_t ctx;
-            soa_load(a.st.ctx, kCtxWords, i, ctx);
             const vertex_store_t svs{a.st.verts, a.st.vert_words, i}, evs{a.st.verts, a.st.vert_words, (size_t)a.st.cap + i};
-            auto one = [&](int s, int t) __attribute__((always_inline)) {
-                const stokes_t flux = bdpt_strategy(a.sc, pool, a.film, svs, evs, s, t, ctx, a.seed, sample_id, stack, &ctr, nullptr);
-                if (t > 1) {
-#pragma unroll
-                    for (int c = 0; c < 4; ++c)
-                        if (flux.s[c] != 0.f) unsafeAtomicAdd(&a.st.lacc[(size_t)c * a.st.cap + i], (double)flux.s[c]);
-                }
-            };
-            if constexpr (!OPEN) {
-                one(sk, tk);
-            } else {
-                const int nT = (int)a.st.walks[(size_t)i * a.st.walk_words + WT_WALK_NVERTS_WORD];
-                const int nS = (int)a.st.walks[((size_t)a.st.cap + i) * a.st.walk_words + WT_WALK_NVERTS_WORD];
-                const int t1 = tk == K ? nT : tk, s1 = sk == K ? nS : sk;
-                for (int t = tk; t <= t1; ++t)
-                    for (int s = sk; s <= s1; ++s)
-                        if (strategy_valid(a.sc.opts, s, t, nS, nT)) one(s, t);
-            }
-        }
-    }
-    if (a.count_stats) flush_counters(a.st.counters, ctr);
-}
-__global__ void __launch_bounds__(kBlock, WTGPU_LB_CONNECT) k_connect_strat(launch_args_t a) { connect_strat_body<false>(a); }
-__global__ void __launch_bounds__(kBlock, WTGPU_LB_CONNECT) k_connect_strat_open(launch_args_t a) { connect_strat_body<true>(a); }
+            const uint32_t v = bdpt_connect_visible(a.sc, svs, evs, s, t, stack, nullptr);
+            rays += v != CONN_NO_RAY;
+            clear = v == CONN_CLEAR;
+        }
+        const unsigned long long m = __ballot(clear);
+        if (wave_first_lane()) a.st.ext->strat_vis[idx >> 6] = m;
+    }
+    if (a.count_stats) {
+        for (int off = 32; off > 0; off >>= 1) rays += __shfl_down(rays, off, 64);
+        if ((threadIdx.x & 63) == 0 && rays) atomicAdd(a.st.counters + offsetof(bdpt_counters_t, shadow_rays) / sizeof(unsigned long long), rays);
+    }
+}
 constexpr uint32_t kPendShadow = 0x80000000u;
 WT_D void pending_append(const launch_args_t& a, uint32_t* cctl, bool keep, uint32_t i, int s, int t, const connect_ret_t& cr) {
     const bdpt_ext_t& x = *a.st.ext;
diff --git a/wave_tracer_amd/csrc/wt/bdpt.h b/wave_tracer_amd/csrc/wt/bdpt.h
--- a/wave_tracer_amd/csrc/wt/bdpt.h
+++ b/wave_tracer_amd/csrc/wt/bdpt.h
@@ -1049,8 +1049,9 @@
 
 template <bool DEFER>
 WT_HD stokes_t connect_and_integrate(const scene_t& sc, const beam_t& db, const conn_end_t& dv, const beam_t& eb, const conn_end_t& ev, const stack_ref_t& stack,
-                                     bdpt_counters_t* ctr, bvh_counters_t* bctr, connect_ret_t& ret) {
+                                     bdpt_counters_t* ctr, bvh_counters_t* bctr, connect_ret_t& ret, const bool* vis = nullptr) {
     if (beam_intensity(db) == 0.f || beam_intensity(eb) == 0.f) return stokes_zero();
+    if (vis) return *vis ? integrate_beams(db, eb) : stokes_zero();
     if (ctr) ctr->shadow_rays++;
     const shadow_ray_t ray = conn_shadow_ray(sc, dv, ev);
     if (DEFER) {
@@ -1103,7 +1104,8 @@
 
 template <bool DEFER = false>
 WT_HD void bdpt_connect(const scene_t& sc, const fsd_pool_t& pool, const vertex_store_t& svs, const vertex_store_t& evs, int s, int t,
-                        uint64_t seed, uint64_t sample_id, const stack_ref_t& stack, connect_ret_t& ret, bdpt_counters_t* ctr, bvh_counters_t* bctr) {
+                        uint64_t seed, uint64_t sample_id, const stack_ref_t& stack, connect_ret_t& ret, bdpt_counters_t* ctr, bvh_counters_t* bctr,
+                        const bool* vis = nullptr) {
     ret.L = stokes_zero();
     ret.has_temp = 0;
     ret.has_element = 0;
@@ -1111,7 +1113,7 @@
     sampler_t smp = make_sampler(seed, sample_id, connect_stream(s, t));
     if (ctr) ctr->connections++;
 
-    if (s == 0) {
+    if (!vis && s == 0) {
         vertex_t last;
         svs.load(t - 1, last);
         if (vertex_on_emitter(last)) {
@@ -1119,7 +1121,7 @@
             beam_scale(QE, last.rr_weight);
             ret.L = emitter_Li(sc, vertex_get_emitter(last), QE, last.surf);
         }
-    } else if (t == 0) {
+    } else if (!vis && t == 0) {
         if (sensor_is_virtual(sc.sensor)) {
             vertex_t last;
             evs.load(s - 1, last);
@@ -1142,7 +1144,7 @@
                 ret.L = integrate_beams(dc.beam, beam);
             }
         }
-    } else if (s == 1) {
+    } else if (!vis && s == 1) {
         vertex_t last;
         svs.load(t - 1, last);
         if (vertex_is_connectible(sc, last)) {
@@ -1160,7 +1162,7 @@
                     ret.L = connect_and_integrate<DEFER>(sc, db, conn_end_of(last), ed.beam, conn_end_of(ret.temporary_vert), stack, ctr, bctr, ret);
             }
         }
-    } else if (t == 1) {
+    } else if (!vis && t == 1) {
         vertex_t last;
         evs.load(s - 1, last);
         const bool is_virtual = sensor_is_virtual(sc.sensor);
@@ -1217,10 +1219,24 @@
                 if (ev_on) wsv *= fabsf(dot(ev_ns, d));
                 beam_scale(db, wsv);
                 beam_scale(eb, wev);
-                ret.L = connect_and_integrate<DEFER>(sc, db, sv_end, eb, ev_end, stack, ctr, bctr, ret);
-            }
-        }
-    }
+                ret.L = connect_and_integrate<DEFER>(sc, db, sv_end, eb, ev_end, stack, ctr, bctr, ret, vis);
+            }
+        }
+    }
+}
+enum conn_vis_e : uint32_t { CONN_NO_RAY = 0, CONN_OCCLUDED = 1, CONN_CLEAR = 2 };
+WT_HD conn_end_t vertex_store_conn_end(const vertex_store_t& vs, uint32_t idx) {
+    constexpr size_t ng = (offsetof(vertex_t, surf) + offsetof(surface_t, geo) + offsetof(frame_t, n)) / 4;
+    return conn_end_t{vs.load_wp(idx), vec3{vs.load_word<float>(idx, ng), vs.load_word<float>(idx, ng + 1), vs.load_word<float>(idx, ng + 2)},
+                      vs.load_word<uint32_t>(idx, WT_VWORD(geo_kind)), vs.load_word<uint32_t>(idx, (offsetof(vertex_t, surf) + offsetof(surface_t, tuid)) / 4)};
+}
+WT_HD uint32_t bdpt_connect_visible(const scene_t& sc, const vertex_store_t& svs, const vertex_store_t& evs, int s, int t, const stack_ref_t& stack,
+                                    bvh_counters_t* bctr) {
+    const conn_end_t ev_end = vertex_store_conn_end(evs, s - 1), sv_end = vertex_store_conn_end(svs, t - 1);
+    const vec3 dl = ev_end.wp - sv_end.wp;
+    if (!vertex_store_connectible(sc, evs, s - 1) || !vertex_store_connectible(sc, svs, t - 1) || (dl.x == 0.f && dl.y == 0.f && dl.z == 0.f)) return CONN_NO_RAY;
+    const shadow_ray_t ray = conn_shadow_ray(sc, sv_end, ev_end);
+    return ads_shadow_ray(sc, ray.o, ray.d, range_t{0.f, ray.dist}, stack, bctr) ? CONN_OCCLUDED : CONN_CLEAR;
 }
 WT_HD void bdpt_connect_temp(const scene_t& sc, const vertex_store_t& svs, const vertex_store_t& evs, int s, int t, uint64_t seed, uint64_t sample_id, vertex_nb_t& tv,
                              sensor_element_t& element, bool& has_element) {
@@ -1255,6 +1271,28 @@
     }
     if (has_temp) __builtin_memcpy(&tv, &tmp, offsetof(vertex_t, beam));
     tv.beam.k = 0.f;
+}
+
+struct vertex_next_t {
+    uint32_t type;
+    int32_t ref;
+    uint32_t geo_kind;
+    struct {
+        vec3 wp;
+        struct {
+            vec3 n;
+        } geo;
+    } surf;
+};
+WT_HD vertex_next_t vertex_store_next(const vertex_store_t& vs, uint32_t idx, vec3 wp) {
+    constexpr size_t ng = (offsetof(vertex_t, surf) + offsetof(surface_t, geo) + offsetof(frame_t, n)) / 4;
+    vertex_next_t v;
+    v.type = vs.load_word<uint32_t>(idx, WT_VWORD(type));
+    v.ref = vs.load_word<int32_t>(idx, WT_VWORD(ref));
+    v.geo_kind = vs.load_word<uint32_t>(idx, WT_VWORD(geo_kind));
+    v.surf.wp = wp;
+    v.surf.geo.n = vec3{vs.load_word<float>(idx, ng), vs.load_word<float>(idx, ng + 1), vs.load_word<float>(idx, ng + 2)};
+    return v;
 }
 
 template <class TV>
@@ -1300,9 +1338,7 @@
         evs.load(s - 1, ev);
         svs.load(t - 1, sv);
         const vec3 ev_prev_wp = evs.load_wp(s - 2), sv_prev_wp = svs.load_wp(t - 2);
-        vertex_nb_t ev_prev, sv_prev;
-        evs.load(s - 2, ev_prev);
-        svs.load(t - 2, sv_prev);
+        const vertex_next_t ev_prev = vertex_store_next(evs, s - 2, ev_prev_wp), sv_prev = vertex_store_next(svs, t - 2, sv_prev_wp);
         erev_last = vertex_pdf(sc, pool, sv, sv_prev_wp, ev, TRANSPORT_BACKWARD);
         erev_prev = vertex_pdf(sc, pool, ev, vertex_wp(sv), ev_prev, TRANSPORT_BACKWARD);
         srev_last = vertex_pdf(sc, pool, ev, ev_prev_wp, sv, TRANSPORT_FORWARD);
@@ -1418,9 +1454,9 @@
 template <bool STAGED = false>
 WT_HD stokes_t bdpt_strategy(const scene_t& sc, const fsd_pool_t& pool, const film_t& film, const vertex_store_t& svs, const vertex_store_t& evs, int s,
                              int t, const sample_ctx_t& ctx, uint64_t seed, uint64_t sample_id, const stack_ref_t& stack, bdpt_counters_t* ctr,
-                             bvh_counters_t* bctr) {
+                             bvh_counters_t* bctr, const bool* vis = nullptr) {
     connect_ret_t cr;
-    bdpt_connect<STAGED>(sc, pool, svs, evs, s, t, seed, sample_id, stack, cr, ctr, bctr);
+    bdpt_connect<STAGED>(sc, pool, svs, evs, s, t, seed, sample_id, stack, cr, ctr, bctr, vis);
     if (!(cr.L.s[0] > 0.f)) return stokes_zero();
     if (STAGED) {
         if (cr.need_shadow && ads_shadow_ray(sc, cr.ray.o, cr.ray.d, range_t{0.f, cr.ray.dist}, stack, bctr)) return stokes_zero();
diff --git a/wave_tracer_amd/csrc/wtgpu.hip b/wave_tracer_amd/csrc/wtgpu.hip
--- a/wave_tracer_amd/csrc/wtgpu.hip
+++ b/wave_tracer_amd/csrc/wtgpu.hip
@@ -190,7 +190,12 @@
                     HP_LAUNCH(k_connect_mis, dim3(g), dim3(kBlock), 0, st_, a, c);
                 }
             } else {
-                HP_LAUNCH(k_connect_strat, dim3(gf), dim3(kBlock), 0, st_, a);
+                if (K.connect_vis) {
+                    HP_LAUNCH(k_connect_vis, dim3(gf), dim3(kBlock), 0, st_, a);
+                    HP_LAUNCH(k_connect_strat_inner, dim3(gf), dim3(kBlock), 0, st_, a);
+                    HP_LAUNCH(k_connect_strat_edge, dim3(gf), dim3(kBlock), 0, st_, a);
+                } else
+                    HP_LAUNCH(k_connect_strat, dim3(gf), dim3(kBlock), 0, st_, a);
                 if (open) HP_LAUNCH(k_connect_strat_open, dim3(std::max<uint32_t>(1u, gf / 8u)), dim3(kBlock), 0, st_, a);
             }
             const uint32_t fw = a.film.width, fh = a.film.height, planes = film_planes(s->host.sensor);
diff --git a/wave_tracer_amd/csrc/wtgpu_kernels.h b/wave_tracer_amd/csrc/wtgpu_kernels.h
--- a/wave_tracer_amd/csrc/wtgpu_kernels.h
+++ b/wave_tracer_amd/csrc/wtgpu_kernels.h
@@ -38,6 +38,9 @@
 #ifndef WTGPU_LB_CONNECT
 #define WTGPU_LB_CONNECT 2
 #endif
+#ifndef WTGPU_LB_CONNECT_INNER
+#define WTGPU_LB_CONNECT_INNER 2
+#endif
 constexpr uint32_t kFluxTaskTris = 2048;
 constexpr int kBlock = 128;
 #ifndef WTGPU_LDS_STACK
@@ -51,6 +54,7 @@
                   CTL_ROUNDS = 7, CTL_STRAT_HEAD = 8, CTL_INTB_COUNT = 9, CTL_INTB_HEAD = 10, CTL_GATHER_COUNT = 11, CTL_GATHER_HEAD = 12, CTL_INTC_COUNT = 13, CTL_INTC_HEAD = 14, CTL_FTASK_COUNT = 15, CTL_FTASK_HEAD = 16, CTL_FSPLIT_HEAD = 17, CTL_EPOOL_COUNT = 18, CTL_FSD_ECOUNTER = 19, CTL_INTD_COUNT = 20, CTL_INTD_HEAD = 21, CTL_BACK0 = 22, CTL_BACK1 = 23,
                   CTL_TPOL_COUNT0 = 41, CTL_TPOL_COUNT1 = 42, CTL_TPOL_HEAD = 43, CTL_TCONE_COUNT0 = 44, CTL_TCONE_COUNT1 = 45, CTL_TCONE_HEAD = 46,
                   CTL_CLS_COUNT0 = 33, CTL_CLS_HEAD0 = 37,
+                  CTL_STRAT_HEAD_VIS = 49, CTL_STRAT_HEAD_EDGE = 50, CTL_STRAT_HEAD_INNER = 51,
                   CTL_LIGHT_DONE = 47, CTL_LIGHT_STOP = 48,
                   CTL_WORDS = 56 };
 constexpr uint32_t kTriListWords = 128;
@@ -99,6 +103,7 @@
     uint32_t* surv = nullptr;
     uint32_t* chunk_ctl = nullptr;
     uint32_t pend_cap = 0, n_chunks = 0;
+    uint64_t* strat_vis = nullptr;
 };
 enum : uint32_t { CHUNK_EVAL_HEAD = 0, CHUNK_PEND_COUNT = 1, CHUNK_PEND_HEAD = 2, CHUNK_SURV_COUNT = 3, CHUNK_MIS_HEAD = 4, kChunkCtlWords = 8 };
 struct conn_pending_t {
@@ -317,6 +322,9 @@
 __global__ void k_connect_scan(launch_args_t a);
 __global__ void k_connect_strat(launch_args_t a);
 __global__ void k_connect_strat_open(launch_args_t a);
+__global__ void k_connect_vis(launch_args_t a);
+__global__ void k_connect_strat_edge(launch_args_t a);
+__global__ void k_connect_strat_inner(launch_args_t a);
 __global__ void k_connect_eval(launch_args_t a, uint32_t chunk);
 __global__ void k_connect_shadow(launch_args_t a, uint32_t chunk);
 __global__ void k_connect_mis(launch_args_t a, uint32_t chunk);
diff --git a/wave_tracer_amd/csrc/wtgpu_knobs.h b/wave_tracer_amd/csrc/wtgpu_knobs.h
--- a/wave_tracer_amd/csrc/wtgpu_knobs.h
+++ b/wave_tracer_amd/csrc/wtgpu_knobs.h
@@ -8,7 +8,7 @@
     uint32_t first_rounds, rounds_margin, light_rounds, max_rounds, stagger_round;
     uint32_t shrink_r1, shrink_f1, shrink_r2, shrink_f2, shrink_h1, decay_q, decay_c;
     uint32_t heavy_waves_per_cu, round_blocks_per_cu, grid_div_b, grid_div_c, grid_div_hard, grid_mul_flux;
-    uint32_t sorted_interact, coop_io, staged_connect, tiled_splat;
+    uint32_t sorted_interact, coop_io, staged_connect, connect_vis, tiled_splat;
     uint32_t trace_staged, trace_stages, trace_staged_rounds, trace_sm, trace_ab;
     uint32_t dbg_stage;
     uint32_t host_prof, trace_launch, tail_diag, trace_ab_verbose;
diff --git a/wave_tracer_amd/csrc/wtgpu_knobs.hip b/wave_tracer_amd/csrc/wtgpu_knobs.hip
--- a/wave_tracer_amd/csrc/wtgpu_knobs.hip
+++ b/wave_tracer_amd/csrc/wtgpu_knobs.hip
@@ -49,6 +49,7 @@
     {"WTGPU_SORTED_INTERACT", K(sorted_interact), KNOB_U32, 0, 0, kU32, "pass A: 0 k_interact (one kernel, every walk); 1 k_classify + one kernel per material class; 2 k_classify + k_interact_sorted"},
     {"WTGPU_COOP_IO", K(coop_io), KNOB_U32, 0, 0, kU32, "1: pass A with wave-cooperative record transfers (k_interact_coop)"},
     {"WTGPU_STAGED_CONNECT", K(staged_connect), KNOB_U32, 0, 0, kU32, "connections: 0 k_connect_strat (one kernel per strategy item); 1 k_connect_eval -> k_connect_shadow -> k_connect_mis, in chunks"},
+    {"WTGPU_CONNECT_VIS", K(connect_vis), KNOB_U32, 0, 0, kU32, "connections with s,t >= 2: 1 their rays first (k_connect_vis), then k_connect_strat_inner for the visible ones, k_connect_strat_edge for the rest; 0 k_connect_strat for all"},
     {"WTGPU_TILED_SPLAT", K(tiled_splat), KNOB_U32, 1, 0, kU32, "0: the plain per-sample splat kernel"},
     {"WTGPU_TRACE_STAGED", K(trace_staged), KNOB_U32, 1, 0, kU32, "1: the traversal in stages (k_tr_axis / k_tr_cone / k_tr_policy / k_tr_tail) ..."},
     {"WTGPU_TRACE_STAGES", K(trace_stages), KNOB_U32, 3, 1, 16, "... with this many cone stages before the tail ..."},
diff --git a/wave_tracer_amd/csrc/wtgpu_upload.hip b/wave_tracer_amd/csrc/wtgpu_upload.hip
--- a/wave_tracer_amd/csrc/wtgpu_upload.hip
+++ b/wave_tracer_amd/csrc/wtgpu_upload.hip
@@ -153,6 +153,7 @@
             if ((rc = dmalloc(s, &X.chunk_ctl, (size_t)X.n_chunks * kChunkCtlWords))) return rc;
         } else
             X.pend_cap = 0;
+        if (s->knobs.connect_vis && (rc = dmalloc(s, &X.strat_vis, (size_t)kNumKeys * st.cap / 64 + kNumKeys))) return rc;
         s->pend_cap = X.pend_cap;
         s->n_chunks = X.n_chunks;
         bdpt_ext_t* dX = nullptr;
@@ -203,7 +204,7 @@
         const uint64_t mv = (uint64_t)h.opts.max_depth + 2;
         uint64_t per_sample = 4ull * (2 * ((pm ? kPathWalkWords : kWalkWords) + (pm ? 0 : mv * kVertexWords) + kTravWords + kStageWords + 2 + kTriListWords) + kCtxWords) + 64ull * 28ull + 2048ull;
         if (pm) per_sample += 2ull * 48ull * sizeof(utd_edge_rec_t) + sizeof(path_nee_rec_t) + 3ull * 4ull + 4ull + sizeof(uint2);
-        else per_sample += (s->knobs.staged_connect ? (uint64_t)s->knobs.conn_pool * (sizeof(conn_pending_t) + 4ull) : 0ull) + (s->knobs.sorted_interact ? 4ull * 2ull * kNumWalkClasses : 0ull);
+        else per_sample += (s->knobs.staged_connect ? (uint64_t)s->knobs.conn_pool * (sizeof(conn_pending_t) + 4ull) : 0ull) + (s->knobs.sorted_interact ? 4ull * 2ull * kNumWalkClasses : 0ull) + (s->knobs.connect_vis ? (uint64_t)kNumKeys / 8ull + 1ull : 0ull);
         uint64_t budget = (uint64_t)s->knobs.state_gb << 30;
         size_t free_b = 0, total_b = 0;
         if (hipMemGetInfo(&free_b, &total_b) == hipSuccess && free_b > 0) budget = std::min<uint64_t>(budget, (uint64_t)((double)free_b * 0.85));
```

Result: no change. 30.63 (median of 4 runs) (+0.3%).
